# argriffing/phyly

Hardware: AMD Instinct MI355X
Metric: sites/sec (arbplf-ll) (higher is better)
Workload: dtype f64

## Files before the change

### phyly_amd/csrc/plk_engine.hip

```cpp
#include <hip/hip_runtime.h>
#include <algorithm>
#include <utility>
#include <climits>
#include <cmath>
#include <cstdio>
#include <cstdlib>
#include <cstring>
#include <dlfcn.h>
#include <mutex>
#include <set>
#include <string>
#include <type_traits>
#include <vector>

#include "plk.h"
#include "plk_dd.h"
#define PLK_K1_FN __host__ __device__ static inline
#include "plk_k1_check.h"
#include "plk_program.h"

#define PLK_MAX_K 64
#define PLK_MAX_C 64

enum LlFamily { LL_FUSED4 = 1, LL_GENERIC = 2, LL_MFMA = 3, LL_VEC = 4 };
struct LlPlan {
    LlFamily family = LL_GENERIC;
    PlkK4Choice k4;
    PlkK4Stream k4s;
    bool pair_tables = false;
    int npairs = 0;
    int block = 0, wg_sites = 0;
    size_t lds = 0;
    int mfma_T = 0;
    bool mfma_ns2 = false;
    bool vec_rs = false;
    int vec_reg_lo = 0;
    long info_variant = 0, info_form = 0, info_exec_flops = 0;
};

struct plk_engine {
    int device = 0;
    hipStream_t stream = nullptr, own_stream = nullptr;
    bool info_pending = false;
    hipEvent_t ev0 = nullptr, ev1 = nullptr, ev2 = nullptr, ev3 = nullptr;
    hipEvent_t evk[64][2] = {};
    bool evk_pending[64] = {};
    int evk_next = 0;
    long evk_sum_ns = 0, evk_count = 0;
    std::string err;

    int N = 0, E = 0;
    std::vector<int> indptr, indices, preorder, b_to_idx, idx_to_a;
    int *d_indptr = nullptr, *d_indices = nullptr, *d_preorder = nullptr;

    int k = 0, C = 0, K = 0, root_mode = 0;
    std::vector<double> Qn, edge_rates, cat_rates, cat_prior, root_w;
    double *d_Qn = nullptr, *d_edge_rates = nullptr, *d_cat_rates = nullptr, *d_cat_prior = nullptr;
    double *d_root_w = nullptr;
    dd *d_Pdd = nullptr;
    double *d_P = nullptr, *d_dP = nullptr;
    bool dp_valid = false;
    dd *d_scratch = nullptr;
    size_t pdd_cap = 0, p_cap = 0, dp_cap = 0, scratch_cap = 0;
    bool model_dirty = true;

    long S = 0, Spad = 0;
    int pat_mode = 0;
    uint8_t *d_codes = nullptr;
    int nchar = 0;
    std::vector<double> defs;
    std::vector<char> node_observed;
    double *d_defs = nullptr;
    double *d_B = nullptr;
    std::vector<char> node_has_data;
    std::vector<int> node_codes;
    double *d_w = nullptr;

    bool prog_dirty = true, fmt_dirty = true, tables_dirty = true;
    LlPlan plan;
    PlkK4StreamCaps k4_caps;
    size_t k4_static_lds[3] = {};
    hipError_t k4_static_lds_err[3] = {};
    bool k4_static_lds_known = false;
    PlkProgram pg;
    std::vector<plk_op2> &ops = pg.ops;
    std::vector<int> &op_edge = pg.op_edge;
    std::vector<int> &tip_edge = pg.tip_edge;
    std::vector<char> &scale_node = pg.scale_node;
    std::vector<int> &obs_nodes = pg.obs_nodes;
    int &slots_needed = pg.slots_needed;
    PlkFused fu;
    PlkFusedPT fpt;
    unsigned *d_words_pt = nullptr;
    PlkFusedV4 fv4;
    PlkVecPT vpt;
    unsigned *d_cstream = nullptr; size_t cstream_cap = 0;
    int *d_obs_row = nullptr;
    int *d_row_nodes = nullptr, *d_tabs = nullptr;
    uint8_t *d_quad_lut = nullptr;
    int *d_quad_codes = nullptr;
    double *d_llstate = nullptr; size_t llstate_cap = 0;
    int num_cus = 256;
    int2 *d_ops = nullptr;
    int4 *d_fops = nullptr;
    unsigned *d_words = nullptr;
    std::vector<int> &mat_edge = fu.mat_edge;
    int *d_op_edge = nullptr, *d_tip_edge = nullptr, *d_obs_nodes = nullptr, *d_mat_edge = nullptr, *d_edge_slot = nullptr;
    double *d_PS = nullptr;
    double *d_tip = nullptr;
    double *d_frag = nullptr; size_t frag_cap = 0;
    double *d_root_wd = nullptr;
    int4 *d_mops = nullptr;
    double *d_exL = nullptr, *d_exF = nullptr;
    int *d_exmask = nullptr;
    dd *d_exscr = nullptr;
    size_t exL_cap = 0, exF_cap = 0, exmask_cap = 0, exscr_cap = 0;
    int *d_u4pack = nullptr;
    double *d_u4tip = nullptr;
    size_t u4pack_cap = 0, u4tip_cap = 0;
    double *d_stage = nullptr; size_t stage_cap = 0;
    double *d_uvmat = nullptr; size_t uvmat_cap = 0;
    int mfma_first_mv = -1, mfma_first_slot = -1, mfma_first_row = 0, vec_second_row = 0;
    size_t ps_cap = 0, tip_cap = 0;

    int cp_kind = 0;
    bool cp_tables_valid = false;
    PlkFused cpf;
    hipEvent_t cp_ev0 = nullptr, cp_ev1 = nullptr;
    long info_cat_posterior_ns = 0;
    int4 *d_cp_fops = nullptr;
    int2 *d_cp_ops = nullptr;
    int *d_cp_mat_edge = nullptr, *d_cp_tip_edge = nullptr, *d_cp_obs_nodes = nullptr, *d_cp_op_edge = nullptr, *d_cp_expo = nullptr, *d_cp_flag = nullptr;
    double *d_cp_PS = nullptr, *d_cp_tip = nullptr, *d_cp_out = nullptr;
    dd *d_cp_partial = nullptr;
    size_t cp_ps_cap = 0, cp_tip_cap = 0, cp_out_cap = 0, cp_expo_cap = 0, cp_partial_cap = 0;

    double *d_slots = nullptr; size_t slots_cap = 0;
    double *d_site_ll = nullptr; size_t site_ll_cap = 0;
    dd *d_partial = nullptr; size_t partial_cap = 0;
    double *d_work = nullptr; size_t work_cap = 0;

    long opt_force_generic = 0, opt_site_chunk = 0, opt_fused_ns = 0, opt_fused_asm = 1, opt_mfma = 1, opt_up_nodes = 2, opt_pair_tables = 1, opt_vec_reg_stack = 1, opt_mfma_ns2 = 0, opt_stream_grid = 0;
    void *comm = nullptr;
    int comm_ranks = 0;
    long info_pair_sums_kernel = 0, info_query_ns = 0;
    double *d_mixD = nullptr; size_t mixd_cap = 0;
    long info_mixture_sens_kernel = 0;
    long info_nni_kernel = 0;
    dd *d_plPdd = nullptr; double *d_plP = nullptr, *d_plrates = nullptr, *d_plstream = nullptr, *d_plT = nullptr, *d_pldense = nullptr;
    uint8_t *d_plcodes = nullptr;
    size_t plpdd_cap = 0, plp_cap = 0, plrates_cap = 0, plstream_cap = 0, plt_cap = 0, pldense_cap = 0, plcodes_cap = 0;
    long info_place_kernel = 0;
    long info_up4_path = 0;
    long info_down4_kernel = 0;
    hipEvent_t q_ev0 = nullptr, q_ev1 = nullptr;
    long info_ll_kernel = 0, info_updown_kernel = 0, info_ll_kernel_ns = 0, info_ll_total_ns = 0, info_ll_variant = 0, info_ll_form = 0, info_ll_fold = 0, info_ll_pairmul = 0, info_ll_triple = 0, info_ll_quad = 0, info_ll_barrier = 0, info_ll_exec_flops = 0, info_cat_posterior_kernel = 0;
};

static std::string g_create_error;

struct PlkNcclId { char internal[128]; };
struct PlkRccl {
    void *lib = nullptr;
    int (*GetUniqueId)(void *) = nullptr;
    int (*CommInitRank)(void **, int,  PlkNcclId, int) = nullptr;
    int (*AllReduce)(const void *, void *, size_t, int, int, void *, hipStream_t) = nullptr;
    int (*CommDestroy)(void *) = nullptr;
    const char *(*GetErrorString)(int) = nullptr;
    std::string err;
};
static PlkRccl g_rccl;
static std::mutex g_rccl_mu;

static bool rccl_load()
{
    std::lock_guard<std::mutex> lk(g_rccl_mu);
    if (g_rccl.lib) return true;
    const char *names[] = {"librccl.so.1", "librccl.so"};
    void *lib = nullptr;
    for (const char *n : names) if (!lib) lib = dlopen(n, RTLD_NOW | RTLD_NOLOAD);
    for (const char *n : names) if (!lib) lib = dlopen(n, RTLD_NOW | RTLD_GLOBAL);
    if (!lib) { g_rccl.err = std::string("RCCL is not available: ") + (dlerror() ? dlerror() : "librccl.so.1 not found"); return false; }
    g_rccl.GetUniqueId = reinterpret_cast<int (*)(void *)>(dlsym(lib, "ncclGetUniqueId"));
    g_rccl.CommInitRank = reinterpret_cast<int (*)(void **, int, PlkNcclId, int)>(dlsym(lib, "ncclCommInitRank"));
    g_rccl.AllReduce = reinterpret_cast<int (*)(const void *, void *, size_t, int, int, void *, hipStream_t)>(dlsym(lib, "ncclAllReduce"));
    g_rccl.CommDestroy = reinterpret_cast<int (*)(void *)>(dlsym(lib, "ncclCommDestroy"));
    g_rccl.GetErrorString = reinterpret_cast<const char *(*)(int)>(dlsym(lib, "ncclGetErrorString"));
    if (!g_rccl.GetUniqueId || !g_rccl.CommInitRank || !g_rccl.AllReduce || !g_rccl.CommDestroy) { g_rccl.err = "RCCL: entry points missing"; return false; }
    g_rccl.lib = lib;
    return true;
}

static std::string rccl_text(int rc) { return g_rccl.GetErrorString ? g_rccl.GetErrorString(rc) : ("code " + std::to_string(rc)); }



static std::mutex g_live_mu;
static std::set<const plk_engine *> g_live;
static bool g_exiting = false, g_atexit_set = false;

static bool plk_live(const plk_engine *h)
{
    if (!h) return false;
    std::lock_guard<std::mutex> lk(g_live_mu);
    return !g_exiting && g_live.count(h) != 0;
}

#define HIPCHK(h, call)                                                            \
    do {                                                                           \
        hipError_t e_ = (call);                                                    \
        if (e_ != hipSuccess) {                                                    \
            (h)->err = std::string(#call) + ": " + hipGetErrorString(e_);         \
            return PLK_E_DEVICE;                                                   \
        }                                                                          \
    } while (0)

template <typename T>
static int dev_alloc(plk_engine *h, T **p, size_t n)
{
    if (*p) { (void)hipFree(*p); *p = nullptr; }
    if (n == 0) n = 1;
    hipError_t e = hipMalloc((void **)p, n * sizeof(T));
    if (e != hipSuccess) {
        h->err = std::string("hipMalloc: ") + hipGetErrorString(e);
        *p = nullptr;
        return PLK_E_NOMEM;
    }
    return PLK_OK;
}

template <typename T>
static int dev_upload(plk_engine *h, T **p, const T *src, size_t n)
{
    int rc = dev_alloc(h, p, n);
    if (rc) return rc;
    if (n) HIPCHK(h, hipMemcpy(*p, src, n * sizeof(T), hipMemcpyHostToDevice));
    return PLK_OK;
}

template <typename T>
static int dev_reserve(plk_engine *h, T **p, size_t *cap, size_t n)
{
    if (*p && *cap >= n) return PLK_OK;
    int rc = dev_alloc(h, p, n);
    *cap = rc ? 0 : n;
    return rc;
}


__device__ static inline dd dd_div_d(dd x, double y)
{
    double q1 = x.hi / y;
    dd p = dd_two_prod(q1, y);
    dd r = dd_add(x, dd_make(-p.hi, -p.lo));
// ... 1029 lines not shown
#pragma unroll
                        for (int i = 0; i < K; i++) fe[i] *= m2[i];
                    } else {
                        const double *ev = a.EV + ((size_t)idx2 * a.C + c) * a.k * n + slc;
#pragma unroll
                        for (int i = 0; i < K; i++)
                            if (i < a.k) fe[i] *= ev[(size_t)i * n];
                    }
                }
                const double prior = as_uniform(a.cat_prior)[c] * (a.CW ? a.CW[(size_t)c * n + slc] : 1.0);
                if (want_d) {
                    if (b_leaf) up_stage_obs<K>(a, b, sg, tid, xs);
                    else {
                        const double *lb = a.LN + ((size_t)b * a.C + c) * a.k * n + slc;
                        for (int j = 0; j < a.k; j++) xs[j][tid] = lb[(size_t)j * n];
                    }
                    double y[K];
                    if (idx == a.mod_edge) up_matvec<K, 2>(a.D2T + ((size_t)c * a.E + idx) * K * K, a.k, xs, tid, y);
                    else if (a.dzero) up_matvec<K, 2>(a.DT + ((size_t)c * a.E + idx) * K * K, a.k, xs, tid, y);
                    else up_matvec<K, 0>(a.DT + ((size_t)c * a.E + idx) * K * K, a.k, xs, tid, y);
                    double d = 0.0;
#pragma unroll
                    for (int i = 0; i < K; i++) d = fma(fe[i], y[i], d);
                    dsum = fma(prior, d, dsum);
                }
                if (want_f) {
#pragma unroll
                    for (int i = 0; i < K; i++) xs[i][tid] = fe[i];
                    double fb[K];
                    up_matvec<K, 0>((idx == a.mod_edge ? a.DN : a.PN) + ((size_t)c * a.E + idx) * K * K, a.k, xs, tid, fb);
                    if (!b_leaf) {
                        double *fo = a.FN + ((size_t)b * a.C + c) * a.k * n + slc;
#pragma unroll
                        for (int i = 0; i < K; i++)
                            if (i < a.k && valid) fo[(size_t)i * n] = fb[i];
                    }
                    if (want_m) {
                        if (b_leaf) {
                            double lb[K];
                            up_load_obs_reg<K>(a, b, sg, lb);
#pragma unroll
                            for (int i = 0; i < K; i++) macc[i] = fma(prior * fb[i], lb[i], macc[i]);
                        } else {
                            const double *lb = a.LN + ((size_t)b * a.C + c) * a.k * n + slc;
#pragma unroll
                            for (int i = 0; i < K; i++)
                                if (i < a.k) macc[i] = fma(prior * fb[i], lb[(size_t)i * n], macc[i]);
                        }
                    }
                }
            }
            if (want_d && valid) a.DV[(size_t)idx * n + sl] = dsum * inv;
            if (want_m) {
                double *mv = a.MV + (size_t)b * a.k * n + slc;
#pragma unroll
                for (int i = 0; i < K; i++)
                    if (i < a.k && valid) mv[(size_t)i * n] = macc[i] * inv;
            }
        }
    }
}

#include "plk_pairsums.h"
#include "plk_mixsens.h"
#include "plk_nni.h"
#include "plk_place.h"

__global__ void k_build_edge_stream(int k, int K, int mode, const double *__restrict__ M, double *__restrict__ out)
{
    const size_t ce = blockIdx.x;
    const double *src = M + ce * k * k;
    double *dst = out + ce * K * K;
    for (int idx = threadIdx.x; idx < K * K; idx += blockDim.x) {
        int r = idx / K, q = idx - r * K;
        double v = 0.0;
        if (r < k && q < k) v = mode == 0 ? src[q * k + r] : src[r * k + q];
        dst[idx] = v;
    }
}


static int pad_K(int k)
{
    const int ks[] = {2, 4, 8, 16, 20, 32, 61, 64};
    for (int v : ks) if (k <= v) return v;
    return -1;
}

extern "C" const char *plk_create_error(void) { return g_create_error.c_str(); }

extern "C" int plk_create(plk_engine **out, int device)
{
    if (!out) return PLK_E_ARG;
    *out = nullptr;
    int ndev = 0;
    hipError_t e = hipGetDeviceCount(&ndev);
    if (e != hipSuccess || ndev <= 0) {
        g_create_error = std::string("plk_create: no HIP device available (") +
                         (e != hipSuccess ? hipGetErrorString(e) : "device count 0") +
                         "); this engine has no CPU fallback";
        return PLK_E_DEVICE;
    }
    if (device < 0 || device >= ndev) {
        g_create_error = "plk_create: device index out of range";
        return PLK_E_ARG;
    }
    e = hipSetDevice(device);
    if (e != hipSuccess) {
        g_create_error = std::string("hipSetDevice: ") + hipGetErrorString(e);
        return PLK_E_DEVICE;
    }
    plk_engine *h = new plk_engine();
    h->device = device;
    { int cus = 0; if (hipDeviceGetAttribute(&cus, hipDeviceAttributeMultiprocessorCount, device) == hipSuccess && cus > 0) h->num_cus = cus; }
    if (const char *v = getenv("ARBPLF_UP_NODES")) h->opt_up_nodes = atol(v);
    if (hipStreamCreate(&h->own_stream) != hipSuccess ||
        hipEventCreate(&h->ev0) != hipSuccess || hipEventCreate(&h->ev1) != hipSuccess ||
        hipEventCreate(&h->ev2) != hipSuccess || hipEventCreate(&h->ev3) != hipSuccess) {
        g_create_error = "plk_create: stream/event creation failed";
        delete h;
        return PLK_E_DEVICE;
    }
    {
        std::lock_guard<std::mutex> lk(g_live_mu);
        if (!g_atexit_set) {
            g_atexit_set = true;
            atexit([]() { std::lock_guard<std::mutex> lk2(g_live_mu); g_exiting = true; g_live.clear(); });
        }
        g_live.insert(h);
    }
    h->stream = h->own_stream;
    for (int i = 0; i < 64; i++)
        if (hipEventCreate(&h->evk[i][0]) != hipSuccess || hipEventCreate(&h->evk[i][1]) != hipSuccess) {
            g_create_error = "plk_create: event creation failed";
            plk_destroy(h);
            return PLK_E_DEVICE;
        }
    *out = h;
    return PLK_OK;
}

extern "C" void plk_destroy(plk_engine *h)
{
    if (!h) return;
    {
        std::lock_guard<std::mutex> lk(g_live_mu);
        if (g_exiting || !g_live.erase(h)) return;
    }
    (void)hipSetDevice(h->device);
    if (h->comm && g_rccl.CommDestroy) { (void)hipStreamSynchronize(h->stream); (void)g_rccl.CommDestroy(h->comm); h->comm = nullptr; }
    void *ptrs[] = {h->d_indptr, h->d_indices, h->d_preorder, h->d_Qn, h->d_edge_rates, h->d_cat_rates,
                    h->d_cat_prior, h->d_root_w, h->d_Pdd, h->d_P, h->d_dP, h->d_scratch, h->d_codes,
                    h->d_defs, h->d_B, h->d_w, h->d_ops, h->d_fops, h->d_words, h->d_mat_edge, h->d_edge_slot, h->d_op_edge, h->d_tip_edge, h->d_obs_nodes,
                    h->d_words_pt, h->d_row_nodes, h->d_tabs, h->d_quad_lut, h->d_quad_codes, h->d_llstate, h->d_cstream, h->d_obs_row, h->d_PS, h->d_tip, h->d_frag, h->d_root_wd, h->d_mops, h->d_u4pack, h->d_u4tip, h->d_uvmat, h->d_stage, h->d_exL, h->d_exF, h->d_exmask, h->d_exscr, h->d_slots, h->d_site_ll, h->d_partial, h->d_work,
                    h->d_cp_fops, h->d_cp_ops, h->d_cp_mat_edge, h->d_cp_tip_edge, h->d_cp_obs_nodes, h->d_cp_op_edge, h->d_cp_expo, h->d_cp_flag,
                    h->d_cp_PS, h->d_cp_tip, h->d_cp_out, h->d_cp_partial, h->d_mixD,
                    h->d_plPdd, h->d_plP, h->d_plrates, h->d_plstream, h->d_plT, h->d_pldense, h->d_plcodes};
    for (void *p : ptrs) if (p) (void)hipFree(p);
    if (h->ev0) (void)hipEventDestroy(h->ev0);
    if (h->ev1) (void)hipEventDestroy(h->ev1);
    if (h->ev2) (void)hipEventDestroy(h->ev2);
    if (h->ev3) (void)hipEventDestroy(h->ev3);
    if (h->cp_ev0) (void)hipEventDestroy(h->cp_ev0);
    if (h->q_ev0) (void)hipEventDestroy(h->q_ev0);
    if (h->q_ev1) (void)hipEventDestroy(h->q_ev1);
    if (h->cp_ev1) (void)hipEventDestroy(h->cp_ev1);
    for (int i = 0; i < 64; i++) for (int j = 0; j < 2; j++) if (h->evk[i][j]) (void)hipEventDestroy(h->evk[i][j]);
    if (h->own_stream) (void)hipStreamDestroy(h->own_stream);
    delete h;
}

extern "C" const char *plk_last_error(const plk_engine *h) { return plk_live(h) ? h->err.c_str() : "invalid engine handle"; }

extern "C" int plk_set_option(plk_engine *h, int option, long value)
{
    if (!plk_live(h)) return PLK_E_ARG;
    if (option == PLK_OPT_FORCE_GENERIC) { h->opt_force_generic = value; h->prog_dirty = true; return PLK_OK; }
    if (option == PLK_OPT_SITE_CHUNK) { h->opt_site_chunk = value; return PLK_OK; }
    if (option == PLK_OPT_FUSED_SITES_PER_LANE) { h->opt_fused_ns = value; h->fmt_dirty = true; return PLK_OK; }
    if (option == PLK_OPT_FUSED_ASM) { h->opt_fused_asm = value; h->fmt_dirty = true; return PLK_OK; }
    if (option == PLK_OPT_UP_NODES) { h->opt_up_nodes = value; return PLK_OK; }
    if (option == PLK_OPT_MFMA) { h->opt_mfma = value; h->fmt_dirty = true; return PLK_OK; }
    if (option == PLK_OPT_MFMA_NS2) { h->opt_mfma_ns2 = value; h->fmt_dirty = true; return PLK_OK; }
    if (option == PLK_OPT_VEC_REG_STACK) { h->opt_vec_reg_stack = value; h->fmt_dirty = true; return PLK_OK; }
    if (option == PLK_OPT_PAIR_TABLES) { h->opt_pair_tables = value; h->fmt_dirty = true; return PLK_OK; }
    if (option == PLK_OPT_STREAM_GRID) {
        if (value < 0) { h->err = "PLK_OPT_STREAM_GRID: a workgroup count, or 0 for the default"; return PLK_E_ARG; }
        h->opt_stream_grid = value; h->fmt_dirty = true; return PLK_OK;
    }
    h->err = "plk_set_option: unknown option";
    return PLK_E_ARG;
}

static int evk_resolve(plk_engine *h, int i)
{
    if (!h->evk_pending[i]) return PLK_OK;
    float ms = 0;
    HIPCHK(h, hipEventSynchronize(h->evk[i][1]));
    HIPCHK(h, hipEventElapsedTime(&ms, h->evk[i][0], h->evk[i][1]));
    h->evk_pending[i] = false;
    h->info_ll_kernel_ns = (long)(ms * 1e6);
    h->evk_sum_ns += h->info_ll_kernel_ns;
    h->evk_count++;
    return PLK_OK;
}

extern "C" int plk_get_info(plk_engine *h, int what, long *out)
{
    if (!plk_live(h) || !out) return PLK_E_ARG;
    if (what >= PLK_INFO_LAST_LL_KERNEL_NS && what <= PLK_INFO_LL_KERNEL_COUNT) {
        HIPCHK(h, hipSetDevice(h->device));
        int rc;
        for (int j = 0; j < 64; j++) if ((rc = evk_resolve(h, (h->evk_next + j) & 63))) return rc;
        if (h->info_pending) {
            float ms_t = 0;
            HIPCHK(h, hipEventSynchronize(h->ev3));
            HIPCHK(h, hipEventElapsedTime(&ms_t, h->ev0, h->ev3));
            h->info_ll_total_ns = (long)(ms_t * 1e6);
            h->info_pending = false;
        }
    }
    switch (what) {
    case PLK_INFO_LL_KERNEL_NS_SUM: *out = h->evk_sum_ns; h->evk_sum_ns = 0; return PLK_OK;
    case PLK_INFO_LL_KERNEL_COUNT: *out = h->evk_count; h->evk_count = 0; return PLK_OK;
    case PLK_INFO_LL_KERNEL: *out = h->info_ll_kernel; return PLK_OK;
    case PLK_INFO_UPDOWN_KERNEL: *out = h->info_updown_kernel; return PLK_OK;
    case PLK_INFO_CAT_POSTERIOR_KERNEL: *out = h->info_cat_posterior_kernel; return PLK_OK;
    case PLK_INFO_CATEGORIES: *out = h->C; return PLK_OK;
    case PLK_INFO_LAST_CAT_POSTERIOR_NS: *out = h->info_cat_posterior_ns; return PLK_OK;
    case PLK_INFO_PAIR_SUMS_KERNEL: *out = h->info_pair_sums_kernel; return PLK_OK;
    case PLK_INFO_LAST_QUERY_NS: *out = h->info_query_ns; return PLK_OK;
    case PLK_INFO_MIXTURE_SENS_KERNEL: *out = h->info_mixture_sens_kernel; return PLK_OK;
    case PLK_INFO_NNI_KERNEL: *out = h->info_nni_kernel; return PLK_OK;
    case PLK_INFO_PLACE_KERNEL: *out = h->info_place_kernel; return PLK_OK;
    case PLK_INFO_UP4_PATH: *out = h->info_up4_path; return PLK_OK;
    case PLK_INFO_DOWN4_KERNEL: *out = h->info_down4_kernel; return PLK_OK;
    case PLK_INFO_LL_VARIANT: *out = h->info_ll_variant; return PLK_OK;
    case PLK_INFO_LL_FORM: *out = h->info_ll_form; return PLK_OK;
    case PLK_INFO_LL_FOLD: *out = h->info_ll_fold; return PLK_OK;
    case PLK_INFO_LL_PAIRMUL: *out = h->info_ll_pairmul; return PLK_OK;
    case PLK_INFO_LL_TRIPLE: *out = h->info_ll_triple; return PLK_OK;
    case PLK_INFO_LL_QUAD: *out = h->info_ll_quad; return PLK_OK;
    case PLK_INFO_LL_BARRIER: *out = h->info_ll_barrier; return PLK_OK;
    case PLK_INFO_LL_EXEC_FLOPS: *out = h->info_ll_exec_flops; return PLK_OK;
    case PLK_INFO_PAIR_TABLES: *out = !h->fmt_dirty && h->plan.pair_tables ? h->plan.npairs : 0; return PLK_OK;
    case PLK_INFO_STACK_SLOTS: *out = h->slots_needed; return PLK_OK;
    case PLK_INFO_PROGRAM_OPS: *out = (long)h->ops.size(); return PLK_OK;
    case PLK_INFO_LAST_LL_KERNEL_NS: *out = h->info_ll_kernel_ns; return PLK_OK;
    case PLK_INFO_LAST_LL_TOTAL_NS: *out = h->info_ll_total_ns; return PLK_OK;
    }
    h->err = "plk_get_info: unknown item";
    return PLK_E_ARG;
}

extern "C" int plk_set_tree(plk_engine *h, int N, const int *indptr, const int *indices, const int *preorder)
{
    if (!plk_live(h)) return PLK_E_ARG;
    if (N < 2 || !indptr || !indices || !preorder) { h->err = "plk_set_tree: bad arguments"; return PLK_E_ARG; }
    HIPCHK(h, hipSetDevice(h->device));
    const int E = N - 1;
    if (indptr[0] != 0 || indptr[N] != E) { h->err = "plk_set_tree: indptr does not describe N-1 edges"; return PLK_E_ARG; }
    std::vector<int> b2i(N, -1), i2a(E, -1);
    for (int a = 0; a < N; a++) {
        if (indptr[a + 1] < indptr[a]) { h->err = "plk_set_tree: indptr not monotone"; return PLK_E_ARG; }
        for (int idx = indptr[a]; idx < indptr[a + 1]; idx++) {
            int b = indices[idx];
            if (b < 0 || b >= N || b == a || b2i[b] != -1) { h->err = "plk_set_tree: not a tree"; return PLK_E_ARG; }
            b2i[b] = idx;
            i2a[idx] = a;
        }
    }
    std::vector<char> seen(N, 0);
    for (int u = 0; u < N; u++) {
        int a = preorder[u];
        if (a < 0 || a >= N || seen[a]) { h->err = "plk_set_tree: preorder is not a permutation"; return PLK_E_ARG; }
        if (u == 0 ? b2i[a] != -1 : (b2i[a] == -1 || !seen[i2a[b2i[a]]])) {
            h->err = "plk_set_tree: preorder does not start at the root / parents first";
            return PLK_E_ARG;
        }
        seen[a] = 1;
    }
    h->N = N; h->E = E;
    h->indptr.assign(indptr, indptr + N + 1);
    h->indices.assign(indices, indices + E);
    h->preorder.assign(preorder, preorder + N);
    h->b_to_idx = b2i; h->idx_to_a = i2a;
    int rc;
    if ((rc = dev_upload(h, &h->d_indptr, indptr, (size_t)N + 1))) return rc;
    if ((rc = dev_upload(h, &h->d_indices, indices, (size_t)E))) return rc;
    if ((rc = dev_upload(h, &h->d_preorder, preorder, (size_t)N))) return rc;
    h->prog_dirty = true;
    h->model_dirty = true;
    h->pat_mode = 0;
    h->k = 0;
    return PLK_OK;
}

#define K1_CSR_NOTE " (edges numbered in CSR order)"

static int k1_check(plk_engine *h, const char *who, const double *edge_rates)
{
    char msg[320];
    const size_t kk = (size_t)h->k * h->k;
    if (plk_k1_check_values(h->k, h->C, h->E, h->Qn.data(), h->Qn.data() + kk, edge_rates, h->cat_rates.data(), h->cat_prior.data(),
                            h->root_mode, h->root_w.data(), msg, sizeof msg)) {
        h->err = std::string(who) + ": " + msg + K1_CSR_NOTE;
        return PLK_E_ARG;
// ... 270 lines not shown

static bool use_vec(const plk_engine *h)
{
    return !h->opt_force_generic && h->opt_mfma == 1 && h->pat_mode == 1 && h->k >= 9 && h->k <= 32;
}

static bool use_mfma(const plk_engine *h)
{
    return !h->opt_force_generic && h->opt_mfma && h->pat_mode == 1 && h->k >= 9 && h->k <= 64;
}

static size_t mfma_ll_lds_bytes(const plk_engine *h, int sites)
{
    const int T = (h->k + 15) / 16, kk4 = (h->k + 3) / 4;
    return (size_t)T * kk4 * 64 * sizeof(double) + h->obs_nodes.size() * (size_t)sites;
}

static int vec_reg_window(const plk_engine *h)
{
    std::vector<long> per_slot(std::max(h->slots_needed, 1), 0);
    for (const plk_op2 &o : h->ops) if ((o.x & 0xff) == OP_PUSH && o.y < (int)per_slot.size()) per_slot[o.y]++;
    long best = -1;
    int lo_best = 0;
    for (int lo = 0; lo + 3 <= std::max(h->slots_needed, 3); lo++) {
        long cnt = 0;
        for (int q = lo; q < lo + 3 && q < (int)per_slot.size(); q++) cnt += per_slot[q];
        if (cnt > best) { best = cnt; lo_best = lo; }
    }
    return lo_best;
}

static int upload_pair_table_lists(plk_engine *h)
{
    const PlkFusedPT &f = h->fpt;
    int rc;
    const size_t nrows = f.row_node.size(), ntab = f.tab_unit.size();
    std::vector<int> rn(5 * nrows, -1);
    for (size_t r = 0; r < nrows; r++) {
        rn[r] = f.row_node[r]; rn[nrows + r] = f.row_node2[r];
        if (r < f.row_node3.size()) rn[2 * nrows + r] = f.row_node3[r];
        if (r < f.row_node4.size()) { rn[3 * nrows + r] = f.row_node4[r]; rn[4 * nrows + r] = f.row_lut[r]; }
    }
    if ((rc = dev_upload(h, &h->d_row_nodes, rn.data(), rn.size()))) return rc;
    auto kind = [&](size_t t) { return t < f.tab_shape.size() && f.tab_shape[t] ? 2 : t < f.tab_el.size() && f.tab_el[t] >= 0 ? 1 : 0; };
    std::vector<size_t> order;
    for (int pass = 0; pass < 3; pass++)
        for (size_t t = 0; t < ntab; t++) if (kind(t) == pass) order.push_back(t);
    std::vector<int> tabs(10 * ntab, -1);
    std::vector<int> qcodes;
    for (size_t q = 0; q < ntab; q++) {
        const size_t t = order[q];
        tabs[q] = f.tab_unit[t]; tabs[ntab + q] = f.tab_edge[t]; tabs[2 * ntab + q] = f.tab_eb[t]; tabs[3 * ntab + q] = f.tab_ec[t];
        if (t < f.tab_el.size()) { tabs[4 * ntab + q] = f.tab_ea[t]; tabs[5 * ntab + q] = f.tab_el[t]; }
        if (t < f.tab_shape.size()) { tabs[6 * ntab + q] = f.tab_shape[t]; tabs[7 * ntab + q] = f.tab_et[t]; tabs[8 * ntab + q] = f.tab_ef[t]; tabs[9 * ntab + q] = f.tab_eg[t]; }
        if (kind(t) != 2) continue;
        const int row = t < f.tab_row.size() ? f.tab_row[t] : -1;
        if (row < 0 || (size_t)row >= nrows || f.row_lut[row] < 0 || h->node_codes.size() != (size_t)h->N) { h->err = "internal: a four-leaf table without its rank tables"; return PLK_E_ARG; }
        const int nd[4] = {f.row_node[row], f.row_node2[row], f.row_node3[row], f.row_node4[row]};
        for (int j = 0; j < 4; j++) {
            int code_of[4];
            plk_v4q_rank_codes(h->node_codes[nd[j]], code_of);
            qcodes.insert(qcodes.end(), code_of, code_of + 4);
        }
    }
    if (f.nquads > 0) {
        if ((rc = dev_upload(h, &h->d_quad_lut, f.lut.data(), f.lut.size()))) return rc;
        if ((rc = dev_upload(h, &h->d_quad_codes, qcodes.data(), qcodes.size()))) return rc;
    }
    return dev_upload(h, &h->d_tabs, tabs.data(), tabs.size());
}

static int stream_cus(const plk_engine *h) { return h->opt_stream_grid > 0 ? (int)std::min<long>(h->opt_stream_grid, h->num_cus) : h->num_cus; }

static int upload_formats_fused4(plk_engine *h, LlPlan &p)
{
    int rc;
    if (!h->k4_static_lds_known) {
        const void *fns[3] = {(const void *)k_ll_fused4_v4s<768>, (const void *)k_ll_fused4_v4<768>, (const void *)k_ll_fused4_v4<512>};
        for (int i = 0; i < 3; i++) {
            hipFuncAttributes fa;
            h->k4_static_lds_err[i] = hipFuncGetAttributes(&fa, fns[i]);
            if (h->k4_static_lds_err[i] == hipSuccess) h->k4_static_lds[i] = fa.sharedSizeBytes;
            else (void)hipGetLastError();
        }
        auto same_static_lds = [&](const void *fn) {
            hipFuncAttributes fh;
            if (hipFuncGetAttributes(&fh, fn) != hipSuccess) { (void)hipGetLastError(); return false; }
            return h->k4_static_lds_err[PLK_K4_LDS_V4S_768] == hipSuccess && fh.sharedSizeBytes == h->k4_static_lds[PLK_K4_LDS_V4S_768];
        };
        h->k4_caps.held = same_static_lds((const void *)k_ll_fused4_v4s<768, true>);
        h->k4_caps.pair = same_static_lds((const void *)k_ll_fused4_v4s<768, true, true>);
        h->k4_caps.groups = same_static_lds((const void *)k_ll_fused4_v4s<768, true, true, true>);
        h->k4_static_lds_known = true;
    }
    PlkK4Shape sh = {h->nchar, h->C, h->S, stream_cus(h), h->opt_pair_tables, h->opt_fused_asm, h->opt_fused_ns, {}};
    std::copy(h->k4_static_lds, h->k4_static_lds + 3, sh.static_lds);
    sh.node_codes = h->nchar <= 16 && h->node_codes.size() == (size_t)h->N ? h->node_codes.data() : nullptr;
    const long nunits = (h->S + PLK_V4S_UNIT - 1) / PLK_V4S_UNIT;
    PlkFusedV4S fv4s;
    p.k4 = plk_k4_choose(h->N, h->indptr.data(), h->indices.data(), h->pg, sh, h->k4_static_lds_err[PLK_K4_LDS_V4S_768] == hipSuccess, h->fu, h->fpt, h->fv4, fv4s);
    if (p.k4.variant == PLK_K4_V4S && dev_reserve(h, &h->d_cstream, &h->cstream_cap, (size_t)nunits * fv4s.chunks * PLK_V4S_UNIT) != PLK_OK) {
        h->err.clear();
        (void)hipGetLastError();
        p.k4 = plk_k4_choose(h->N, h->indptr.data(), h->indices.data(), h->pg, sh, false, h->fu, h->fpt, h->fv4, fv4s);
    }
    const PlkK4Choice &c = p.k4;
    if (c.variant == PLK_K4_NONE) return PLK_OK;
    if (c.variant == PLK_K4_V4) HIPCHK(h, h->k4_static_lds_err[c.tile == 1536 ? PLK_K4_LDS_V4_768 : PLK_K4_LDS_V4_512]);
    if (!c.bad.empty()) { h->err = "internal: " + c.bad; return PLK_E_ARG; }
    p.family = LL_FUSED4;
    p.block = c.block; p.wg_sites = c.tile; p.lds = c.lds;
    p.info_variant = c.variant == PLK_K4_CPP ? 3 : c.variant == PLK_K4_ASM ? 1 : c.variant == PLK_K4_ASM_PT ? 5 : 6;
    p.info_form = c.variant == PLK_K4_V4S ? 1 : 0;
    if (c.variant == PLK_K4_V4S) {
        PlkK4StreamCaps caps = h->k4_caps;
        if (c.triple.nodes + c.triple.quads > 0 && c.triple.groups > 1 && plk_k4_stream_can_group(c, caps) &&
            dev_reserve(h, &h->d_llstate, &h->llstate_cap, (size_t)nunits * PLK_V4S_UNIT * 3 / 2) != PLK_OK) {
            h->err.clear();
            (void)hipGetLastError();
            caps.partial_sums = false;
        }
        p.k4s = plk_k4_stream(h->N, h->indptr.data(), h->indices.data(), h->pg, sh, c, caps, h->fpt, std::move(fv4s));
        p.lds = p.k4s.lds;
        if (!p.k4s.note.empty()) h->err = p.k4s.note;
    }
    const int ntips = (int)h->tip_edge.size();
    if (c.variant == PLK_K4_CPP || c.variant == PLK_K4_ASM) {
        if ((rc = dev_upload(h, &h->d_fops, reinterpret_cast<const int4 *>(h->fu.fops.data()), h->fu.fops.size()))) return rc;
        if ((rc = dev_upload(h, &h->d_words, h->fu.words.data(), h->fu.words.size()))) return rc;
        std::vector<int> me = h->mat_edge;
        me.push_back(-1);
        if ((rc = dev_upload(h, &h->d_mat_edge, me.data(), me.size()))) return rc;
        std::vector<int> em(2 * (size_t)h->E, -1);
        for (size_t mi = 0; mi < h->mat_edge.size(); mi++) em[h->mat_edge[mi]] = (int)mi;
        for (int t = 0; t < ntips; t++) em[(size_t)h->E + h->tip_edge[t]] = t;
        if ((rc = dev_upload(h, &h->d_edge_slot, em.data(), em.size()))) return rc;
        if ((rc = dev_reserve(h, &h->d_PS, &h->ps_cap, (size_t)h->C * (h->mat_edge.size() + 1) * 16))) return rc;
        if ((rc = dev_reserve(h, &h->d_tip, &h->tip_cap, (size_t)h->C * (ntips + 1) * h->nchar * 4))) return rc;
        HIPCHK(h, hipMemsetAsync(h->d_PS, 0, (size_t)h->C * (h->mat_edge.size() + 1) * 16 * sizeof(double), h->stream));
        hipLaunchKernelGGL(k_build_tip, dim3(ntips + 1, h->C), dim3(64), 0, h->stream,
                           h->E, ntips + 1, h->nchar, h->d_tip_edge, h->d_Pdd, h->d_defs, h->d_tip);
        HIPCHK(h, hipGetLastError());
        return PLK_OK;
    }
    const PlkFusedPT &f = h->fpt;
    p.pair_tables = true; p.npairs = f.npairs;
    const PlkFusedV4S &vs = p.k4s.fv4s;
    const std::vector<unsigned> &words = c.variant == PLK_K4_V4S ? p.k4s.words() : c.variant == PLK_K4_V4 ? h->fv4.words : f.words;
    if ((rc = dev_upload(h, &h->d_words_pt, words.data(), words.size()))) return rc;
    if (c.variant == PLK_K4_V4S && (rc = dev_upload(h, &h->d_obs_row, vs.obs_row.data(), vs.obs_row.size()))) return rc;
    if ((rc = upload_pair_table_lists(h))) return rc;
    if (c.variant == PLK_K4_V4S) {
        const size_t total = (size_t)nunits * vs.chunks * PLK_V4S_UNIT;
        if (total > h->cstream_cap || (total + 255) / 256 > 0x7fffffffu) { h->err = "internal: code stream size"; return PLK_E_ARG; }
        hipLaunchKernelGGL(k_build_code_stream, dim3((unsigned)((total + 255) / 256)), dim3(256), 0, h->stream, h->d_codes, h->Spad, nunits,
                           h->d_obs_row, vs.nobs, h->d_row_nodes, (int)f.row_node.size(), h->nchar, vs.chunks,
                           f.nquads > 0 ? h->d_quad_lut : (const uint8_t *)nullptr, h->d_cstream);
        HIPCHK(h, hipGetLastError());
    }
    std::vector<int> em(2 * (size_t)h->E, -1);
    for (size_t mi = 0; mi < f.mat_edge.size(); mi++) em[f.mat_edge[mi]] = (int)mi;
    if ((rc = dev_upload(h, &h->d_edge_slot, em.data(), em.size()))) return rc;
    if ((rc = dev_reserve(h, &h->d_PS, &h->ps_cap, (size_t)h->C * (f.mat_edge.size() + 1) * 16))) return rc;
    if ((rc = dev_reserve(h, &h->d_tip, &h->tip_cap, (size_t)h->C * f.units * h->nchar * 4))) return rc;
    HIPCHK(h, hipMemsetAsync(h->d_PS, 0, (size_t)h->C * (f.mat_edge.size() + 1) * 16 * sizeof(double), h->stream));
    return PLK_OK;
}

static int upload_formats_generic(plk_engine *h, LlPlan &p)
{
    int rc;
    const int nops = (int)h->ops.size();
    std::vector<plk_op2> gops(h->ops);
    int first = -1, prev = -1;
    for (int pc = 0; pc < nops; pc++)
        if ((gops[pc].x & 0xff) == OP_MATVEC) {
            if (first < 0) first = pc;
            if (prev >= 0) gops[prev].y = pc;
            prev = pc;
        }
    if (prev >= 0) gops[prev].y = first;
    if ((rc = dev_upload(h, &h->d_ops, reinterpret_cast<const int2 *>(gops.data()), gops.size()))) return rc;
    if ((rc = dev_upload(h, &h->d_op_edge, h->op_edge.data(), h->op_edge.size()))) return rc;
    if ((rc = dev_reserve(h, &h->d_PS, &h->ps_cap, (size_t)h->C * std::max(nops, 1) * h->K * h->K))) return rc;
    p.family = LL_GENERIC;
    p.block = GEN_BLOCK; p.wg_sites = GEN_BLOCK;
    return PLK_OK;
}

static int upload_formats_vec(plk_engine *h, LlPlan &p)
{
    int rc;
    if ((rc = upload_formats_generic(h, p))) return rc;
    p.family = LL_VEC;
    p.block = VEC_BLOCK; p.wg_sites = VEC_BLOCK;
    p.vec_rs = h->opt_vec_reg_stack && h->K <= 20 && h->slots_needed >= 1;
    p.vec_reg_lo = p.vec_rs ? vec_reg_window(h) : 0;
    if (h->opt_pair_tables && h->K <= 32 && !h->obs_nodes.empty()) {
        const long per_pair = (long)h->nchar * h->nchar * h->K * (long)sizeof(double);
        const int max_pairs = (int)std::min<long>(INT_MAX, (64L << 20) / std::max<long>(per_pair, 1));
        plk_fused_pt_build(h->N, h->indptr.data(), h->indices.data(), h->pg, h->nchar, max_pairs, h->fpt, false);
        if (h->fpt.npairs > 0) {
            plk_vec_pt_build(h->fpt, h->nchar, h->vpt);
            const std::string bad = plk_vec_pt_check(h->N, h->indptr.data(), h->indices.data(), h->pg, h->fpt, h->vpt, h->nchar, h->E);
            if (!bad.empty()) { h->err = "internal: " + bad; return PLK_E_ARG; }
            if ((rc = upload_pair_table_lists(h)) ||
                (rc = dev_upload(h, &h->d_mops, reinterpret_cast<const int4 *>(h->vpt.ops.data()), h->vpt.ops.size())) ||
                (rc = dev_upload(h, &h->d_op_edge, h->vpt.op_edge.data(), h->vpt.op_edge.size())) ||
                (rc = dev_reserve(h, &h->d_PS, &h->ps_cap, (size_t)h->C * h->vpt.ops.size() * h->K * h->K)) ||
                (rc = dev_reserve(h, &h->d_tip, &h->tip_cap, (size_t)h->C * h->fpt.units * h->nchar * h->K))) return rc;
            p.pair_tables = true; p.npairs = h->fpt.npairs;
            return PLK_OK;
        }
    }
    if ((rc = dev_reserve(h, &h->d_tip, &h->tip_cap, (size_t)h->C * (h->tip_edge.size() + 1) * h->nchar * h->K))) return rc;
    PlkChain ch;
    plk_chain_build(h->N, h->pg, 3, h->indices.data(), nullptr, nullptr, nullptr, ch);
    const std::string bad = plk_chain_check(h->N, h->pg, ch, 3, INT_MAX, 0, 0, 0, 0, 0);
    if (!bad.empty()) { h->err = "internal: " + bad; return PLK_E_ARG; }
    h->mfma_first_slot = ch.first_slot; h->mfma_first_row = ch.first_row; h->vec_second_row = ch.second_row;
    return dev_upload(h, &h->d_mops, reinterpret_cast<const int4 *>(ch.ops.data()), ch.ops.size());
}

static int upload_formats_mfma(plk_engine *h, LlPlan &p)
{
    int rc;
    if ((rc = upload_formats_generic(h, p))) return rc;
    const int nops = (int)h->ops.size(), ntips = (int)h->tip_edge.size();
    const int T = (h->k + 15) / 16, R = 4 * T, kk4 = (h->k + 3) / 4;
    p.family = LL_MFMA;
    p.mfma_T = T;
    p.mfma_ns2 = h->opt_mfma_ns2 == 1 && T >= 3 && mfma_ll_lds_bytes(h, 2 * MF_SITES) <= PLK_LDS_LIMIT;
    p.block = MF_BLOCK; p.wg_sites = p.mfma_ns2 ? 2 * MF_SITES : MF_SITES;
    p.lds = mfma_ll_lds_bytes(h, p.wg_sites);
    std::vector<double> rwd((size_t)4 * R, 0.0);
    for (int i = 0; i < h->k; i++) rwd[(size_t)(i & 3) * R + (i >> 2)] = h->root_w[i];
    if ((rc = dev_upload(h, &h->d_root_wd, rwd.data(), rwd.size()))) return rc;
    if ((rc = dev_reserve(h, &h->d_frag, &h->frag_cap, (size_t)h->C * nops * T * kk4 * 64))) return rc;
    if ((rc = dev_reserve(h, &h->d_tip, &h->tip_cap, (size_t)h->C * (ntips + 1) * h->nchar * 4 * R))) return rc;
    PlkChain ch;
    plk_chain_build(h->N, h->pg, 0, nullptr, nullptr, nullptr, nullptr, ch);
    const std::string bad = plk_chain_check(h->N, h->pg, ch, 0, INT_MAX, 0, 0, 0, MF_SITES, (size_t)h->obs_nodes.size() * MF_SITES);
    if (!bad.empty()) { h->err = "internal: " + bad; return PLK_E_ARG; }
    h->mfma_first_slot = ch.first_slot; h->mfma_first_row = ch.first_row;
    h->mfma_first_mv = -1;
    for (size_t pc = 0; pc < h->pg.ops.size() && h->mfma_first_mv < 0; pc++) if ((h->pg.ops[pc].x & 0xff) == OP_MATVEC) h->mfma_first_mv = (int)pc;
    return dev_upload(h, &h->d_mops, reinterpret_cast<const int4 *>(ch.ops.data()), ch.ops.size());
}

static long ll_exec_flops(const plk_engine *h, const LlPlan &p)
{
    long nprod = 0, nmul = 0;
    if (p.family == LL_VEC && p.pair_tables) {
        for (const PlkFusedPT::VOp &o : h->fpt.vops) { if (o.code == OP_MATVEC) nprod++; if (o.code == OP_TIP_MUL || o.code == OP_POPMUL) nmul++; }
    } else if (p.family == LL_FUSED4 && p.pair_tables) {
        nprod = (long)h->fpt.mat_edge.size();
        for (unsigned w : h->fpt.words) {
            const unsigned hx = w & 31;
            if (hx == OP_TIP_MUL || hx == PLK_WORD_TIPMUL_NOWAIT || hx == PLK_WORD_MATVEC_TIPMUL) nmul++;
            if ((hx >= 16 && hx < 20) || hx >= 28 || (hx >= PLK_WORD_SET_POPMUL && hx < PLK_WORD_SET_POPMUL + 4)) nmul++;
        }
    } else {
        for (const plk_op2 &o : h->ops) {
            const int code = o.x & 0xff;
            if (code == OP_MATVEC) nprod++;
            if (code == OP_TIP_MUL || code == OP_NODE_MUL || code == OP_POPMUL) nmul++;
            if ((code == OP_TIP_SET || code == OP_TIP_MUL) && p.family == LL_GENERIC) { nprod++; if (code == OP_TIP_MUL) nmul++; }
        }
    }
    const long kp = p.family == LL_MFMA ? (h->k + 15) / 16 * 16 : h->k;
    return (long)h->C * (nprod * (2 * kp * kp - kp) + nmul * h->k);
}

static int upload_formats(plk_engine *h)
{
    int rc;
    h->fmt_dirty = true;
    std::vector<int> te = h->tip_edge;
    te.push_back(-1);
    if ((rc = dev_upload(h, &h->d_tip_edge, te.data(), te.size()))) return rc;
    if ((rc = dev_upload(h, &h->d_obs_nodes, h->obs_nodes.data(), h->obs_nodes.size()))) return rc;
    LlPlan p;
    if (!h->opt_force_generic && h->k == 4 && h->pat_mode == 1 && (rc = upload_formats_fused4(h, p))) return rc;
    if (p.family != LL_FUSED4) {
        if (use_vec(h)) rc = upload_formats_vec(h, p);
        else if (use_mfma(h) && mfma_ll_lds_bytes(h, MF_SITES) <= PLK_LDS_LIMIT) rc = upload_formats_mfma(h, p);
        else rc = upload_formats_generic(h, p);
        if (rc) return rc;
    }
    p.info_exec_flops = ll_exec_flops(h, p);
    h->plan = std::move(p);
    h->fmt_dirty = false;
    h->tables_dirty = true;
    return PLK_OK;
}

static int build_tables(plk_engine *h)
{
    const LlPlan &p = h->plan;
    const int nops = (int)h->ops.size(), ntips = (int)h->tip_edge.size(), K = h->K, C = h->C;
    if (p.family == LL_FUSED4) return run_expm(h, true);
    if (p.family == LL_VEC && p.pair_tables) {
        const int nv = (int)h->vpt.ops.size(), ntab = (int)h->fpt.tab_unit.size();
        hipLaunchKernelGGL(k_build_stream, dim3(nv, C), dim3(K * K >= 256 ? 256 : 64), 0, h->stream,
                           h->k, K, h->E, nv, h->d_op_edge, h->d_P, h->d_PS);
        hipLaunchKernelGGL(k_build_tables_pt_vec, dim3(ntab, C, 8), dim3(256), (size_t)4 * h->nchar * h->k * sizeof(double), h->stream,
                           h->k, K, h->E, ntab, h->fpt.units, h->nchar, h->d_tabs, h->d_Pdd, h->d_defs, h->d_tip);
        HIPCHK(h, hipGetLastError());
        h->tables_dirty = false;
        return PLK_OK;
    }
    if (nops > 0)
        hipLaunchKernelGGL(k_build_stream, dim3(nops, C), dim3(K * K >= 256 ? 256 : 64), 0, h->stream,
                           h->k, K, h->E, nops, h->d_op_edge, h->d_P, h->d_PS);
    if (p.family == LL_VEC) {
        hipLaunchKernelGGL(k_build_tip_vec, dim3(ntips + 1, C), dim3(256), 0, h->stream,
                           h->k, K, h->E, ntips, h->nchar, h->d_tip_edge, h->d_Pdd, h->d_defs, h->d_tip);
    } else if (p.family == LL_MFMA) {
        const int T = p.mfma_T, R = 4 * T, kk4 = (h->k + 3) / 4;
        hipLaunchKernelGGL(k_build_frag, dim3(nops, C), dim3(256), 0, h->stream,
                           h->k, T, kk4, h->E, nops, h->d_op_edge, h->d_P, h->d_frag);
        hipLaunchKernelGGL(k_build_tip_dist, dim3(ntips + 1, C), dim3(256), 0, h->stream,
                           h->k, R, h->E, ntips, h->nchar, h->d_tip_edge, h->d_Pdd, h->d_defs, h->K, h->d_tip);
    }
    HIPCHK(h, hipGetLastError());
    h->tables_dirty = false;
    return PLK_OK;
}

template <int D, int NS>
static void launch_fused(plk_engine *h, const FusedArgs &a, unsigned grid, size_t lds)
{
    hipLaunchKernelGGL((k_ll_fused4<D, NS>), dim3(grid), dim3(PLK_TILE), lds, h->stream, a);
}

template <typename F>
static void dispatch_K(int K, F &&f)
{
    switch (K) {
    case 2: f(std::integral_constant<int, 2>{}); break;
    case 4: f(std::integral_constant<int, 4>{}); break;
    case 8: f(std::integral_constant<int, 8>{}); break;
    case 16: f(std::integral_constant<int, 16>{}); break;
    case 20: f(std::integral_constant<int, 20>{}); break;
    case 32: f(std::integral_constant<int, 32>{}); break;
    case 61: f(std::integral_constant<int, 61>{}); break;
    default: f(std::integral_constant<int, 64>{}); break;
    }
}

template <int K>
static void launch_generic(plk_engine *h, const GenArgs &a, unsigned grid)
{
    hipLaunchKernelGGL(k_ll_generic<K>, dim3(grid), dim3(GEN_BLOCK), 0, h->stream, a);
}

#define PLK_PARTIAL_OFF 72

static int reserve_partials(plk_engine *h, bool want_sum, unsigned n, dd **partial)
{
    *partial = nullptr;
    if (!want_sum) return PLK_OK;
    const int rc = dev_reserve(h, &h->d_partial, &h->partial_cap, (size_t)n + PLK_PARTIAL_OFF);
    if (rc == PLK_OK) *partial = h->d_partial + PLK_PARTIAL_OFF;
    return rc;
}

static int launch_ll_fused4(plk_engine *h, const LlPlan &p, double *d_out, bool want_sum, unsigned *npartials)
{
    const PlkK4Choice &c = p.k4;
    const long S = h->S;
    const int ntiles = (int)((S + p.wg_sites - 1) / p.wg_sites);
    unsigned grid = (unsigned)ntiles;
    if (c.variant == PLK_K4_V4S) grid = (unsigned)std::min<long>(((S + PLK_V4S_UNIT - 1) / PLK_V4S_UNIT + 11) / 12, stream_cus(h));
    else if (c.variant == PLK_K4_V4 || c.variant == PLK_K4_ASM_PT) grid = (unsigned)std::min(ntiles, c.tile == 512 ? 2 * h->num_cus : h->num_cus);
    *npartials = c.variant == PLK_K4_V4S ? grid * 12 : (unsigned)ntiles;
    int rc;
    FusedArgs a;
    if ((rc = reserve_partials(h, want_sum, *npartials, &a.partial))) return rc;
    a.S = S; a.Spad = h->Spad; a.C = h->C; a.nops = (int)h->ops.size(); a.nmat = (int)h->mat_edge.size();
    a.ntips = (int)h->tip_edge.size() + 1; a.nchar = h->nchar; a.nobs = (int)h->obs_nodes.size();
    a.ops = h->d_fops; a.PS = h->d_PS; a.tip = h->d_tip;
    a.codes = h->d_codes; a.obs_nodes = h->d_obs_nodes; a.defs = h->d_defs;
    a.cat_prior = h->d_cat_prior; a.root_w = h->d_root_w; a.w = h->d_w;
    a.site_ll = d_out;
    a.root_mode = h->root_mode; a.first_row = h->fu.first_row;
    if (p.pair_tables) {
        const PlkFusedPT &f = h->fpt;
        FusedPTArgs pa;
        pa.f = a;
        pa.f.nmat = (int)f.mat_edge.size(); pa.f.ntips = f.units; pa.f.nobs = (int)f.row_node.size();
        pa.words = h->d_words_pt; pa.row_nodes = h->d_row_nodes; pa.nwords = (int)(c.variant == PLK_K4_ASM_PT ? f.words.size() : h->fv4.words.size());
        pa.first_unit = f.first_unit; pa.first_row = f.first_row; pa.second_row = f.second_row; pa.ntiles = ntiles;
        pa.warm = c.warm;
        if (c.variant == PLK_K4_V4S) {
            FusedV4SArgs sa;
            sa.pt = pa;
            const PlkK4Stream &r = p.k4s;
            const bool pairmul = r.runs == PlkK4Stream::PAIR;
            sa.pt.nwords = (int)r.stride();
            sa.stream = h->d_cstream; sa.chunks = r.fv4s.chunks; sa.first_y = r.fv4s.first_y[0];
            sa.sync = r.sync;
            h->info_ll_barrier = (sa.sync == 0 ? 1 : sa.sync == 1 ? 2 : 3) | (r.sync_auto ? 16 : 0);
            sa.first_y1 = pairmul ? r.pair.first_y1[0] : 0u; sa.first_b1 = pairmul ? r.pair.first_b1 : 0u;
            sa.groups = r.triple.groups; sa.cg = r.triple.Cg > 0 ? r.triple.Cg : h->C;
            sa.part_sum = h->d_llstate;
            sa.part_exp = h->d_llstate ? reinterpret_cast<int *>(h->d_llstate + (size_t)((S + PLK_V4S_UNIT - 1) / PLK_V4S_UNIT) * PLK_V4S_UNIT) : nullptr;
            if (sa.groups > 1) {
                if (!pairmul || !h->d_llstate || h->llstate_cap < (size_t)((S + PLK_V4S_UNIT - 1) / PLK_V4S_UNIT) * PLK_V4S_UNIT * 3 / 2) { h->err = "internal: category groups without their plan"; return PLK_E_ARG; }
                hipLaunchKernelGGL((k_ll_fused4_v4s<768, true, true, true>), dim3(grid), dim3(p.block), p.lds, h->stream, sa);
            } else if (pairmul) hipLaunchKernelGGL((k_ll_fused4_v4s<768, true, true>), dim3(grid), dim3(p.block), p.lds, h->stream, sa);
            else if (r.held) hipLaunchKernelGGL((k_ll_fused4_v4s<768, true>), dim3(grid), dim3(p.block), p.lds, h->stream, sa);
            else hipLaunchKernelGGL((k_ll_fused4_v4s<768, false>), dim3(grid), dim3(p.block), p.lds, h->stream, sa);
        } else if (c.variant == PLK_K4_V4) {
            FusedV4Args va;
            va.pt = pa; va.first_y = h->fv4.first_y; va.first_z = h->fv4.first_z; va.second_z = h->fv4.second_z;
            if (c.tile == 1536) hipLaunchKernelGGL(k_ll_fused4_v4<768>, dim3(grid), dim3(p.block), p.lds, h->stream, va);
            else hipLaunchKernelGGL(k_ll_fused4_v4<512>, dim3(grid), dim3(p.block), p.lds, h->stream, va);
        } else if (c.tile == 1024) hipLaunchKernelGGL(k_ll_fused4_asm_pt<1024>, dim3(grid), dim3(p.block), p.lds, h->stream, pa);
        else hipLaunchKernelGGL(k_ll_fused4_asm_pt<512>, dim3(grid), dim3(p.block), p.lds, h->stream, pa);
        return PLK_OK;
    }
    if (c.variant == PLK_K4_ASM) {
        FusedAsmArgs aa;
        aa.f = a; aa.words = h->d_words;
        aa.first_tip = h->fu.asm_first_tip; aa.first_row = h->fu.asm_first_row; aa.second_row = h->fu.asm_second_row;
        aa.pack4 = c.pack4;
        if (c.D == 4) hipLaunchKernelGGL(k_ll_fused4_asm<4>, dim3(grid), dim3(p.block), p.lds, h->stream, aa);
        else hipLaunchKernelGGL(k_ll_fused4_asm<8>, dim3(grid), dim3(p.block), p.lds, h->stream, aa);
        return PLK_OK;
    }
    if (c.NS == 2) {
        if (c.D == 4) launch_fused<4, 2>(h, a, grid, p.lds);
        else launch_fused<8, 2>(h, a, grid, p.lds);
    } else {
        if (c.D == 4) launch_fused<4, 1>(h, a, grid, p.lds);
        else if (c.D == 8) launch_fused<8, 1>(h, a, grid, p.lds);
        else launch_fused<16, 1>(h, a, grid, p.lds);
    }
    return PLK_OK;
}

static int launch_ll_vec(plk_engine *h, const LlPlan &p, double *d_out, bool want_sum, unsigned *npartials)
{
    const long S = h->S;
    const int K = h->K;
    const unsigned grid = (unsigned)((S + p.wg_sites - 1) / p.wg_sites);
    *npartials = grid;
    int rc;
    VecArgs a;
    if ((rc = reserve_partials(h, want_sum, grid, &a.partial))) return rc;
    if ((rc = dev_reserve(h, &h->d_slots, &h->slots_cap, (size_t)std::max(h->slots_needed, 1) * K * S))) return rc;
    a.S = S; a.Spad = h->Spad; a.k = h->k; a.C = h->C; a.nops = (int)h->ops.size(); a.ntips = (int)h->tip_edge.size(); a.nchar = h->nchar;
    a.root_mode = h->root_mode; a.ops = h->d_mops; a.PS = h->d_PS; a.tip = h->d_tip; a.codes = h->d_codes;
    a.obs_nodes = h->d_obs_nodes; a.first_slot = h->mfma_first_slot; a.first_row = h->mfma_first_row; a.second_row = h->vec_second_row;
    a.obs_nodes2 = nullptr; a.units = 0;
    if (p.pair_tables) {
        const int nrows = (int)h->fpt.row_node.size();
        a.nops = (int)h->vpt.ops.size(); a.obs_nodes = h->d_row_nodes; a.obs_nodes2 = h->d_row_nodes + nrows; a.units = h->fpt.units;
        a.first_slot = 0; a.first_row = h->vpt.first_row;
    }
    a.cat_prior = h->d_cat_prior; a.root_w = h->d_root_w; a.w = h->d_w; a.slots = h->d_slots; a.site_ll = d_out;
    a.reg_lo = p.vec_reg_lo;
    if (p.vec_rs && K == 16) hipLaunchKernelGGL((k_ll_vec_rs<16, 3>), dim3(grid), dim3(p.block), 0, h->stream, a);
    else if (p.vec_rs) hipLaunchKernelGGL((k_ll_vec_rs<20, 3>), dim3(grid), dim3(p.block), 0, h->stream, a);
    else if (K == 16) hipLaunchKernelGGL(k_ll_vec<16>, dim3(grid), dim3(p.block), 0, h->stream, a);
    else if (K == 20) hipLaunchKernelGGL(k_ll_vec<20>, dim3(grid), dim3(p.block), 0, h->stream, a);
    else hipLaunchKernelGGL(k_ll_vec<32>, dim3(grid), dim3(p.block), 0, h->stream, a);
    return PLK_OK;
}

static int launch_ll_mfma(plk_engine *h, const LlPlan &p, double *d_out, bool want_sum, unsigned *npartials)
{
    const long S = h->S;
    const int T = p.mfma_T, R = 4 * T, kk4 = (h->k + 3) / 4;
    const unsigned grid = (unsigned)((S + p.wg_sites - 1) / p.wg_sites);
    *npartials = grid;
    int rc;
    MfmaArgs a;
    if ((rc = reserve_partials(h, want_sum, grid, &a.partial))) return rc;
    const long slot_stride = (long)grid * p.wg_sites * 4;
    if ((rc = dev_reserve(h, &h->d_slots, &h->slots_cap, (size_t)std::max(h->slots_needed, 1) * R * slot_stride))) return rc;
    a.S = S; a.Spad = h->Spad; a.k = h->k; a.kk4 = kk4; a.C = h->C; a.nops = (int)h->ops.size(); a.ntips = (int)h->tip_edge.size();
    a.nchar = h->nchar; a.root_mode = h->root_mode; a.ops = h->d_mops; a.frag = h->d_frag; a.tip = h->d_tip;
    a.obs_nodes = h->d_obs_nodes; a.nobs = (int)h->obs_nodes.size();
    a.first_slot = h->mfma_first_slot; a.first_row = h->mfma_first_row; a.first_mv = h->mfma_first_mv;
    a.codes = h->d_codes; a.cat_prior = h->d_cat_prior; a.root_wd = h->d_root_wd; a.w = h->d_w;
    a.slots = h->d_slots; a.slot_stride = slot_stride; a.site_ll = d_out;
    if (p.mfma_ns2 && T == 3) hipLaunchKernelGGL(k_ll_mfma_ns2<3>, dim3(grid), dim3(p.block), p.lds, h->stream, a);
    else if (p.mfma_ns2) hipLaunchKernelGGL(k_ll_mfma_ns2<4>, dim3(grid), dim3(p.block), p.lds, h->stream, a);
    else if (T == 1) hipLaunchKernelGGL(k_ll_mfma<1>, dim3(grid), dim3(p.block), p.lds, h->stream, a);
    else if (T == 2) hipLaunchKernelGGL(k_ll_mfma<2>, dim3(grid), dim3(p.block), p.lds, h->stream, a);
    else if (T == 3) hipLaunchKernelGGL(k_ll_mfma_occ4<3>, dim3(grid), dim3(p.block), p.lds, h->stream, a);
    else hipLaunchKernelGGL(k_ll_mfma_occ4<4>, dim3(grid), dim3(p.block), p.lds, h->stream, a);
    return PLK_OK;
}

static int launch_ll_generic(plk_engine *h, const LlPlan &p, double *d_out, bool want_sum, unsigned *npartials)
{
    const long S = h->S;
    const unsigned grid = (unsigned)((S + p.wg_sites - 1) / p.wg_sites);
    *npartials = grid;
    int rc;
    GenArgs a;
    if ((rc = reserve_partials(h, want_sum, grid, &a.partial))) return rc;
    if ((rc = dev_reserve(h, &h->d_slots, &h->slots_cap, (size_t)std::max(h->slots_needed, 1) * h->k * S))) return rc;
    a.S = S; a.Spad = h->Spad; a.k = h->k; a.C = h->C; a.nops = (int)h->ops.size(); a.nchar = h->nchar;
    a.pat_mode = h->pat_mode; a.root_mode = h->root_mode; a.ops = h->d_ops; a.PS = h->d_PS;
    a.codes = h->d_codes; a.defs = h->d_defs; a.B = h->d_B; a.cat_prior = h->d_cat_prior;
    a.root_w = h->d_root_w; a.w = h->d_w; a.slots = h->d_slots; a.site_ll = d_out;
    dispatch_K(h->K, [&](auto Kc) { launch_generic<decltype(Kc)::value>(h, a, grid); });
    return PLK_OK;
}

static int ll_impl(plk_engine *h, double *site_ll_out, int where, double *sum_out, double *sum_dev, bool async)
{
    if (h->k == 0 || h->pat_mode == 0) { h->err = "plk_ll: tree, model and patterns must be set"; return PLK_E_ARG; }
    HIPCHK(h, hipSetDevice(h->device));
    int rc;
    HIPCHK(h, hipEventRecord(h->ev0, h->stream));
    if (h->prog_dirty) { if ((rc = build_program(h))) return rc; }
    if (h->fmt_dirty) { if ((rc = upload_formats(h))) return rc; }
    if (h->model_dirty) { if ((rc = run_expm(h, true, false))) return rc; }
    if (h->tables_dirty) { if ((rc = build_tables(h))) return rc; }
    const LlPlan &p = h->plan;
    const bool want_sum = sum_out || sum_dev;
    const long S = h->S;
    double *d_out = nullptr;
    if (site_ll_out) {
        if (where == PLK_DEVICE) d_out = site_ll_out;
        else { if ((rc = dev_reserve(h, &h->d_site_ll, &h->site_ll_cap, (size_t)S))) return rc; d_out = h->d_site_ll; }
    }
    const int evi = h->evk_next;
    h->evk_next = (evi + 1) & 63;
    if ((rc = evk_resolve(h, evi))) return rc;
    HIPCHK(h, hipEventRecord(h->evk[evi][0], h->stream));
    unsigned npartials = 0;
    h->info_ll_barrier = 0;
    switch (p.family) {
    case LL_FUSED4: rc = launch_ll_fused4(h, p, d_out, want_sum, &npartials); break;
    case LL_VEC: rc = launch_ll_vec(h, p, d_out, want_sum, &npartials); break;
    case LL_MFMA: rc = launch_ll_mfma(h, p, d_out, want_sum, &npartials); break;
    default: rc = launch_ll_generic(h, p, d_out, want_sum, &npartials); break;
    }
    if (rc) return rc;
    h->info_ll_kernel = p.family; h->info_ll_variant = p.info_variant; h->info_ll_form = p.info_form; h->info_ll_fold = p.k4s.info_fold; h->info_ll_pairmul = p.k4s.info_pairmul; h->info_ll_triple = p.k4s.info_triple; h->info_ll_quad = p.k4s.info_quad; h->info_ll_exec_flops = p.info_exec_flops;
    HIPCHK(h, hipGetLastError());
    HIPCHK(h, hipEventRecord(h->evk[evi][1], h->stream));
    h->evk_pending[evi] = true;
    if (want_sum) {
        dd *out = sum_dev ? reinterpret_cast<dd *>(sum_dev) : h->d_partial;
        const int g2 = npartials > 1024 ? (int)std::min<unsigned>(64u, (npartials + 511) / 512) : 1;
        if (g2 > 1) {
            hipLaunchKernelGGL(k_dd_slices, dim3(g2), dim3(256), 0, h->stream, (int)npartials, h->d_partial + PLK_PARTIAL_OFF, h->d_partial + 4);
            hipLaunchKernelGGL(k_dd_final, dim3(1), dim3(64), 0, h->stream, g2, h->d_partial + 4, out);
        } else {
            hipLaunchKernelGGL(k_dd_final, dim3(1), dim3(256), 0, h->stream, (int)npartials, h->d_partial + PLK_PARTIAL_OFF, out);
        }
// ... 2127 lines not shown
```

### phyly_amd/csrc/plk_fused4_v4p_asm.h

```cpp
#ifndef PLK_FUSED4_V4P_ASM_H
#define PLK_FUSED4_V4P_ASM_H

#define PLK_V4P_STACK_SLOTS 3
#define PLK_V4P_FOLD_ADV 36
#define PLK_V4P_PAIR_EVEN 52
#define PLK_V4P_PAIR_ODD 55
#define PLK_V4P_GEN_OBS_EVEN {0, 1, 3, 4, 12, 13, 14, 20, 21, 22}
#define PLK_V4P_GEN_OBS_ODD {5, 11, 15, 19, 23, 27, 31, -1, 59, 63}
#define PLK_V4P_GEN_OBS_FOLDED {1, 4, 12, 13, 14, 21, 22}

#define PLK_V4P_PROGRAM_HELD \
        "v_mov_b32 v24, 0\n\t" \
        "v_mov_b32 v25, 0x3ff00000\n\t" \
        "v_mov_b32 v32, 0\n\t" \
        "v_mov_b32 v33, 0x3ff00000\n\t" \
        "v_mov_b32 v26, 0\n\t" \
        "v_mov_b32 v27, 0x3ff00000\n\t" \
        "v_mov_b32 v34, 0\n\t" \
        "v_mov_b32 v35, 0x3ff00000\n\t" \
        "v_mov_b32 v28, 0\n\t" \
        "v_mov_b32 v29, 0x3ff00000\n\t" \
        "v_mov_b32 v36, 0\n\t" \
        "v_mov_b32 v37, 0x3ff00000\n\t" \
        "v_mov_b32 v30, 0\n\t" \
        "v_mov_b32 v31, 0x3ff00000\n\t" \
        "v_mov_b32 v38, 0\n\t" \
        "v_mov_b32 v39, 0x3ff00000\n\t" \
        "v_mov_b32 v76, %[voff]\n\t" \
        "s_mov_b64 s[34:35], %[strm]\n\t" \
        "v_mov_b64 v[74:75], %[c0]\n\t" \
        "v_mov_b64 v[146:147], %[c1]\n\t" \
        "v_mov_b64 v[148:149], %[c2]\n\t" \
        "s_add_u32 s34, s34, 0x600\n\t" \
        "s_addc_u32 s35, s35, 0\n\t" \
        "v_mov_b32 v78, 0\n\t" \
        "v_mov_b32 v79, 0\n\t" \
        "s_mov_b64 s[20:21], %[ops]\n\t" \
        "s_mov_b64 s[30:31], %[mstream]\n\t" \
        "s_movk_i32 s27, 0xfc02\n\t" \
        "s_mov_b32 m0, 0\n\t" \
        "s_load_dwordx16 s[68:83], s[20:21], 0x0\n\t" \
        "s_load_dwordx16 s[84:99], s[20:21], 0x40\n\t" \
        "s_add_u32 s20, s20, 0x80\n\t" \
        "s_addc_u32 s21, s21, 0\n\t" \
        "s_load_dwordx16 s[36:51], s[30:31], 0x0\n\t" \
        "s_load_dwordx16 s[52:67], s[30:31], 0x40\n\t" \
        "s_getpc_b64 s[24:25]\n\t" \
        ".Lpcref_%=:\n" \
        "s_add_u32 s26, s24, .Lh0_%=-.Lpcref_%=\n\t" \
        "s_addc_u32 s25, s25, 0\n\t" \
        "v_bfe_u32 v72, v74, 0, 8\n\t" \
        "v_bfe_u32 v73, v75, 0, 8\n\t" \
        "v_add_lshl_u32 v72, v72, %[y0], 5\n\t" \
        "v_add_lshl_u32 v73, v73, %[y0], 5\n\t" \
        "ds_read_b128 v[56:59], v72\n\t" \
        "ds_read_b128 v[60:63], v72 offset:16\n\t" \
        "ds_read_b128 v[64:67], v73\n\t" \
        "ds_read_b128 v[68:71], v73 offset:16\n\t" \
        "v_bfe_u32 v72, v74, %[b1], 8\n\t" \
        "v_bfe_u32 v73, v75, %[b1], 8\n\t" \
        "v_add_lshl_u32 v72, v72, %[y1], 5\n\t" \
        "v_add_lshl_u32 v73, v73, %[y1], 5\n\t" \
        "ds_read_b128 v[130:133], v72\n\t" \
        "ds_read_b128 v[134:137], v72 offset:16\n\t" \
        "ds_read_b128 v[138:141], v73\n\t" \
        "ds_read_b128 v[142:145], v73 offset:16\n\t" \
        "s_waitcnt lgkmcnt(0)\n\t" \
        "s_movrels_b64 s[22:23], s[68:69]\n\t" \
        "s_addk_i32 m0, 0x2\n\t" \
        "s_or_b32 s24, s26, s22\n\t" \
        "s_setpc_b64 s[24:25]\n\t" \
        ".p2align 15\n" \
        ".Lh0_%=:\n" \
        "s_waitcnt lgkmcnt(0)\n\t" \
        "v_mov_b64 v[24:25], v[56:57]\n\t" \
        "v_mov_b64 v[32:33], v[64:65]\n\t" \
        "v_mov_b64 v[26:27], v[58:59]\n\t" \
        "v_mov_b64 v[34:35], v[66:67]\n\t" \
        "v_mov_b64 v[28:29], v[60:61]\n\t" \
        "v_mov_b64 v[36:37], v[68:69]\n\t" \
        "v_mov_b64 v[30:31], v[62:63]\n\t" \
        "v_mov_b64 v[38:39], v[70:71]\n\t" \
        "s_lshr_b32 s28, s23, 16\n\t" \
        "v_bfe_u32 v72, v74, s23, 8\n\t" \
        "v_bfe_u32 v73, v75, s23, 8\n\t" \
        "v_add_lshl_u32 v72, v72, s28, 5\n\t" \
        "v_add_lshl_u32 v73, v73, s28, 5\n\t" \
        "ds_read_b128 v[56:59], v72\n\t" \
        "ds_read_b128 v[60:63], v72 offset:16\n\t" \
        "ds_read_b128 v[64:67], v73\n\t" \
        "ds_read_b128 v[68:71], v73 offset:16\n\t" \
        "s_movrels_b64 s[22:23], s[68:69]\n\t" \
        "s_addk_i32 m0, 0x2\n\t" \
        "s_or_b32 s24, s26, s22\n\t" \
        "s_setpc_b64 s[24:25]\n\t" \
        ".p2align 9\n" \
        "s_waitcnt lgkmcnt(0)\n\t" \
        "v_mul_f64 v[24:25], v[24:25], v[56:57]\n\t" \
        "v_mul_f64 v[32:33], v[32:33], v[64:65]\n\t" \
        "v_mul_f64 v[26:27], v[26:27], v[58:59]\n\t" \
        "v_mul_f64 v[34:35], v[34:35], v[66:67]\n\t" \
        "v_mul_f64 v[28:29], v[28:29], v[60:61]\n\t" \
        "v_mul_f64 v[36:37], v[36:37], v[68:69]\n\t" \
        "v_mul_f64 v[30:31], v[30:31], v[62:63]\n\t" \
        "v_mul_f64 v[38:39], v[38:39], v[70:71]\n\t" \
        "s_lshr_b32 s28, s23, 16\n\t" \
        "v_bfe_u32 v72, v74, s23, 8\n\t" \
        "v_bfe_u32 v73, v75, s23, 8\n\t" \
        "v_add_lshl_u32 v72, v72, s28, 5\n\t" \
        "v_add_lshl_u32 v73, v73, s28, 5\n\t" \
        "ds_read_b128 v[56:59], v72\n\t" \
        "ds_read_b128 v[60:63], v72 offset:16\n\t" \
        "ds_read_b128 v[64:67], v73\n\t" \
        "ds_read_b128 v[68:71], v73 offset:16\n\t" \
        "s_movrels_b64 s[22:23], s[68:69]\n\t" \
        "s_addk_i32 m0, 0x2\n\t" \
        "s_or_b32 s24, s26, s22\n\t" \
        "s_setpc_b64 s[24:25]\n\t" \
        ".p2align 9\n" \
        "s_waitcnt lgkmcnt(0)\n\t" \
        "v_mul_f64 v[40:41], s[36:37], v[24:25]\n\t" \
        "v_mul_f64 v[48:49], s[36:37], v[32:33]\n\t" \
        "v_mul_f64 v[42:43], s[38:39], v[24:25]\n\t" \
        "v_mul_f64 v[50:51], s[38:39], v[32:33]\n\t" \
        "v_mul_f64 v[44:45], s[40:41], v[24:25]\n\t" \
        "v_mul_f64 v[52:53], s[40:41], v[32:33]\n\t" \
        "v_mul_f64 v[46:47], s[42:43], v[24:25]\n\t" \
        "v_mul_f64 v[54:55], s[42:43], v[32:33]\n\t" \
        "v_fma_f64 v[40:41], s[44:45], v[26:27], v[40:41]\n\t" \
        "v_fma_f64 v[48:49], s[44:45], v[34:35], v[48:49]\n\t" \
        "v_fma_f64 v[42:43], s[46:47], v[26:27], v[42:43]\n\t" \
        "v_fma_f64 v[50:51], s[46:47], v[34:35], v[50:51]\n\t" \
        "v_fma_f64 v[44:45], s[48:49], v[26:27], v[44:45]\n\t" \
        "v_fma_f64 v[52:53], s[48:49], v[34:35], v[52:53]\n\t" \
        "v_fma_f64 v[46:47], s[50:51], v[26:27], v[46:47]\n\t" \
        "v_fma_f64 v[54:55], s[50:51], v[34:35], v[54:55]\n\t" \
        "v_fma_f64 v[40:41], s[52:53], v[28:29], v[40:41]\n\t" \
        "v_fma_f64 v[48:49], s[52:53], v[36:37], v[48:49]\n\t" \
        "v_fma_f64 v[42:43], s[54:55], v[28:29], v[42:43]\n\t" \
        "v_fma_f64 v[50:51], s[54:55], v[36:37], v[50:51]\n\t" \
        "v_fma_f64 v[44:45], s[56:57], v[28:29], v[44:45]\n\t" \
        "v_fma_f64 v[52:53], s[56:57], v[36:37], v[52:53]\n\t" \
        "v_fma_f64 v[46:47], s[58:59], v[28:29], v[46:47]\n\t" \
        "v_fma_f64 v[54:55], s[58:59], v[36:37], v[54:55]\n\t" \
        "v_fma_f64 v[24:25], s[60:61], v[30:31], v[40:41]\n\t" \
        "v_fma_f64 v[32:33], s[60:61], v[38:39], v[48:49]\n\t" \
        "v_fma_f64 v[26:27], s[62:63], v[30:31], v[42:43]\n\t" \
        "v_fma_f64 v[34:35], s[62:63], v[38:39], v[50:51]\n\t" \
        "v_fma_f64 v[28:29], s[64:65], v[30:31], v[44:45]\n\t" \
        "v_fma_f64 v[36:37], s[64:65], v[38:39], v[52:53]\n\t" \
        "v_fma_f64 v[30:31], s[66:67], v[30:31], v[46:47]\n\t" \
        "v_fma_f64 v[38:39], s[66:67], v[38:39], v[54:55]\n\t" \
        "s_add_u32 s30, s30, 0x80\n\t" \
        "s_addc_u32 s31, s31, 0\n\t" \
        "s_load_dwordx16 s[36:51], s[30:31], 0x0\n\t" \
        "s_load_dwordx16 s[52:67], s[30:31], 0x40\n\t" \
        "s_movrels_b64 s[22:23], s[68:69]\n\t" \
        "s_addk_i32 m0, 0x2\n\t" \
        "s_or_b32 s24, s26, s22\n\t" \
        "s_setpc_b64 s[24:25]\n\t" \
        ".p2align 9\n" \
        "v_mul_f64 v[24:25], v[24:25], v[56:57]\n\t" \
        "v_mul_f64 v[32:33], v[32:33], v[64:65]\n\t" \
        "v_mul_f64 v[26:27], v[26:27], v[58:59]\n\t" \
        "v_mul_f64 v[34:35], v[34:35], v[66:67]\n\t" \
        "v_mul_f64 v[28:29], v[28:29], v[60:61]\n\t" \
        "v_mul_f64 v[36:37], v[36:37], v[68:69]\n\t" \
        "v_mul_f64 v[30:31], v[30:31], v[62:63]\n\t" \
        "v_mul_f64 v[38:39], v[38:39], v[70:71]\n\t" \
        "s_lshr_b32 s28, s23, 16\n\t" \
        "v_bfe_u32 v72, v74, s23, 8\n\t" \
        "v_bfe_u32 v73, v75, s23, 8\n\t" \
        "v_add_lshl_u32 v72, v72, s28, 5\n\t" \
        "v_add_lshl_u32 v73, v73, s28, 5\n\t" \
        "ds_read_b128 v[56:59], v72\n\t" \
        "ds_read_b128 v[60:63], v72 offset:16\n\t" \
        "ds_read_b128 v[64:67], v73\n\t" \
        "ds_read_b128 v[68:71], v73 offset:16\n\t" \
        "s_movrels_b64 s[22:23], s[68:69]\n\t" \
        "s_addk_i32 m0, 0x2\n\t" \
        "s_or_b32 s24, s26, s22\n\t" \
        "s_setpc_b64 s[24:25]\n\t" \
        ".p2align 9\n" \
        "s_waitcnt lgkmcnt(0)\n\t" \
        "v_mul_f64 v[40:41], s[36:37], v[24:25]\n\t" \
        "v_mul_f64 v[48:49], s[36:37], v[32:33]\n\t" \
        "v_mul_f64 v[42:43], s[38:39], v[24:25]\n\t" \
        "v_mul_f64 v[50:51], s[38:39], v[32:33]\n\t" \
        "v_mul_f64 v[44:45], s[40:41], v[24:25]\n\t" \
        "v_mul_f64 v[52:53], s[40:41], v[32:33]\n\t" \
        "v_mul_f64 v[46:47], s[42:43], v[24:25]\n\t" \
        "v_mul_f64 v[54:55], s[42:43], v[32:33]\n\t" \
        "v_fma_f64 v[40:41], s[44:45], v[26:27], v[40:41]\n\t" \
        "v_fma_f64 v[48:49], s[44:45], v[34:35], v[48:49]\n\t" \
        "v_fma_f64 v[42:43], s[46:47], v[26:27], v[42:43]\n\t" \
        "v_fma_f64 v[50:51], s[46:47], v[34:35], v[50:51]\n\t" \
        "v_fma_f64 v[44:45], s[48:49], v[26:27], v[44:45]\n\t" \
        "v_fma_f64 v[52:53], s[48:49], v[34:35], v[52:53]\n\t" \
        "v_fma_f64 v[46:47], s[50:51], v[26:27], v[46:47]\n\t" \
        "v_fma_f64 v[54:55], s[50:51], v[34:35], v[54:55]\n\t" \
        "v_fma_f64 v[40:41], s[52:53], v[28:29], v[40:41]\n\t" \
        "v_fma_f64 v[48:49], s[52:53], v[36:37], v[48:49]\n\t" \
        "v_fma_f64 v[42:43], s[54:55], v[28:29], v[42:43]\n\t" \
        "v_fma_f64 v[50:51], s[54:55], v[36:37], v[50:51]\n\t" \
        "v_fma_f64 v[44:45], s[56:57], v[28:29], v[44:45]\n\t" \
        "v_fma_f64 v[52:53], s[56:57], v[36:37], v[52:53]\n\t" \
        "v_fma_f64 v[46:47], s[58:59], v[28:29], v[46:47]\n\t" \
        "v_fma_f64 v[54:55], s[58:59], v[36:37], v[54:55]\n\t" \
        "v_fma_f64 v[24:25], s[60:61], v[30:31], v[40:41]\n\t" \
        "v_fma_f64 v[32:33], s[60:61], v[38:39], v[48:49]\n\t" \
        "v_fma_f64 v[26:27], s[62:63], v[30:31], v[42:43]\n\t" \
        "v_fma_f64 v[34:35], s[62:63], v[38:39], v[50:51]\n\t" \
        "v_fma_f64 v[28:29], s[64:65], v[30:31], v[44:45]\n\t" \
        "v_fma_f64 v[36:37], s[64:65], v[38:39], v[52:53]\n\t" \
        "v_fma_f64 v[30:31], s[66:67], v[30:31], v[46:47]\n\t" \
// ... 1571 lines not shown
        "v_mul_f64 v[46:47], s[42:43], v[24:25]\n\t" \
        "v_mul_f64 v[54:55], s[42:43], v[32:33]\n\t" \
        "v_fma_f64 v[40:41], s[44:45], v[26:27], v[40:41]\n\t" \
        "v_fma_f64 v[48:49], s[44:45], v[34:35], v[48:49]\n\t" \
        "v_fma_f64 v[42:43], s[46:47], v[26:27], v[42:43]\n\t" \
        "v_fma_f64 v[50:51], s[46:47], v[34:35], v[50:51]\n\t" \
        "v_fma_f64 v[44:45], s[48:49], v[26:27], v[44:45]\n\t" \
        "v_fma_f64 v[52:53], s[48:49], v[34:35], v[52:53]\n\t" \
        "v_fma_f64 v[46:47], s[50:51], v[26:27], v[46:47]\n\t" \
        "v_fma_f64 v[54:55], s[50:51], v[34:35], v[54:55]\n\t" \
        "v_fma_f64 v[40:41], s[52:53], v[28:29], v[40:41]\n\t" \
        "v_fma_f64 v[48:49], s[52:53], v[36:37], v[48:49]\n\t" \
        "v_fma_f64 v[42:43], s[54:55], v[28:29], v[42:43]\n\t" \
        "v_fma_f64 v[50:51], s[54:55], v[36:37], v[50:51]\n\t" \
        "v_fma_f64 v[44:45], s[56:57], v[28:29], v[44:45]\n\t" \
        "v_fma_f64 v[52:53], s[56:57], v[36:37], v[52:53]\n\t" \
        "v_fma_f64 v[46:47], s[58:59], v[28:29], v[46:47]\n\t" \
        "v_fma_f64 v[54:55], s[58:59], v[36:37], v[54:55]\n\t" \
        "v_fma_f64 v[24:25], s[60:61], v[30:31], v[40:41]\n\t" \
        "v_fma_f64 v[32:33], s[60:61], v[38:39], v[48:49]\n\t" \
        "v_fma_f64 v[26:27], s[62:63], v[30:31], v[42:43]\n\t" \
        "v_fma_f64 v[34:35], s[62:63], v[38:39], v[50:51]\n\t" \
        "v_fma_f64 v[28:29], s[64:65], v[30:31], v[44:45]\n\t" \
        "v_fma_f64 v[36:37], s[64:65], v[38:39], v[52:53]\n\t" \
        "v_fma_f64 v[30:31], s[66:67], v[30:31], v[46:47]\n\t" \
        "v_fma_f64 v[38:39], s[66:67], v[38:39], v[54:55]\n\t" \
        "s_add_u32 s30, s30, 0x80\n\t" \
        "s_addc_u32 s31, s31, 0\n\t" \
        "s_load_dwordx16 s[36:51], s[30:31], 0x0\n\t" \
        "s_load_dwordx16 s[52:67], s[30:31], 0x40\n\t" \
        "v_mul_f64 v[24:25], v[24:25], v[98:99]\n\t" \
        "v_mul_f64 v[32:33], v[32:33], v[106:107]\n\t" \
        "v_mul_f64 v[26:27], v[26:27], v[100:101]\n\t" \
        "v_mul_f64 v[34:35], v[34:35], v[108:109]\n\t" \
        "v_mul_f64 v[28:29], v[28:29], v[102:103]\n\t" \
        "v_mul_f64 v[36:37], v[36:37], v[110:111]\n\t" \
        "v_mul_f64 v[30:31], v[30:31], v[104:105]\n\t" \
        "v_mul_f64 v[38:39], v[38:39], v[112:113]\n\t" \
        "v_max_u32 v80, v25, v27\n\t" \
        "v_max3_u32 v80, v29, v31, v80\n\t" \
        "v_lshrrev_b32 v80, 20, v80\n\t" \
        "v_sub_u32 v72, 0x3fe, v80\n\t" \
        "v_ldexp_f64 v[24:25], v[24:25], v72\n\t" \
        "v_ldexp_f64 v[26:27], v[26:27], v72\n\t" \
        "v_ldexp_f64 v[28:29], v[28:29], v72\n\t" \
        "v_ldexp_f64 v[30:31], v[30:31], v72\n\t" \
        "v_add3_u32 v78, v78, v80, s27\n\t" \
        "v_max_u32 v81, v33, v35\n\t" \
        "v_max3_u32 v81, v37, v39, v81\n\t" \
        "v_lshrrev_b32 v81, 20, v81\n\t" \
        "v_sub_u32 v72, 0x3fe, v81\n\t" \
        "v_ldexp_f64 v[32:33], v[32:33], v72\n\t" \
        "v_ldexp_f64 v[34:35], v[34:35], v72\n\t" \
        "v_ldexp_f64 v[36:37], v[36:37], v72\n\t" \
        "v_ldexp_f64 v[38:39], v[38:39], v72\n\t" \
        "v_add3_u32 v79, v79, v81, s27\n\t" \
        "s_movrels_b64 s[22:23], s[68:69]\n\t" \
        "s_addk_i32 m0, 0x2\n\t" \
        "s_or_b32 s24, s26, s22\n\t" \
        "s_setpc_b64 s[24:25]\n\t" \
        ".p2align 9\n" \
        "s_waitcnt lgkmcnt(0)\n\t" \
        "v_mul_f64 v[40:41], s[36:37], v[24:25]\n\t" \
        "v_mul_f64 v[48:49], s[36:37], v[32:33]\n\t" \
        "v_mul_f64 v[42:43], s[38:39], v[24:25]\n\t" \
        "v_mul_f64 v[50:51], s[38:39], v[32:33]\n\t" \
        "v_mul_f64 v[44:45], s[40:41], v[24:25]\n\t" \
        "v_mul_f64 v[52:53], s[40:41], v[32:33]\n\t" \
        "v_mul_f64 v[46:47], s[42:43], v[24:25]\n\t" \
        "v_mul_f64 v[54:55], s[42:43], v[32:33]\n\t" \
        "v_fma_f64 v[40:41], s[44:45], v[26:27], v[40:41]\n\t" \
        "v_fma_f64 v[48:49], s[44:45], v[34:35], v[48:49]\n\t" \
        "v_fma_f64 v[42:43], s[46:47], v[26:27], v[42:43]\n\t" \
        "v_fma_f64 v[50:51], s[46:47], v[34:35], v[50:51]\n\t" \
        "v_fma_f64 v[44:45], s[48:49], v[26:27], v[44:45]\n\t" \
        "v_fma_f64 v[52:53], s[48:49], v[34:35], v[52:53]\n\t" \
        "v_fma_f64 v[46:47], s[50:51], v[26:27], v[46:47]\n\t" \
        "v_fma_f64 v[54:55], s[50:51], v[34:35], v[54:55]\n\t" \
        "v_fma_f64 v[40:41], s[52:53], v[28:29], v[40:41]\n\t" \
        "v_fma_f64 v[48:49], s[52:53], v[36:37], v[48:49]\n\t" \
        "v_fma_f64 v[42:43], s[54:55], v[28:29], v[42:43]\n\t" \
        "v_fma_f64 v[50:51], s[54:55], v[36:37], v[50:51]\n\t" \
        "v_fma_f64 v[44:45], s[56:57], v[28:29], v[44:45]\n\t" \
        "v_fma_f64 v[52:53], s[56:57], v[36:37], v[52:53]\n\t" \
        "v_fma_f64 v[46:47], s[58:59], v[28:29], v[46:47]\n\t" \
        "v_fma_f64 v[54:55], s[58:59], v[36:37], v[54:55]\n\t" \
        "v_fma_f64 v[24:25], s[60:61], v[30:31], v[40:41]\n\t" \
        "v_fma_f64 v[32:33], s[60:61], v[38:39], v[48:49]\n\t" \
        "v_fma_f64 v[26:27], s[62:63], v[30:31], v[42:43]\n\t" \
        "v_fma_f64 v[34:35], s[62:63], v[38:39], v[50:51]\n\t" \
        "v_fma_f64 v[28:29], s[64:65], v[30:31], v[44:45]\n\t" \
        "v_fma_f64 v[36:37], s[64:65], v[38:39], v[52:53]\n\t" \
        "v_fma_f64 v[30:31], s[66:67], v[30:31], v[46:47]\n\t" \
        "v_fma_f64 v[38:39], s[66:67], v[38:39], v[54:55]\n\t" \
        "s_add_u32 s30, s30, 0x80\n\t" \
        "s_addc_u32 s31, s31, 0\n\t" \
        "s_load_dwordx16 s[36:51], s[30:31], 0x0\n\t" \
        "s_load_dwordx16 s[52:67], s[30:31], 0x40\n\t" \
        "v_mul_f64 v[24:25], v[24:25], v[114:115]\n\t" \
        "v_mul_f64 v[32:33], v[32:33], v[122:123]\n\t" \
        "v_mul_f64 v[26:27], v[26:27], v[116:117]\n\t" \
        "v_mul_f64 v[34:35], v[34:35], v[124:125]\n\t" \
        "v_mul_f64 v[28:29], v[28:29], v[118:119]\n\t" \
        "v_mul_f64 v[36:37], v[36:37], v[126:127]\n\t" \
        "v_mul_f64 v[30:31], v[30:31], v[120:121]\n\t" \
        "v_mul_f64 v[38:39], v[38:39], v[128:129]\n\t" \
        "v_max_u32 v80, v25, v27\n\t" \
        "v_max3_u32 v80, v29, v31, v80\n\t" \
        "v_lshrrev_b32 v80, 20, v80\n\t" \
        "v_sub_u32 v72, 0x3fe, v80\n\t" \
        "v_ldexp_f64 v[24:25], v[24:25], v72\n\t" \
        "v_ldexp_f64 v[26:27], v[26:27], v72\n\t" \
        "v_ldexp_f64 v[28:29], v[28:29], v72\n\t" \
        "v_ldexp_f64 v[30:31], v[30:31], v72\n\t" \
        "v_add3_u32 v78, v78, v80, s27\n\t" \
        "v_max_u32 v81, v33, v35\n\t" \
        "v_max3_u32 v81, v37, v39, v81\n\t" \
        "v_lshrrev_b32 v81, 20, v81\n\t" \
        "v_sub_u32 v72, 0x3fe, v81\n\t" \
        "v_ldexp_f64 v[32:33], v[32:33], v72\n\t" \
        "v_ldexp_f64 v[34:35], v[34:35], v72\n\t" \
        "v_ldexp_f64 v[36:37], v[36:37], v72\n\t" \
        "v_ldexp_f64 v[38:39], v[38:39], v72\n\t" \
        "v_add3_u32 v79, v79, v81, s27\n\t" \
        "s_movrels_b64 s[22:23], s[68:69]\n\t" \
        "s_addk_i32 m0, 0x2\n\t" \
        "s_or_b32 s24, s26, s22\n\t" \
        "s_setpc_b64 s[24:25]\n\t" \
        ".p2align 9\n" \
        "s_waitcnt lgkmcnt(0)\n\t" \
        "v_mov_b64 v[114:115], v[130:131]\n\t" \
        "v_mov_b64 v[122:123], v[138:139]\n\t" \
        "v_mov_b64 v[116:117], v[132:133]\n\t" \
        "v_mov_b64 v[124:125], v[140:141]\n\t" \
        "v_mov_b64 v[118:119], v[134:135]\n\t" \
        "v_mov_b64 v[126:127], v[142:143]\n\t" \
        "v_mov_b64 v[120:121], v[136:137]\n\t" \
        "v_mov_b64 v[128:129], v[144:145]\n\t" \
        "s_lshr_b32 s28, s23, 16\n\t" \
        "v_bfe_u32 v72, v74, s23, 8\n\t" \
        "v_bfe_u32 v73, v75, s23, 8\n\t" \
        "v_add_lshl_u32 v72, v72, s28, 5\n\t" \
        "v_add_lshl_u32 v73, v73, s28, 5\n\t" \
        "ds_read_b128 v[130:133], v72\n\t" \
        "ds_read_b128 v[134:137], v72 offset:16\n\t" \
        "ds_read_b128 v[138:141], v73\n\t" \
        "ds_read_b128 v[142:145], v73 offset:16\n\t" \
        "s_movrels_b64 s[22:23], s[68:69]\n\t" \
        "s_addk_i32 m0, 0x2\n\t" \
        "s_or_b32 s24, s26, s22\n\t" \
        "s_setpc_b64 s[24:25]\n\t" \
        ".p2align 9\n" \
        ".Ldone_%=:\n" \
        "s_waitcnt vmcnt(0) lgkmcnt(0)\n\t" \
        "v_mul_f64 v[40:41], %[w0], v[24:25]\n\t" \
        "v_fma_f64 v[40:41], %[w1], v[26:27], v[40:41]\n\t" \
        "v_fma_f64 v[40:41], %[w2], v[28:29], v[40:41]\n\t" \
        "v_fma_f64 v[40:41], %[w3], v[30:31], v[40:41]\n\t" \
        "v_mul_f64 v[48:49], %[w0], v[32:33]\n\t" \
        "v_fma_f64 v[48:49], %[w1], v[34:35], v[48:49]\n\t" \
        "v_fma_f64 v[48:49], %[w2], v[36:37], v[48:49]\n\t" \
        "v_fma_f64 v[48:49], %[w3], v[38:39], v[48:49]\n\t" \
        "v_mov_b32 %[al], v40\n\t" \
        "v_mov_b32 %[ah], v41\n\t" \
        "v_mov_b32 %[bl], v48\n\t" \
        "v_mov_b32 %[bh], v49\n\t" \
        "v_mov_b32 %[ea], v78\n\t" \
        "v_mov_b32 %[eb], v79\n\t" \
        "s_nop 1\n\t" \
        ""

#endif
```

### phyly_amd/csrc/plk_fused4_v4s.h

```cpp
#ifndef PLK_FUSED4_V4S_H
#define PLK_FUSED4_V4S_H

#include "plk_fused4_v4s_asm.h"
#include "plk_fused4_v4p_asm.h"

struct FusedV4SArgs {
    FusedPTArgs pt;
    const unsigned *stream;
    int chunks;
    unsigned first_y;
    int sync;
    unsigned first_y1, first_b1;
    int groups, cg;
    double *part_sum;
    int *part_exp;
};
#define PLK_V4S_NO_TERM INT_MIN

__global__ __launch_bounds__(256) void k_build_code_stream(const uint8_t *__restrict__ codes, long Spad, long nunits,
                                                           const int *__restrict__ obs_row, int nobs, const int *__restrict__ row_nodes ,
                                                           int nrows, int nchar, int chunks, const uint8_t *__restrict__ luts, unsigned *__restrict__ out)
{
    const size_t idx = (size_t)blockIdx.x * 256 + threadIdx.x, total = (size_t)nunits * chunks * PLK_V4S_UNIT;
    if (idx >= total) return;
    const int half = (int)(idx & 1), lane = (int)((idx >> 1) & 63);
    const size_t uc = idx >> 7, unit = uc / (size_t)chunks;
    const int chunk = (int)(uc - unit * (size_t)chunks);
    const size_t site = unit * PLK_V4S_UNIT + (size_t)half * 64 + lane;
    out[plk_stream_dword(unit, chunk, lane, half, chunks)] =
        site < (size_t)Spad ? plk_stream_site_dword(codes, (size_t)Spad, site, obs_row, nobs, row_nodes, nrows, nchar, chunk, 5, luts) : 0u;
}

template <bool HELD, bool PAIR>
__device__ __forceinline__ void fused_run_program_v4s(double &lha, double &lhb, int &ea, int &eb, const void *ops, const void *mstream,
                                                       const void *strm, unsigned voff, unsigned y0,
                                                       double w0, double w1, double w2, double w3,
                                                       unsigned long long c0, unsigned long long c1, unsigned long long c2,
                                                       unsigned y1, unsigned b1)
{
    int al, ah, bl, bh;
#ifdef PLK_EXP_EMPTY
    al = bl = 0; ah = bh = 0x3ff00000; ea = eb = 0;
#else
    static_assert(HELD || !PAIR, "the pair-product text has the held prologue only");
    if constexpr (PAIR)
        asm volatile(PLK_V4P_PROGRAM_HELD
                     : [al] "=v"(al), [ah] "=v"(ah), [bl] "=v"(bl), [bh] "=v"(bh), [ea] "=v"(ea), [eb] "=v"(eb)
                     : [voff] "v"(voff), [ops] "s"(ops), [mstream] "s"(mstream), [strm] "s"(strm), [y0] "s"(y0), [y1] "s"(y1), [b1] "s"(b1),
                       [w0] "s"(w0), [w1] "s"(w1), [w2] "s"(w2), [w3] "s"(w3), [c0] "v"(c0), [c1] "v"(c1), [c2] "v"(c2)
                     : PLK_V4S_CLOBBERS);
    else if constexpr (HELD)
        asm volatile(PLK_V4S_PROGRAM_HELD
                     : [al] "=v"(al), [ah] "=v"(ah), [bl] "=v"(bl), [bh] "=v"(bh), [ea] "=v"(ea), [eb] "=v"(eb)
                     : [voff] "v"(voff), [ops] "s"(ops), [mstream] "s"(mstream), [strm] "s"(strm), [y0] "s"(y0),
                       [w0] "s"(w0), [w1] "s"(w1), [w2] "s"(w2), [w3] "s"(w3), [c0] "v"(c0), [c1] "v"(c1), [c2] "v"(c2)
                     : PLK_V4S_CLOBBERS);
    else
        asm volatile(PLK_V4S_PROGRAM
                     : [al] "=v"(al), [ah] "=v"(ah), [bl] "=v"(bl), [bh] "=v"(bh), [ea] "=v"(ea), [eb] "=v"(eb)
                     : [voff] "v"(voff), [ops] "s"(ops), [mstream] "s"(mstream), [strm] "s"(strm), [y0] "s"(y0),
                       [w0] "s"(w0), [w1] "s"(w1), [w2] "s"(w2), [w3] "s"(w3)
                     : PLK_V4S_CLOBBERS);
#endif
    lha = __hiloint2double(ah, al);
    lhb = __hiloint2double(bh, bl);
}

template <int THREADS, bool HELD = false, bool PAIR = false, bool GROUPS = false>
__global__ __launch_bounds__(THREADS) void k_ll_fused4_v4s(FusedV4SArgs va)
{
    constexpr int NW = THREADS / 64;
    const FusedPTArgs &aa = va.pt;
    const FusedArgs &a = aa.f;
    extern __shared__ double lds_dyn[];
    const int tip_doubles = a.ntips * a.nchar * 4;
    const int tid = threadIdx.x;
    const int lane = tid & 63, wave = __builtin_amdgcn_readfirstlane(tid >> 6);
    const PLK_AS4 double *prior = as_uniform(a.cat_prior);
    const PLK_AS4 double *rootw = as_uniform(a.root_w);
    const bool plain = a.root_mode == PLK_ROOT_NONE || a.root_mode == PLK_ROOT_UNIFORM;
    const double wu = a.root_mode == PLK_ROOT_NONE ? 1.0 : 0.25;
    const double rw0 = plain ? wu : rootw[0], rw1 = plain ? wu : rootw[1], rw2 = plain ? wu : rootw[2], rw3 = plain ? wu : rootw[3];
    const long nunits = (a.S + PLK_V4S_UNIT - 1) / PLK_V4S_UNIT;
    const unsigned cat32 = (unsigned)(a.ntips * a.nchar);
    dd acc = dd_make(0.0, 0.0);
    const long stride = (long)gridDim.x * NW, passes = (nunits + stride - 1) / stride;
    const int ngroups = GROUPS ? va.groups : 1;
    for (int g = 0; g < ngroups; g++) {
        const int c_lo = GROUPS ? g * va.cg : 0, c_hi = GROUPS ? min(a.C, c_lo + va.cg) : a.C;
        if (GROUPS && g > 0) __syncthreads();
        {
            const double2 *src = reinterpret_cast<const double2 *>(a.tip) + (size_t)c_lo * (tip_doubles / 2);
            double2 *dst = reinterpret_cast<double2 *>(lds_dyn);
            const int n2 = (c_hi - c_lo) * (tip_doubles / 2);
            int first = tid;
            if (GROUPS) {
                int l;
                asm volatile("v_mbcnt_lo_u32_b32 %0, -1, 0\n\tv_mbcnt_hi_u32_b32 %0, -1, %0" : "=v"(l));
                first = wave * 64 + l;
            }
            for (int i0 = first; i0 < n2; i0 += 4 * THREADS) {
                double2 v[4];
#pragma unroll
                for (int u = 0; u < 4; u++) v[u] = i0 + u * THREADS < n2 ? src[i0 + u * THREADS] : double2{0.0, 0.0};
#pragma unroll
                for (int u = 0; u < 4; u++) if (i0 + u * THREADS < n2) dst[i0 + u * THREADS] = v[u];
            }
        }
        __syncthreads();
        unsigned long long c0 = 0, c1 = 0, c2 = 0;
        auto request = [&](long unit) {
            unsigned off = (unsigned)lane * 8u;
            asm volatile("" : "+v"(off));
            const char *p = reinterpret_cast<const char *>(va.stream + (size_t)unit * (size_t)va.chunks * PLK_V4S_UNIT) + off;
            c0 = *reinterpret_cast<const unsigned long long *>(p);
            c1 = *reinterpret_cast<const unsigned long long *>(p + PLK_V4S_CHUNK_BYTES);
            c2 = *reinterpret_cast<const unsigned long long *>(p + 2 * PLK_V4S_CHUNK_BYTES);
        };
        if (HELD && (long)blockIdx.x * NW + wave < nunits) request((long)blockIdx.x * NW + wave);
        for (long pass = 0; pass < passes; pass++) {
            const long u = pass * stride + (long)blockIdx.x * NW + wave;
            const bool active = u < nunits;
            const unsigned *strm = va.stream + (size_t)(active ? u : 0) * (size_t)va.chunks * PLK_V4S_UNIT;
            double sum[2] = {0.0, 0.0};
            int Eexp[2] = {0, 0};
            bool have[2] = {false, false};
            if (GROUPS && g > 0 && active) {
#pragma unroll
                for (int j = 0; j < 2; j++) {
                    const size_t s = (size_t)u * PLK_V4S_UNIT + j * 64 + lane;
                    sum[j] = va.part_sum[s]; Eexp[j] = va.part_exp[s];
                    have[j] = Eexp[j] != PLK_V4S_NO_TERM;
                }
            }
            if (va.sync & 1) __syncthreads();
            for (int c = c_lo; c < c_hi; c++) {
                const double *ps = a.PS + (size_t)c * (a.nmat + 1) * 16;
                const unsigned *ops = aa.words + (size_t)c * aa.nwords;
                if (va.sync & 2) __syncthreads();
                if (!active) continue;
                if (aa.warm) {
                    fused_touch_lines(ps, (unsigned)(a.nmat + 1) * 128u, (unsigned)wave * 64u, NW * 64u);
                    fused_touch_lines(ops, (unsigned)aa.nwords * 4u, (unsigned)wave * 64u, NW * 64u);
                }
                double lhs[2];
                int esc[2];
                fused_run_program_v4s<HELD, PAIR>(lhs[0], lhs[1], esc[0], esc[1], ops, ps, strm, (unsigned)lane * 8u, va.first_y + (unsigned)(c - c_lo) * cat32,
                                                  rw0, rw1, rw2, rw3, c0, c1, c2, va.first_y1 + (unsigned)(c - c_lo) * cat32, va.first_b1);
#pragma unroll
                for (int j = 0; j < 2; j++) {
                    const double lh = lhs[j];
                    const double term = prior[c] * lh;
                    if (term != 0.0) {
                        if (!have[j]) { sum[j] = term; Eexp[j] = esc[j]; have[j] = true; }
                        else if (esc[j] > Eexp[j]) { sum[j] = ldexp(sum[j], Eexp[j] - esc[j]) + term; Eexp[j] = esc[j]; }
                        else sum[j] += ldexp(term, esc[j] - Eexp[j]);
                    }
                }
            }
            if (HELD && u + stride < nunits) request(u + stride);
            if (GROUPS && g + 1 < ngroups) {
                if (active) {
#pragma unroll
                    for (int j = 0; j < 2; j++) {
                        const size_t s = (size_t)u * PLK_V4S_UNIT + j * 64 + lane;
                        va.part_sum[s] = sum[j]; va.part_exp[s] = have[j] ? Eexp[j] : PLK_V4S_NO_TERM;
                    }
                }
                continue;
            }
#pragma unroll
            for (int j = 0; j < 2; j++) {
                const long s = u * PLK_V4S_UNIT + j * 64 + lane;
                const double ll = have[j] ? log(sum[j]) + (double)Eexp[j] * 0.6931471805599453094 : -INFINITY;
                if (active && s < a.S) {
                    if (a.site_ll) a.site_ll[s] = ll;
                    acc = dd_add(acc, dd_weighted(a.w, s, ll));
                }
            }
        }
    }
    if (a.partial) {
        const dd r = dd_wave_sum(acc);
        if (lane == 0) a.partial[(size_t)blockIdx.x * NW + wave] = r;
    }
}

#endif
```

### phyly_amd/csrc/plk_fused4_v4s_asm.h

```cpp
#ifndef PLK_FUSED4_V4S_ASM_H
#define PLK_FUSED4_V4S_ASM_H

#define PLK_V4S_ADVANCE 34
#define PLK_V4S_CHUNK_BYTES 512
#define PLK_V4S_FOLD_ADV 36
#define PLK_V4S_FOLD_SCALE 60

#define PLK_V4S_PROLOGUE \
        "v_mov_b32 v24, 0\n\t" \
        "v_mov_b32 v25, 0x3ff00000\n\t" \
        "v_mov_b32 v32, 0\n\t" \
        "v_mov_b32 v33, 0x3ff00000\n\t" \
        "v_mov_b32 v26, 0\n\t" \
        "v_mov_b32 v27, 0x3ff00000\n\t" \
        "v_mov_b32 v34, 0\n\t" \
        "v_mov_b32 v35, 0x3ff00000\n\t" \
        "v_mov_b32 v28, 0\n\t" \
        "v_mov_b32 v29, 0x3ff00000\n\t" \
        "v_mov_b32 v36, 0\n\t" \
        "v_mov_b32 v37, 0x3ff00000\n\t" \
        "v_mov_b32 v30, 0\n\t" \
        "v_mov_b32 v31, 0x3ff00000\n\t" \
        "v_mov_b32 v38, 0\n\t" \
        "v_mov_b32 v39, 0x3ff00000\n\t" \
        "s_waitcnt vmcnt(0)\n\t" \
        "v_mov_b32 v76, %[voff]\n\t" \
        "s_mov_b64 s[34:35], %[strm]\n\t" \
        "global_load_dwordx2 v[74:75], v76, s[34:35]\n\t" \
        "global_load_dwordx2 v[146:147], v76, s[34:35] offset:512\n\t" \
        "global_load_dwordx2 v[148:149], v76, s[34:35] offset:1024\n\t" \
        "s_add_u32 s34, s34, 0x600\n\t" \
        "s_addc_u32 s35, s35, 0\n\t" \
        "v_mov_b32 v78, 0\n\t" \
        "v_mov_b32 v79, 0\n\t" \
        "s_mov_b64 s[20:21], %[ops]\n\t" \
        "s_mov_b64 s[30:31], %[mstream]\n\t" \
        "s_movk_i32 s27, 0xfc02\n\t" \
        "s_mov_b32 m0, 0\n\t" \
        "s_load_dwordx16 s[68:83], s[20:21], 0x0\n\t" \
        "s_load_dwordx16 s[84:99], s[20:21], 0x40\n\t" \
        "s_add_u32 s20, s20, 0x80\n\t" \
        "s_addc_u32 s21, s21, 0\n\t" \
        "s_load_dwordx16 s[36:51], s[30:31], 0x0\n\t" \
        "s_load_dwordx16 s[52:67], s[30:31], 0x40\n\t" \
        "s_getpc_b64 s[24:25]\n\t" \
        ".Lpcref_%=:\n" \
        "s_add_u32 s26, s24, .Lh0_%=-.Lpcref_%=\n\t" \
        "s_addc_u32 s25, s25, 0\n\t" \
        "s_waitcnt vmcnt(2)\n\t" \
        "v_bfe_u32 v72, v74, 0, 8\n\t" \
        "v_bfe_u32 v73, v75, 0, 8\n\t" \
        "v_add_lshl_u32 v72, v72, %[y0], 5\n\t" \
        "v_add_lshl_u32 v73, v73, %[y0], 5\n\t" \
        "ds_read_b128 v[56:59], v72\n\t" \
        "ds_read_b128 v[60:63], v72 offset:16\n\t" \
        "ds_read_b128 v[64:67], v73\n\t" \
        "ds_read_b128 v[68:71], v73 offset:16\n\t" \
        "s_waitcnt lgkmcnt(0)\n\t" \
        "s_movrels_b64 s[22:23], s[68:69]\n\t" \
        "s_addk_i32 m0, 0x2\n\t" \
        "s_or_b32 s24, s26, s22\n\t" \
        "s_setpc_b64 s[24:25]\n\t" \
        ""

#define PLK_V4S_PROLOGUE_HELD \
        "v_mov_b32 v24, 0\n\t" \
        "v_mov_b32 v25, 0x3ff00000\n\t" \
        "v_mov_b32 v32, 0\n\t" \
        "v_mov_b32 v33, 0x3ff00000\n\t" \
        "v_mov_b32 v26, 0\n\t" \
        "v_mov_b32 v27, 0x3ff00000\n\t" \
        "v_mov_b32 v34, 0\n\t" \
        "v_mov_b32 v35, 0x3ff00000\n\t" \
        "v_mov_b32 v28, 0\n\t" \
        "v_mov_b32 v29, 0x3ff00000\n\t" \
        "v_mov_b32 v36, 0\n\t" \
        "v_mov_b32 v37, 0x3ff00000\n\t" \
        "v_mov_b32 v30, 0\n\t" \
        "v_mov_b32 v31, 0x3ff00000\n\t" \
        "v_mov_b32 v38, 0\n\t" \
        "v_mov_b32 v39, 0x3ff00000\n\t" \
        "v_mov_b32 v76, %[voff]\n\t" \
        "s_mov_b64 s[34:35], %[strm]\n\t" \
        "v_mov_b64 v[74:75], %[c0]\n\t" \
        "v_mov_b64 v[146:147], %[c1]\n\t" \
        "v_mov_b64 v[148:149], %[c2]\n\t" \
        "s_add_u32 s34, s34, 0x600\n\t" \
        "s_addc_u32 s35, s35, 0\n\t" \
        "v_mov_b32 v78, 0\n\t" \
        "v_mov_b32 v79, 0\n\t" \
        "s_mov_b64 s[20:21], %[ops]\n\t" \
        "s_mov_b64 s[30:31], %[mstream]\n\t" \
        "s_movk_i32 s27, 0xfc02\n\t" \
        "s_mov_b32 m0, 0\n\t" \
        "s_load_dwordx16 s[68:83], s[20:21], 0x0\n\t" \
        "s_load_dwordx16 s[84:99], s[20:21], 0x40\n\t" \
        "s_add_u32 s20, s20, 0x80\n\t" \
        "s_addc_u32 s21, s21, 0\n\t" \
        "s_load_dwordx16 s[36:51], s[30:31], 0x0\n\t" \
        "s_load_dwordx16 s[52:67], s[30:31], 0x40\n\t" \
        "s_getpc_b64 s[24:25]\n\t" \
        ".Lpcref_%=:\n" \
        "s_add_u32 s26, s24, .Lh0_%=-.Lpcref_%=\n\t" \
        "s_addc_u32 s25, s25, 0\n\t" \
        "v_bfe_u32 v72, v74, 0, 8\n\t" \
        "v_bfe_u32 v73, v75, 0, 8\n\t" \
        "v_add_lshl_u32 v72, v72, %[y0], 5\n\t" \
        "v_add_lshl_u32 v73, v73, %[y0], 5\n\t" \
        "ds_read_b128 v[56:59], v72\n\t" \
        "ds_read_b128 v[60:63], v72 offset:16\n\t" \
        "ds_read_b128 v[64:67], v73\n\t" \
        "ds_read_b128 v[68:71], v73 offset:16\n\t" \
        "s_waitcnt lgkmcnt(0)\n\t" \
        "s_movrels_b64 s[22:23], s[68:69]\n\t" \
        "s_addk_i32 m0, 0x2\n\t" \
        "s_or_b32 s24, s26, s22\n\t" \
        "s_setpc_b64 s[24:25]\n\t" \
        ""

#define PLK_V4S_TABLE \
        ".p2align 15\n" \
        ".Lh0_%=:\n" \
        "s_waitcnt lgkmcnt(0)\n\t" \
        "v_mov_b64 v[24:25], v[56:57]\n\t" \
        "v_mov_b64 v[32:33], v[64:65]\n\t" \
        "v_mov_b64 v[26:27], v[58:59]\n\t" \
        "v_mov_b64 v[34:35], v[66:67]\n\t" \
        "v_mov_b64 v[28:29], v[60:61]\n\t" \
        "v_mov_b64 v[36:37], v[68:69]\n\t" \
        "v_mov_b64 v[30:31], v[62:63]\n\t" \
        "v_mov_b64 v[38:39], v[70:71]\n\t" \
        "s_lshr_b32 s28, s23, 16\n\t" \
        "v_bfe_u32 v72, v74, s23, 8\n\t" \
        "v_bfe_u32 v73, v75, s23, 8\n\t" \
        "v_add_lshl_u32 v72, v72, s28, 5\n\t" \
        "v_add_lshl_u32 v73, v73, s28, 5\n\t" \
        "ds_read_b128 v[56:59], v72\n\t" \
        "ds_read_b128 v[60:63], v72 offset:16\n\t" \
        "ds_read_b128 v[64:67], v73\n\t" \
        "ds_read_b128 v[68:71], v73 offset:16\n\t" \
        "s_movrels_b64 s[22:23], s[68:69]\n\t" \
        "s_addk_i32 m0, 0x2\n\t" \
        "s_or_b32 s24, s26, s22\n\t" \
        "s_setpc_b64 s[24:25]\n\t" \
        ".p2align 9\n" \
        "s_waitcnt lgkmcnt(0)\n\t" \
        "v_mul_f64 v[24:25], v[24:25], v[56:57]\n\t" \
        "v_mul_f64 v[32:33], v[32:33], v[64:65]\n\t" \
        "v_mul_f64 v[26:27], v[26:27], v[58:59]\n\t" \
        "v_mul_f64 v[34:35], v[34:35], v[66:67]\n\t" \
        "v_mul_f64 v[28:29], v[28:29], v[60:61]\n\t" \
        "v_mul_f64 v[36:37], v[36:37], v[68:69]\n\t" \
        "v_mul_f64 v[30:31], v[30:31], v[62:63]\n\t" \
        "v_mul_f64 v[38:39], v[38:39], v[70:71]\n\t" \
        "s_lshr_b32 s28, s23, 16\n\t" \
        "v_bfe_u32 v72, v74, s23, 8\n\t" \
        "v_bfe_u32 v73, v75, s23, 8\n\t" \
        "v_add_lshl_u32 v72, v72, s28, 5\n\t" \
        "v_add_lshl_u32 v73, v73, s28, 5\n\t" \
        "ds_read_b128 v[56:59], v72\n\t" \
        "ds_read_b128 v[60:63], v72 offset:16\n\t" \
        "ds_read_b128 v[64:67], v73\n\t" \
        "ds_read_b128 v[68:71], v73 offset:16\n\t" \
        "s_movrels_b64 s[22:23], s[68:69]\n\t" \
        "s_addk_i32 m0, 0x2\n\t" \
        "s_or_b32 s24, s26, s22\n\t" \
        "s_setpc_b64 s[24:25]\n\t" \
        ".p2align 9\n" \
        "s_waitcnt lgkmcnt(0)\n\t" \
        "v_mul_f64 v[40:41], s[36:37], v[24:25]\n\t" \
        "v_mul_f64 v[48:49], s[36:37], v[32:33]\n\t" \
        "v_mul_f64 v[42:43], s[38:39], v[24:25]\n\t" \
        "v_mul_f64 v[50:51], s[38:39], v[32:33]\n\t" \
        "v_mul_f64 v[44:45], s[40:41], v[24:25]\n\t" \
        "v_mul_f64 v[52:53], s[40:41], v[32:33]\n\t" \
        "v_mul_f64 v[46:47], s[42:43], v[24:25]\n\t" \
        "v_mul_f64 v[54:55], s[42:43], v[32:33]\n\t" \
        "v_fma_f64 v[40:41], s[44:45], v[26:27], v[40:41]\n\t" \
        "v_fma_f64 v[48:49], s[44:45], v[34:35], v[48:49]\n\t" \
        "v_fma_f64 v[42:43], s[46:47], v[26:27], v[42:43]\n\t" \
        "v_fma_f64 v[50:51], s[46:47], v[34:35], v[50:51]\n\t" \
        "v_fma_f64 v[44:45], s[48:49], v[26:27], v[44:45]\n\t" \
        "v_fma_f64 v[52:53], s[48:49], v[34:35], v[52:53]\n\t" \
        "v_fma_f64 v[46:47], s[50:51], v[26:27], v[46:47]\n\t" \
        "v_fma_f64 v[54:55], s[50:51], v[34:35], v[54:55]\n\t" \
        "v_fma_f64 v[40:41], s[52:53], v[28:29], v[40:41]\n\t" \
        "v_fma_f64 v[48:49], s[52:53], v[36:37], v[48:49]\n\t" \
        "v_fma_f64 v[42:43], s[54:55], v[28:29], v[42:43]\n\t" \
        "v_fma_f64 v[50:51], s[54:55], v[36:37], v[50:51]\n\t" \
        "v_fma_f64 v[44:45], s[56:57], v[28:29], v[44:45]\n\t" \
        "v_fma_f64 v[52:53], s[56:57], v[36:37], v[52:53]\n\t" \
        "v_fma_f64 v[46:47], s[58:59], v[28:29], v[46:47]\n\t" \
        "v_fma_f64 v[54:55], s[58:59], v[36:37], v[54:55]\n\t" \
        "v_fma_f64 v[24:25], s[60:61], v[30:31], v[40:41]\n\t" \
        "v_fma_f64 v[32:33], s[60:61], v[38:39], v[48:49]\n\t" \
        "v_fma_f64 v[26:27], s[62:63], v[30:31], v[42:43]\n\t" \
        "v_fma_f64 v[34:35], s[62:63], v[38:39], v[50:51]\n\t" \
        "v_fma_f64 v[28:29], s[64:65], v[30:31], v[44:45]\n\t" \
        "v_fma_f64 v[36:37], s[64:65], v[38:39], v[52:53]\n\t" \
        "v_fma_f64 v[30:31], s[66:67], v[30:31], v[46:47]\n\t" \
        "v_fma_f64 v[38:39], s[66:67], v[38:39], v[54:55]\n\t" \
        "s_add_u32 s30, s30, 0x80\n\t" \
        "s_addc_u32 s31, s31, 0\n\t" \
        "s_load_dwordx16 s[36:51], s[30:31], 0x0\n\t" \
        "s_load_dwordx16 s[52:67], s[30:31], 0x40\n\t" \
        "s_movrels_b64 s[22:23], s[68:69]\n\t" \
        "s_addk_i32 m0, 0x2\n\t" \
        "s_or_b32 s24, s26, s22\n\t" \
        "s_setpc_b64 s[24:25]\n\t" \
        ".p2align 9\n" \
        "v_mul_f64 v[24:25], v[24:25], v[56:57]\n\t" \
        "v_mul_f64 v[32:33], v[32:33], v[64:65]\n\t" \
        "v_mul_f64 v[26:27], v[26:27], v[58:59]\n\t" \
        "v_mul_f64 v[34:35], v[34:35], v[66:67]\n\t" \
        "v_mul_f64 v[28:29], v[28:29], v[60:61]\n\t" \
        "v_mul_f64 v[36:37], v[36:37], v[68:69]\n\t" \
        "v_mul_f64 v[30:31], v[30:31], v[62:63]\n\t" \
        "v_mul_f64 v[38:39], v[38:39], v[70:71]\n\t" \
        "s_lshr_b32 s28, s23, 16\n\t" \
        "v_bfe_u32 v72, v74, s23, 8\n\t" \
        "v_bfe_u32 v73, v75, s23, 8\n\t" \
        "v_add_lshl_u32 v72, v72, s28, 5\n\t" \
        "v_add_lshl_u32 v73, v73, s28, 5\n\t" \
        "ds_read_b128 v[56:59], v72\n\t" \
        "ds_read_b128 v[60:63], v72 offset:16\n\t" \
        "ds_read_b128 v[64:67], v73\n\t" \
        "ds_read_b128 v[68:71], v73 offset:16\n\t" \
        "s_movrels_b64 s[22:23], s[68:69]\n\t" \
        "s_addk_i32 m0, 0x2\n\t" \
        "s_or_b32 s24, s26, s22\n\t" \
        "s_setpc_b64 s[24:25]\n\t" \
        ".p2align 9\n" \
        "s_waitcnt lgkmcnt(0)\n\t" \
        "v_mul_f64 v[40:41], s[36:37], v[24:25]\n\t" \
        "v_mul_f64 v[48:49], s[36:37], v[32:33]\n\t" \
        "v_mul_f64 v[42:43], s[38:39], v[24:25]\n\t" \
        "v_mul_f64 v[50:51], s[38:39], v[32:33]\n\t" \
        "v_mul_f64 v[44:45], s[40:41], v[24:25]\n\t" \
        "v_mul_f64 v[52:53], s[40:41], v[32:33]\n\t" \
        "v_mul_f64 v[46:47], s[42:43], v[24:25]\n\t" \
        "v_mul_f64 v[54:55], s[42:43], v[32:33]\n\t" \
        "v_fma_f64 v[40:41], s[44:45], v[26:27], v[40:41]\n\t" \
        "v_fma_f64 v[48:49], s[44:45], v[34:35], v[48:49]\n\t" \
        "v_fma_f64 v[42:43], s[46:47], v[26:27], v[42:43]\n\t" \
        "v_fma_f64 v[50:51], s[46:47], v[34:35], v[50:51]\n\t" \
        "v_fma_f64 v[44:45], s[48:49], v[26:27], v[44:45]\n\t" \
        "v_fma_f64 v[52:53], s[48:49], v[34:35], v[52:53]\n\t" \
        "v_fma_f64 v[46:47], s[50:51], v[26:27], v[46:47]\n\t" \
        "v_fma_f64 v[54:55], s[50:51], v[34:35], v[54:55]\n\t" \
        "v_fma_f64 v[40:41], s[52:53], v[28:29], v[40:41]\n\t" \
        "v_fma_f64 v[48:49], s[52:53], v[36:37], v[48:49]\n\t" \
        "v_fma_f64 v[42:43], s[54:55], v[28:29], v[42:43]\n\t" \
        "v_fma_f64 v[50:51], s[54:55], v[36:37], v[50:51]\n\t" \
        "v_fma_f64 v[44:45], s[56:57], v[28:29], v[44:45]\n\t" \
        "v_fma_f64 v[52:53], s[56:57], v[36:37], v[52:53]\n\t" \
        "v_fma_f64 v[46:47], s[58:59], v[28:29], v[46:47]\n\t" \
        "v_fma_f64 v[54:55], s[58:59], v[36:37], v[54:55]\n\t" \
        "v_fma_f64 v[24:25], s[60:61], v[30:31], v[40:41]\n\t" \
        "v_fma_f64 v[32:33], s[60:61], v[38:39], v[48:49]\n\t" \
        "v_fma_f64 v[26:27], s[62:63], v[30:31], v[42:43]\n\t" \
        "v_fma_f64 v[34:35], s[62:63], v[38:39], v[50:51]\n\t" \
// ... 1614 lines not shown
        "v_ldexp_f64 v[30:31], v[30:31], v72\n\t" \
        "v_add3_u32 v78, v78, v80, s27\n\t" \
        "v_max_u32 v81, v33, v35\n\t" \
        "v_max3_u32 v81, v37, v39, v81\n\t" \
        "v_lshrrev_b32 v81, 20, v81\n\t" \
        "v_sub_u32 v72, 0x3fe, v81\n\t" \
        "v_ldexp_f64 v[32:33], v[32:33], v72\n\t" \
        "v_ldexp_f64 v[34:35], v[34:35], v72\n\t" \
        "v_ldexp_f64 v[36:37], v[36:37], v72\n\t" \
        "v_ldexp_f64 v[38:39], v[38:39], v72\n\t" \
        "v_add3_u32 v79, v79, v81, s27\n\t" \
        "s_movrels_b64 s[22:23], s[68:69]\n\t" \
        "s_addk_i32 m0, 0x2\n\t" \
        "s_or_b32 s24, s26, s22\n\t" \
        "s_setpc_b64 s[24:25]\n\t" \
        ".p2align 9\n" \
        "s_waitcnt lgkmcnt(0)\n\t" \
        "v_mul_f64 v[40:41], s[36:37], v[24:25]\n\t" \
        "v_mul_f64 v[48:49], s[36:37], v[32:33]\n\t" \
        "v_mul_f64 v[42:43], s[38:39], v[24:25]\n\t" \
        "v_mul_f64 v[50:51], s[38:39], v[32:33]\n\t" \
        "v_mul_f64 v[44:45], s[40:41], v[24:25]\n\t" \
        "v_mul_f64 v[52:53], s[40:41], v[32:33]\n\t" \
        "v_mul_f64 v[46:47], s[42:43], v[24:25]\n\t" \
        "v_mul_f64 v[54:55], s[42:43], v[32:33]\n\t" \
        "v_fma_f64 v[40:41], s[44:45], v[26:27], v[40:41]\n\t" \
        "v_fma_f64 v[48:49], s[44:45], v[34:35], v[48:49]\n\t" \
        "v_fma_f64 v[42:43], s[46:47], v[26:27], v[42:43]\n\t" \
        "v_fma_f64 v[50:51], s[46:47], v[34:35], v[50:51]\n\t" \
        "v_fma_f64 v[44:45], s[48:49], v[26:27], v[44:45]\n\t" \
        "v_fma_f64 v[52:53], s[48:49], v[34:35], v[52:53]\n\t" \
        "v_fma_f64 v[46:47], s[50:51], v[26:27], v[46:47]\n\t" \
        "v_fma_f64 v[54:55], s[50:51], v[34:35], v[54:55]\n\t" \
        "v_fma_f64 v[40:41], s[52:53], v[28:29], v[40:41]\n\t" \
        "v_fma_f64 v[48:49], s[52:53], v[36:37], v[48:49]\n\t" \
        "v_fma_f64 v[42:43], s[54:55], v[28:29], v[42:43]\n\t" \
        "v_fma_f64 v[50:51], s[54:55], v[36:37], v[50:51]\n\t" \
        "v_fma_f64 v[44:45], s[56:57], v[28:29], v[44:45]\n\t" \
        "v_fma_f64 v[52:53], s[56:57], v[36:37], v[52:53]\n\t" \
        "v_fma_f64 v[46:47], s[58:59], v[28:29], v[46:47]\n\t" \
        "v_fma_f64 v[54:55], s[58:59], v[36:37], v[54:55]\n\t" \
        "v_fma_f64 v[24:25], s[60:61], v[30:31], v[40:41]\n\t" \
        "v_fma_f64 v[32:33], s[60:61], v[38:39], v[48:49]\n\t" \
        "v_fma_f64 v[26:27], s[62:63], v[30:31], v[42:43]\n\t" \
        "v_fma_f64 v[34:35], s[62:63], v[38:39], v[50:51]\n\t" \
        "v_fma_f64 v[28:29], s[64:65], v[30:31], v[44:45]\n\t" \
        "v_fma_f64 v[36:37], s[64:65], v[38:39], v[52:53]\n\t" \
        "v_fma_f64 v[30:31], s[66:67], v[30:31], v[46:47]\n\t" \
        "v_fma_f64 v[38:39], s[66:67], v[38:39], v[54:55]\n\t" \
        "s_add_u32 s30, s30, 0x80\n\t" \
        "s_addc_u32 s31, s31, 0\n\t" \
        "s_load_dwordx16 s[36:51], s[30:31], 0x0\n\t" \
        "s_load_dwordx16 s[52:67], s[30:31], 0x40\n\t" \
        "v_mul_f64 v[24:25], v[24:25], v[114:115]\n\t" \
        "v_mul_f64 v[32:33], v[32:33], v[122:123]\n\t" \
        "v_mul_f64 v[26:27], v[26:27], v[116:117]\n\t" \
        "v_mul_f64 v[34:35], v[34:35], v[124:125]\n\t" \
        "v_mul_f64 v[28:29], v[28:29], v[118:119]\n\t" \
        "v_mul_f64 v[36:37], v[36:37], v[126:127]\n\t" \
        "v_mul_f64 v[30:31], v[30:31], v[120:121]\n\t" \
        "v_mul_f64 v[38:39], v[38:39], v[128:129]\n\t" \
        "v_max_u32 v80, v25, v27\n\t" \
        "v_max3_u32 v80, v29, v31, v80\n\t" \
        "v_lshrrev_b32 v80, 20, v80\n\t" \
        "v_sub_u32 v72, 0x3fe, v80\n\t" \
        "v_ldexp_f64 v[24:25], v[24:25], v72\n\t" \
        "v_ldexp_f64 v[26:27], v[26:27], v72\n\t" \
        "v_ldexp_f64 v[28:29], v[28:29], v72\n\t" \
        "v_ldexp_f64 v[30:31], v[30:31], v72\n\t" \
        "v_add3_u32 v78, v78, v80, s27\n\t" \
        "v_max_u32 v81, v33, v35\n\t" \
        "v_max3_u32 v81, v37, v39, v81\n\t" \
        "v_lshrrev_b32 v81, 20, v81\n\t" \
        "v_sub_u32 v72, 0x3fe, v81\n\t" \
        "v_ldexp_f64 v[32:33], v[32:33], v72\n\t" \
        "v_ldexp_f64 v[34:35], v[34:35], v72\n\t" \
        "v_ldexp_f64 v[36:37], v[36:37], v72\n\t" \
        "v_ldexp_f64 v[38:39], v[38:39], v72\n\t" \
        "v_add3_u32 v79, v79, v81, s27\n\t" \
        "s_movrels_b64 s[22:23], s[68:69]\n\t" \
        "s_addk_i32 m0, 0x2\n\t" \
        "s_or_b32 s24, s26, s22\n\t" \
        "s_setpc_b64 s[24:25]\n\t" \
        ".p2align 9\n" \
        "s_waitcnt lgkmcnt(0)\n\t" \
        "v_mul_f64 v[40:41], s[36:37], v[24:25]\n\t" \
        "v_mul_f64 v[48:49], s[36:37], v[32:33]\n\t" \
        "v_mul_f64 v[42:43], s[38:39], v[24:25]\n\t" \
        "v_mul_f64 v[50:51], s[38:39], v[32:33]\n\t" \
        "v_mul_f64 v[44:45], s[40:41], v[24:25]\n\t" \
        "v_mul_f64 v[52:53], s[40:41], v[32:33]\n\t" \
        "v_mul_f64 v[46:47], s[42:43], v[24:25]\n\t" \
        "v_mul_f64 v[54:55], s[42:43], v[32:33]\n\t" \
        "v_fma_f64 v[40:41], s[44:45], v[26:27], v[40:41]\n\t" \
        "v_fma_f64 v[48:49], s[44:45], v[34:35], v[48:49]\n\t" \
        "v_fma_f64 v[42:43], s[46:47], v[26:27], v[42:43]\n\t" \
        "v_fma_f64 v[50:51], s[46:47], v[34:35], v[50:51]\n\t" \
        "v_fma_f64 v[44:45], s[48:49], v[26:27], v[44:45]\n\t" \
        "v_fma_f64 v[52:53], s[48:49], v[34:35], v[52:53]\n\t" \
        "v_fma_f64 v[46:47], s[50:51], v[26:27], v[46:47]\n\t" \
        "v_fma_f64 v[54:55], s[50:51], v[34:35], v[54:55]\n\t" \
        "v_fma_f64 v[40:41], s[52:53], v[28:29], v[40:41]\n\t" \
        "v_fma_f64 v[48:49], s[52:53], v[36:37], v[48:49]\n\t" \
        "v_fma_f64 v[42:43], s[54:55], v[28:29], v[42:43]\n\t" \
        "v_fma_f64 v[50:51], s[54:55], v[36:37], v[50:51]\n\t" \
        "v_fma_f64 v[44:45], s[56:57], v[28:29], v[44:45]\n\t" \
        "v_fma_f64 v[52:53], s[56:57], v[36:37], v[52:53]\n\t" \
        "v_fma_f64 v[46:47], s[58:59], v[28:29], v[46:47]\n\t" \
        "v_fma_f64 v[54:55], s[58:59], v[36:37], v[54:55]\n\t" \
        "v_fma_f64 v[24:25], s[60:61], v[30:31], v[40:41]\n\t" \
        "v_fma_f64 v[32:33], s[60:61], v[38:39], v[48:49]\n\t" \
        "v_fma_f64 v[26:27], s[62:63], v[30:31], v[42:43]\n\t" \
        "v_fma_f64 v[34:35], s[62:63], v[38:39], v[50:51]\n\t" \
        "v_fma_f64 v[28:29], s[64:65], v[30:31], v[44:45]\n\t" \
        "v_fma_f64 v[36:37], s[64:65], v[38:39], v[52:53]\n\t" \
        "v_fma_f64 v[30:31], s[66:67], v[30:31], v[46:47]\n\t" \
        "v_fma_f64 v[38:39], s[66:67], v[38:39], v[54:55]\n\t" \
        "s_add_u32 s30, s30, 0x80\n\t" \
        "s_addc_u32 s31, s31, 0\n\t" \
        "s_load_dwordx16 s[36:51], s[30:31], 0x0\n\t" \
        "s_load_dwordx16 s[52:67], s[30:31], 0x40\n\t" \
        "v_mul_f64 v[24:25], v[24:25], v[130:131]\n\t" \
        "v_mul_f64 v[32:33], v[32:33], v[138:139]\n\t" \
        "v_mul_f64 v[26:27], v[26:27], v[132:133]\n\t" \
        "v_mul_f64 v[34:35], v[34:35], v[140:141]\n\t" \
        "v_mul_f64 v[28:29], v[28:29], v[134:135]\n\t" \
        "v_mul_f64 v[36:37], v[36:37], v[142:143]\n\t" \
        "v_mul_f64 v[30:31], v[30:31], v[136:137]\n\t" \
        "v_mul_f64 v[38:39], v[38:39], v[144:145]\n\t" \
        "v_max_u32 v80, v25, v27\n\t" \
        "v_max3_u32 v80, v29, v31, v80\n\t" \
        "v_lshrrev_b32 v80, 20, v80\n\t" \
        "v_sub_u32 v72, 0x3fe, v80\n\t" \
        "v_ldexp_f64 v[24:25], v[24:25], v72\n\t" \
        "v_ldexp_f64 v[26:27], v[26:27], v72\n\t" \
        "v_ldexp_f64 v[28:29], v[28:29], v72\n\t" \
        "v_ldexp_f64 v[30:31], v[30:31], v72\n\t" \
        "v_add3_u32 v78, v78, v80, s27\n\t" \
        "v_max_u32 v81, v33, v35\n\t" \
        "v_max3_u32 v81, v37, v39, v81\n\t" \
        "v_lshrrev_b32 v81, 20, v81\n\t" \
        "v_sub_u32 v72, 0x3fe, v81\n\t" \
        "v_ldexp_f64 v[32:33], v[32:33], v72\n\t" \
        "v_ldexp_f64 v[34:35], v[34:35], v72\n\t" \
        "v_ldexp_f64 v[36:37], v[36:37], v72\n\t" \
        "v_ldexp_f64 v[38:39], v[38:39], v72\n\t" \
        "v_add3_u32 v79, v79, v81, s27\n\t" \
        "s_movrels_b64 s[22:23], s[68:69]\n\t" \
        "s_addk_i32 m0, 0x2\n\t" \
        "s_or_b32 s24, s26, s22\n\t" \
        "s_setpc_b64 s[24:25]\n\t" \
        ".p2align 9\n" \
        ".Ldone_%=:\n" \
        "s_waitcnt vmcnt(0) lgkmcnt(0)\n\t" \
        "v_mul_f64 v[40:41], %[w0], v[24:25]\n\t" \
        "v_fma_f64 v[40:41], %[w1], v[26:27], v[40:41]\n\t" \
        "v_fma_f64 v[40:41], %[w2], v[28:29], v[40:41]\n\t" \
        "v_fma_f64 v[40:41], %[w3], v[30:31], v[40:41]\n\t" \
        "v_mul_f64 v[48:49], %[w0], v[32:33]\n\t" \
        "v_fma_f64 v[48:49], %[w1], v[34:35], v[48:49]\n\t" \
        "v_fma_f64 v[48:49], %[w2], v[36:37], v[48:49]\n\t" \
        "v_fma_f64 v[48:49], %[w3], v[38:39], v[48:49]\n\t" \
        "v_mov_b32 %[al], v40\n\t" \
        "v_mov_b32 %[ah], v41\n\t" \
        "v_mov_b32 %[bl], v48\n\t" \
        "v_mov_b32 %[bh], v49\n\t" \
        "v_mov_b32 %[ea], v78\n\t" \
        "v_mov_b32 %[eb], v79\n\t" \
        "s_nop 1\n\t" \
        ""

#define PLK_V4S_PROGRAM PLK_V4S_PROLOGUE PLK_V4S_TABLE
#define PLK_V4S_PROGRAM_HELD PLK_V4S_PROLOGUE_HELD PLK_V4S_TABLE

#define PLK_V4S_CLOBBERS "memory", "scc", "vcc", \
        "v24", "v25", "v26", "v27", "v28", "v29", "v30", "v31", "v32", "v33", "v34", "v35", "v36", "v37", "v38", "v39", "v40", "v41", "v42", "v43", "v44", "v45", "v46", "v47", "v48", "v49", "v50", "v51", "v52", "v53", "v54", "v55", "v56", "v57", "v58", "v59", "v60", "v61", "v62", "v63", "v64", "v65", "v66", "v67", "v68", "v69", "v70", "v71", "v72", "v73", "v74", "v75", "v76", "v77", "v78", "v79", "v80", "v81", "v82", "v83", "v84", "v85", "v86", "v87", "v88", "v89", "v90", "v91", "v92", "v93", "v94", "v95", "v96", "v97", "v98", "v99", "v100", "v101", "v102", "v103", "v104", "v105", "v106", "v107", "v108", "v109", "v110", "v111", "v112", "v113", "v114", "v115", "v116", "v117", "v118", "v119", "v120", "v121", "v122", "v123", "v124", "v125", "v126", "v127", "v128", "v129", "v130", "v131", "v132", "v133", "v134", "v135", "v136", "v137", "v138", "v139", "v140", "v141", "v142", "v143", "v144", "v145", "v146", "v147", "v148", "v149", \
        "s20", "s21", "s22", "s23", "s24", "s25", "s26", "s27", "s28", "s29", "s30", "s31", "s32", "s33", "s34", "s35", "s36", "s37", "s38", "s39", "s40", "s41", "s42", "s43", "s44", "s45", "s46", "s47", "s48", "s49", "s50", "s51", "s52", "s53", "s54", "s55", "s56", "s57", "s58", "s59", "s60", "s61", "s62", "s63", "s64", "s65", "s66", "s67", "s68", "s69", "s70", "s71", "s72", "s73", "s74", "s75", "s76", "s77", "s78", "s79", "s80", "s81", "s82", "s83", "s84", "s85", "s86", "s87", "s88", "s89", "s90", "s91", "s92", "s93", "s94", "s95", "s96", "s97", "s98", "s99", "m0"

#endif
```

### phyly_amd/csrc/plk_program.h

```cpp
#ifndef PLK_PROGRAM_H
#define PLK_PROGRAM_H

#include <algorithm>
#include <climits>
#include <cmath>
#include <cstdint>
#include <cstdio>
#include <string>
#include <vector>

enum {
    OP_TIP_SET = 0,
    OP_TIP_MUL = 1,
    OP_MATVEC = 2,
    OP_PUSH = 3,
    OP_POPMUL = 4,
    OP_NODE_MUL = 5,
    OP_SCALE = 6,
    OP_END = 7
};
#define PLK_WORD_TIPMUL_NOWAIT 3u
#define PLK_WORD_SET_POPMUL 12u
#define PLK_WORD_SET_PUSH 20u
#define PLK_WORD_MATVEC_TIPMUL 4u

struct plk_op2 { int x, y; };
struct plk_op4 { int x, y, z, w; };

#define PLK_TILE 256
#define PLK_FUSED_SLOTS 16
#define PLK_LDS_LIMIT (150 * 1024)

struct PlkProgram {
    std::vector<plk_op2> ops;
    std::vector<int> op_edge;
    std::vector<int> tip_edge;
    std::vector<char> scale_node;
    std::vector<char> mid_scale_node;
    int mid_scales = 0;
    int wide_node = -1;
    std::vector<char> op_mid;
    std::vector<int> obs_nodes;
    int slots_needed = 0;
};

#define PLK_SCALE_RUN 32

static inline void plk_program_build(int N, const int *ip, const int *ix, const int *preorder,
                                     const char *node_has_data, PlkProgram &pg)
{
    std::vector<int> need(N, 0), since(N, 0);
    pg.scale_node.assign(N, 0);
    pg.mid_scale_node.assign(N, 0);
    pg.mid_scales = 0; pg.wide_node = -1;
    std::vector<std::vector<int>> ichild(N);
    for (int u = N - 1; u >= 0; u--) {
        const int a = preorder[u];
        if (ip[a + 1] == ip[a]) continue;
        std::vector<int> &ic = ichild[a];
        for (int idx = ip[a]; idx < ip[a + 1]; idx++)
            if (ip[ix[idx] + 1] > ip[ix[idx]]) ic.push_back(idx);
        std::stable_sort(ic.begin(), ic.end(), [&](int x, int y) { return need[ix[x]] > need[ix[y]]; });
        int nd = 0;
        for (size_t i = 0; i < ic.size(); i++) nd = std::max(nd, need[ix[ic[i]]] + (i > 0 ? 1 : 0));
        need[a] = nd;
        int acc = 0;
        auto merge = [&](int add) { if (acc + add > PLK_SCALE_RUN) { acc = 0; pg.mid_scale_node[a] = 1; } acc += add; };
        if (!ic.empty()) merge(since[ix[ic[0]]] + 1);
        for (int idx = ip[a]; idx < ip[a + 1]; idx++) if (ip[ix[idx] + 1] == ip[ix[idx]]) merge(1);
        for (size_t i = 1; i < ic.size(); i++) merge(since[ix[ic[i]]] + 1);
        if (pg.mid_scale_node[a]) pg.mid_scales++;
        if (acc >= 16 || pg.mid_scale_node[a]) { pg.scale_node[a] = 1; acc = 0; }
        since[a] = acc;
    }
    const int root = preorder[0];
    pg.slots_needed = need[root];

    pg.ops.clear(); pg.op_edge.clear(); pg.tip_edge.clear(); pg.obs_nodes.clear(); pg.op_mid.clear();
    std::vector<int> obs_row(N, -1);
    auto obs = [&](int node) {
        if (obs_row[node] < 0) { obs_row[node] = (int)pg.obs_nodes.size(); pg.obs_nodes.push_back(node); }
        return obs_row[node];
    };
    auto emit = [&](int code, int tslot, int arg, int edge) {
        plk_op2 o; o.x = code | (tslot << 8); o.y = arg;
        pg.ops.push_back(o); pg.op_edge.push_back(edge); pg.op_mid.push_back(0);
    };
    struct Frame { int a, depth, stage; bool started; int run; };
    std::vector<Frame> stk;
    stk.push_back({root, 0, 0, false, 0});
    auto mid_scale = [&](Frame &f, int add) {
        if (f.run + add > PLK_SCALE_RUN) {
            emit(OP_SCALE, 0, f.a, -1);
            pg.op_mid.back() = 1;
            f.run = 0;
            if (pg.wide_node < 0) pg.wide_node = f.a;
        }
        f.run += add;
    };
    while (!stk.empty()) {
        Frame &f = stk.back();
        const int a = f.a;
        const std::vector<int> &ic = ichild[a];
        if (f.stage == 0) {
            f.stage = 1;
            if (!ic.empty()) { const Frame nf = {ix[ic[0]], f.depth, 0, false, 0}; stk.push_back(nf); continue; }
        }
        if (f.stage == 1) {
            if (!ic.empty()) { emit(OP_MATVEC, 0, 0, ic[0]); f.started = true; f.run = since[ix[ic[0]]] + 1; }
            for (int idx = ip[a]; idx < ip[a + 1]; idx++) {
                const int b = ix[idx];
                if (ip[b + 1] > ip[b]) continue;
                const int t = (int)pg.tip_edge.size();
                pg.tip_edge.push_back(idx);
                mid_scale(f, 1);
                emit(f.started ? OP_TIP_MUL : OP_TIP_SET, t, b, idx);
                obs(b);
                f.started = true;
            }
            f.stage = 2;
        }
        if (f.stage >= 2) {
            const int i = f.stage - 1;
            if (f.stage > 2) {
                emit(OP_MATVEC, 0, 0, ic[i - 1]);
                emit(OP_POPMUL, 0, f.depth, -1);
            }
            if (i < (int)ic.size()) {
                mid_scale(f, since[ix[ic[i]]] + 1);
                emit(OP_PUSH, 0, f.depth, -1);
                f.stage++;
                const Frame nf = {ix[ic[i]], f.depth + 1, 0, false, 0};
                stk.push_back(nf);
                continue;
            }
            if (node_has_data[a]) { emit(OP_NODE_MUL, 0, a, -1); obs(a); }
            if (pg.scale_node[a]) emit(OP_SCALE, 0, a, -1);
            stk.pop_back();
        }
    }
}

static inline std::string plk_fmt(const char *fmt, long a = 0, long b = 0, long c = 0)
{
    char buf[256];
    snprintf(buf, sizeof buf, fmt, a, b, c);
    return std::string(buf);
}

static inline std::string plk_program_check(int N, const int *ip, const int *ix, const int *preorder,
                                            const char *node_has_data, const PlkProgram &pg)
{
    const int E = N - 1;
    const int nops = (int)pg.ops.size();
    if ((int)pg.op_edge.size() != nops || (int)pg.op_mid.size() != nops) return "program: op_edge size";
    if ((int)pg.scale_node.size() != N || (int)pg.mid_scale_node.size() != N) return "program: scale_node size";
    if (pg.slots_needed < 0) return "program: negative stack depth";
    std::vector<int> edge_seen(std::max(E, 1), 0), tip_seen(pg.tip_edge.size(), 0);
// ... 1927 lines not shown
            cur_row = f.z;
            oi++;
        } else if (code == OP_MATVEC) {
            if (f.w != mi || fu.mat_edge[mi] != pg.op_edge[pc]) return "fused program: matrix index mismatch";
            mi++;
        } else if (code == OP_PUSH || code == OP_POPMUL) {
            if (f.y < 0 || f.y >= D) return "fused program: stack slot out of range";
        }
    }
    for (size_t pc = nops; pc < fu.fops.size(); pc++) if ((fu.fops[pc].x & 0xff) != OP_END) return "fused program: padding is not END";
    return "";
}


enum PlkK4Variant { PLK_K4_NONE = 0, PLK_K4_CPP, PLK_K4_ASM, PLK_K4_ASM_PT, PLK_K4_V4, PLK_K4_V4S };
enum { PLK_K4_LDS_V4S_768 = 0, PLK_K4_LDS_V4_768, PLK_K4_LDS_V4_512 };

struct PlkPairTablesOpt { bool on; int mode, warm, sync , fold, held, pair, triple, groups, quad; };
static inline PlkPairTablesOpt plk_pair_tables_opt(long v)
{
    const int quad = (v & (2048 | 32768)) ? 0 : (v & 16384) ? 2 : (v & 1024) ? 0 : 1;
    return {v != 0, (int)(v & 7), (v & 8) ? 0 : 1, (v & 32) ? 0 : (v & 16) ? 1 : (v & 65536) ? 2 : -1, (v & (64 | 256)) ? 0 : 1, (v & (64 | 128)) ? 0 : 1,
            (v & (64 | 128 | 256 | 512)) ? 0 : 1, (v & 2048) ? 0 : (v & 1024) || quad == 2 ? 2 : 1,
            (v & (4096 | 8192)) == (4096 | 8192) ? 2 : (v & 4096) ? 1 : (v & 8192) ? -1 : 0, quad};
}

#define PLK_V4S_SCALAR_CACHE_BYTES (16 * 1024)
static inline int plk_v4s_auto_sync(int Cg, size_t nmat, size_t nwords)
{
    return Cg == 1 && (nmat + 1) * 128 + nwords * 4 <= (size_t)PLK_V4S_SCALAR_CACHE_BYTES ? 0 : 2;
}

struct PlkK4Shape {
    int nchar, C;
    long S;
    int num_cus;
    long pair_tables, fused_asm, sites_per_lane;
    size_t static_lds[3];
    const int *node_codes = nullptr;
};

struct PlkK4Choice {
    PlkK4Variant variant = PLK_K4_NONE;
    int tile = 0;
    int NS = 1, D = 4, pack4 = 0;
    int block = 0;
    size_t lds = 0;
    unsigned tip_base = 0;
    int warm = 1, sync = 2;
    bool sync_auto = false;
    int fold = 1, held = 1;
    int pair = 0;
    PlkV4TPlan triple;
    std::string bad;
};

static inline PlkK4Choice plk_k4_choose(int N, const int *ip, const int *ix, const PlkProgram &pg, const PlkK4Shape &sh, bool allow_stream,
                                        PlkFused &fu, PlkFusedPT &fpt, PlkFusedV4 &fv4, PlkFusedV4S &fv4s)
{
    PlkK4Choice ch;
    const int nchar = sh.nchar;
    const int NS = sh.sites_per_lane == 2 && pg.slots_needed <= 8 ? 2 : 1, pack4 = nchar <= 16 ? 1 : 0;
    const size_t lds_asm = plk_fused_lds_bytes(pg, nchar, pack4 ? PLK_TILE / 2 : PLK_TILE), lds_cpp = plk_fused_lds_bytes(pg, nchar, PLK_TILE * NS);
    const bool asm_fits = NS == 1 && plk_fused_asm_ok(pg) && sh.fused_asm && lds_asm <= PLK_LDS_LIMIT;
    if (pg.slots_needed > PLK_FUSED_SLOTS || (!asm_fits && lds_cpp > PLK_LDS_LIMIT)) return ch;
    const PlkPairTablesOpt po = plk_pair_tables_opt(sh.pair_tables);
    ch.warm = po.warm; ch.sync = po.sync < 0 ? 2 : po.sync; ch.sync_auto = po.sync < 0; ch.fold = po.fold; ch.held = po.held;
    if (po.on && sh.fused_asm && sh.sites_per_lane != 2 && pg.slots_needed <= 4 && nchar <= 16 && !pg.obs_nodes.empty()) {
        if ((po.mode == 1 || po.mode == 7) && sh.S > 0 && allow_stream) {
            plk_fused_pt_build(N, ip, ix, pg, nchar, INT_MAX, fpt, true);
            const size_t lds = plk_fused_v4s_lds_bytes(fpt, nchar, sh.C), st = sh.static_lds[PLK_K4_LDS_V4S_768];
            bool any_obs = false;
            for (const PlkFusedPT::VOp &o : fpt.vops) if (o.code == OP_TIP_SET || o.code == OP_TIP_MUL) any_obs = true;
            if (any_obs && lds + st <= plk_pt_lds_limit(1024) && (st + lds) / 32 < 65536 && fpt.units < 2048 && fpt.row_node.size() < 65536) {
                ch.variant = PLK_K4_V4S; ch.tile = 1536; ch.NS = 2; ch.block = 768; ch.lds = lds; ch.tip_base = (unsigned)st;
                ch.pair = po.pair && pg.slots_needed <= PLK_V4P_STACK_SLOTS;
                plk_fused_v4s_words(fpt, nchar, sh.C, ch.tip_base, fv4s);
                ch.bad = plk_fused_check_pt(N, ip, ix, pg, fpt, nchar, 1, 0, true, false);
                if (ch.bad.empty()) ch.bad = plk_fused_check_v4s(fpt, fv4s, nchar, sh.C, ch.tip_base, lds);
                if (ch.bad.empty())
                    ch.triple = plk_v4t_plan(fpt, nchar, sh.C, sh.S, sh.num_cus, st, po.triple, ch.pair && ch.fold && ch.held ? po.groups : 1, po.quad, sh.node_codes);
                return ch;
            }
        }
        struct Cand { PlkK4Variant variant; int tile; };
        std::vector<Cand> cands;
        switch (po.mode) {
        case 2: cands = {{PLK_K4_ASM_PT, 1024}}; break;
        case 3: cands = {{PLK_K4_ASM_PT, 512}}; break;
        case 5: cands = {{PLK_K4_V4, 1024}}; break;
        case 6: cands = {{PLK_K4_V4, 1536}}; break;
        default: {
            auto rounds = [&](long tile) { const long nt = (sh.S + tile - 1) / tile; return (double)((nt + sh.num_cus - 1) / sh.num_cus); };
            if (sh.S > 0 && rounds(1024) * 1.0 < rounds(1536) * 1.3) cands = {{PLK_K4_V4, 1024}, {PLK_K4_V4, 1536}, {PLK_K4_ASM_PT, 1024}, {PLK_K4_ASM_PT, 512}};
            else cands = {{PLK_K4_V4, 1536}, {PLK_K4_V4, 1024}, {PLK_K4_ASM_PT, 1024}, {PLK_K4_ASM_PT, 512}};
            break;
        }
        }
        for (const Cand &cd : cands) {
            const bool v4 = cd.variant == PLK_K4_V4;
            const long limit = (long)plk_pt_lds_limit(cd.tile);
            int max_pairs = INT_MAX;
            for (int attempt = 0; attempt < 3; attempt++) {
                plk_fused_pt_build(N, ip, ix, pg, nchar, max_pairs, fpt, v4);
                const long bytes = (long)plk_fused_pt_lds_bytes(fpt, nchar, cd.tile);
                if (bytes <= limit && fpt.units < 2048 && fpt.row_node.size() < 65536) {
                    ch.variant = cd.variant; ch.tile = cd.tile; ch.NS = v4 ? 2 : 1; ch.block = v4 ? cd.tile / 2 : cd.tile; ch.lds = (size_t)bytes;
                    ch.bad = plk_fused_check_pt(N, ip, ix, pg, fpt, nchar, cd.tile, ch.lds, v4);
                    if (v4) {
                        ch.tip_base = (unsigned)sh.static_lds[cd.tile == 1536 ? PLK_K4_LDS_V4_768 : PLK_K4_LDS_V4_512];
                        plk_fused_v4_words(fpt, nchar, cd.tile, ch.tip_base, fv4);
                        if (ch.bad.empty()) ch.bad = plk_fused_check_v4(fpt, fv4, nchar, cd.tile, ch.tip_base, ch.lds);
                    }
                    return ch;
                }
                if (fpt.npairs == 0) break;
                const long per_pair = (long)(nchar - 2) * nchar * 32 - cd.tile;
                if (per_pair <= 0) break;
                const long drop = (bytes - limit + per_pair - 1) / per_pair;
                max_pairs = drop >= fpt.npairs ? 0 : fpt.npairs - (int)drop;
            }
        }
    }
    plk_fused_build(N, pg, fu);
    ch.tile = PLK_TILE * NS; ch.NS = NS; ch.block = PLK_TILE;
    ch.D = pg.slots_needed <= 4 ? 4 : (pg.slots_needed <= 8 ? 8 : 16);
    if (asm_fits) {
        ch.variant = PLK_K4_ASM; ch.pack4 = pack4; ch.lds = lds_asm;
        ch.bad = plk_fused_check_asm(N, pg, fu, nchar, ch.D, pack4, lds_asm);
    } else {
        ch.variant = PLK_K4_CPP; ch.lds = lds_cpp;
        ch.bad = plk_fused_check_cpp(N, pg, fu, nchar, ch.D, NS, lds_cpp);
    }
    return ch;
}

struct PlkK4StreamCaps { bool held = true, pair = true, groups = true, partial_sums = true; };

struct PlkK4Stream {
    PlkFusedV4S fv4s;
    PlkFusedV4SFold fold; PlkFusedV4P pair;
    enum Words { CHECKED, FOLDED, PAIR } runs = CHECKED;
    bool held = false;
    PlkV4TPlan triple;
    size_t lds = 0;
    int sync = 2; bool sync_auto = false;
    long info_fold = 0, info_pairmul = 0, info_triple = 0, info_quad = 0;
    std::string note;
    const std::vector<unsigned> &words() const { return runs == PAIR ? pair.words : runs == FOLDED ? fold.words : fv4s.words; }
    size_t stride() const { return runs == PAIR ? pair.stride : runs == FOLDED ? fold.stride : fv4s.stride; }
    int Cg(int C) const { return triple.nodes + triple.quads > 0 && triple.Cg > 0 ? triple.Cg : C; }
};

static inline bool plk_k4_stream_can_group(const PlkK4Choice &ch, const PlkK4StreamCaps &caps) { return ch.pair && ch.fold && ch.held && caps.held && caps.pair && caps.groups; }

static inline void plk_k4_stream_fold_pair(PlkK4Stream &r, bool fold, bool pair, bool pair_kept = false)
{
    r.runs = PlkK4Stream::CHECKED; r.info_fold = r.held ? 2 : 0; r.info_pairmul = 0;
    if (fold) {
        plk_fused_v4s_fold(r.fv4s, r.fold);
        const std::string bad = plk_fused_check_v4s_fold(r.fv4s, r.fold);
        if (bad.empty()) {
            r.runs = PlkK4Stream::FOLDED;
            r.info_fold |= 1 | (long)(r.fold.scale_slots & 15) << 4 | (long)std::min(r.fold.standalone_scale, 255) << 8 |
                           (long)std::min(r.fold.nadv[0], 255) << 16 | (long)std::min(r.fold.nadv[1], 127) << 24;
        } else r.note = "internal: " + bad + " (the unfolded op stream runs)";
    }
    if (!pair || r.runs != PlkK4Stream::FOLDED || !r.held) return;
    if (!pair_kept) plk_fused_v4p_build(r.fv4s, r.pair);
    if (r.pair.words.empty()) return;
    const std::string bad = pair_kept ? "" : plk_fused_check_v4p(r.fv4s, r.pair);
    if (bad.empty()) { r.runs = PlkK4Stream::PAIR; r.info_pairmul = 1 | (long)std::min(r.pair.npair, 65535) << 8; }
    else r.note = "internal: " + bad + " (the folded op stream runs)";
}

static inline PlkK4Stream plk_k4_stream(int N, const int *ip, const int *ix, const PlkProgram &pg, const PlkK4Shape &sh, const PlkK4Choice &ch,
                                        const PlkK4StreamCaps &caps, PlkFusedPT &fpt, PlkFusedV4S fv4s)
{
    PlkK4Stream r;
    r.fv4s = std::move(fv4s); r.held = ch.held && caps.held; r.lds = ch.lds; r.sync = ch.sync; r.sync_auto = ch.sync_auto;
    const PlkPairTablesOpt po = plk_pair_tables_opt(sh.pair_tables);
    PlkV4TPlan tp = ch.triple;
    auto one_group = [&]() { return plk_v4t_plan(fpt, sh.nchar, sh.C, sh.S, sh.num_cus, ch.tip_base, po.triple, 1, po.quad, sh.node_codes); };
    if (tp.groups > 1 && !plk_k4_stream_can_group(ch, caps)) tp = one_group();
    if (tp.nodes + tp.quads > 0 && tp.groups > 1 && !caps.partial_sums) tp = one_group();
    bool pair_kept = false;
    for (int attempt = 0; attempt < 2 && tp.nodes + tp.quads > 0; attempt++) {
        PlkFusedPT fpt_t; PlkFusedV4S fv4s_t;
        std::string bad;
        if (tp.quads > 0) {
            plk_fused_v4q_build(fpt, pg.slots_needed, sh.nchar, sh.node_codes, tp.tri_at, tp.quad_at, tp.quad_shape, true, fpt_t);
            bad = plk_fused_check_v4q(N, ip, ix, fpt, fpt_t, sh.nchar, sh.node_codes);
            if (bad.empty() && fpt_t.nquads != tp.quads) bad = "v4q program: the builder took another number of four-leaf nodes than the plan";
        } else {
            plk_fused_v4t_build(fpt, pg.slots_needed, sh.nchar, tp.extra_bytes, true, fpt_t);
            bad = plk_fused_check_v4t(N, ip, ix, fpt, fpt_t, sh.nchar);
        }
        const size_t lds = plk_fused_v4s_lds_bytes(fpt_t, sh.nchar, tp.Cg);
        if (bad.empty() && fpt_t.ntriples != tp.nodes) bad = "v4t program: the builder took another number of nodes than the plan";
        if (bad.empty()) {
            plk_fused_v4s_words(fpt_t, sh.nchar, sh.C, ch.tip_base, fv4s_t, tp.Cg);
            bad = plk_fused_check_v4s(fpt_t, fv4s_t, sh.nchar, sh.C, ch.tip_base, lds);
        }
        if (bad.empty() && fv4s_t.chunks > r.fv4s.chunks) bad = "v4t program: more chunks than the checked stream";
        if (bad.empty() && tp.groups > 1) {
            plk_fused_v4p_build(fv4s_t, r.pair);
            if (r.pair.words.empty() || !plk_fused_check_v4p(fv4s_t, r.pair).empty()) { tp = one_group(); continue; }
            pair_kept = true;
        }
        if (bad.empty()) {
            fpt = std::move(fpt_t); r.fv4s = std::move(fv4s_t); r.lds = lds; r.triple = tp;
            r.info_triple = 1 | (long)std::min(tp.groups, 15) << 4 | (long)std::min(tp.nodes, 65535) << 8;
            r.info_quad = tp.quads > 0 ? 1 | (long)std::min(tp.quads, 65535) << 8 : 0;
        } else r.note = "internal: " + bad + (tp.quads > 0 ? " (the stream without four-leaf and three-leaf tables runs)" : " (the stream without three-leaf tables runs)");
        break;
    }
    plk_k4_stream_fold_pair(r, ch.fold != 0, ch.pair && caps.pair, pair_kept);
    if (r.sync_auto) r.sync = plk_v4s_auto_sync(r.Cg(sh.C), fpt.mat_edge.size(), r.stride());
    return r;
}


struct PlkStorageMaps {
    std::vector<int> edge_tip;
    std::vector<int> edge_int;
    std::vector<int> node_int;
    std::vector<int> node_scale;
    std::vector<int> tip_edges;
    int ntips = 0, nie = 0, nin = 0, nsc = 0;
};

static inline void plk_storage_maps_build(int N, int E, const int *indptr, const std::vector<int> &tip_edge, const char *scale_node,
                                          PlkStorageMaps &m)
{
    m.ntips = (int)tip_edge.size();
    m.edge_tip.assign(E, -1); m.edge_int.assign(E, -1); m.node_int.assign(N, -1); m.node_scale.assign(N, -1);
    m.nie = m.nin = m.nsc = 0;
    for (int t = 0; t < m.ntips; t++) m.edge_tip[tip_edge[t]] = t;
    for (int e = 0; e < E; e++) if (m.edge_tip[e] < 0) m.edge_int[e] = m.nie++;
    for (int a = 0; a < N; a++) if (indptr[a + 1] > indptr[a]) m.node_int[a] = m.nin++;
    for (int a = 0; a < N; a++) if (m.node_int[a] >= 0 && scale_node[a]) m.node_scale[a] = m.nsc++;
    m.tip_edges = tip_edge;
    m.tip_edges.push_back(-1);
}

static inline long plk_site_chunk(long S, size_t free_bytes, size_t retained_work_bytes, size_t bytes_per_site, long opt_site_chunk,
                                  int tile, bool whole_tiles)
{
    size_t budget = free_bytes > (size_t)(6ull << 30) ? free_bytes - (size_t)(4ull << 30) : free_bytes / 2;
    budget += retained_work_bytes;
    const size_t all = whole_tiles ? (size_t)((S + tile - 1) / tile * tile) : (size_t)S;
    long chunk = (long)std::min<size_t>(all, budget / bytes_per_site);
    if (opt_site_chunk > 0) chunk = std::min<long>(chunk, opt_site_chunk);
    if (whole_tiles) return chunk / tile * tile;
    if (chunk < 1) return 0;
    if (chunk < S) chunk = std::max<long>(tile, chunk / tile * tile);
    return chunk;
}


struct PlkChain {
    std::vector<plk_op4> ops;
    int first_slot = -1, first_row = 0;
    int second_row = 0;
};

static inline void plk_chain_build(int N, const PlkProgram &pg, int mode, const int *indices, const int *node_int,
                                   const int *edge_int, const int *node_scale, PlkChain &ch, const char *skip_store = nullptr)
{
    const int ntips = (int)pg.tip_edge.size();
    std::vector<int> row(N, -1);
    for (size_t r = 0; r < pg.obs_nodes.size(); r++) row[pg.obs_nodes[r]] = (int)r;
    ch.ops.assign(pg.ops.size() + 1, plk_op4{OP_END, 0, 0, 0});
    ch.first_slot = -1; ch.first_row = 0;
    int prev = -1;
    for (size_t pc = 0; pc < pg.ops.size(); pc++) {
        const int code = pg.ops[pc].x & 0xff;
        plk_op4 o = {pg.ops[pc].x, pg.ops[pc].y, 0, 0};
        if (code == OP_TIP_SET || code == OP_TIP_MUL || code == OP_NODE_MUL) {
            const int slot = code == OP_NODE_MUL ? ntips : (o.x >> 8);
            o.y = row[pg.ops[pc].y];
            if (mode != 2) {
                if (prev < 0) { ch.first_slot = slot; ch.first_row = o.y; }
                else { ch.ops[prev].z = slot; ch.ops[prev].w = o.y; }
                prev = (int)pc;
            }
        } else if (code == OP_MATVEC && mode >= 1) {
            o.y = pg.op_edge[pc];
            o.z = node_int ? node_int[indices[o.y]] : 0;
            if (mode >= 1 && skip_store && skip_store[indices[o.y]]) o.z = -1;
            if (mode == 2) o.w = edge_int[o.y];
        } else if (code == OP_SCALE && mode >= 1 && node_scale) {
            o.y = pc < pg.op_mid.size() && pg.op_mid[pc] ? -1 : node_scale[pg.ops[pc].y];
        }
        ch.ops[pc] = o;
    }
    if (prev >= 0) { ch.ops[prev].z = ch.first_slot | (1 << 30); ch.ops[prev].w = ch.first_row; }
    if (mode == 3) {
        std::vector<int> opc_, rows_;
        for (size_t pc = 0; pc < pg.ops.size(); pc++) {
            const int code = pg.ops[pc].x & 0xff;
            if (code == OP_TIP_SET || code == OP_TIP_MUL || code == OP_NODE_MUL) { opc_.push_back((int)pc); rows_.push_back(ch.ops[pc].y); }
        }
        const size_t no = opc_.size();
        ch.second_row = no ? rows_[1 % no] : 0;
        for (size_t i = 0; i < no; i++) ch.ops[opc_[i]].y = rows_[(i + 2) % no];
// ... 362 lines not shown
```

Before: 6.343 billion.

## Move per-category V4S program parameters into a device record table

Per-category parameters for the V4S/V4P assembly programs (ops and mstream pointers, first_y offsets, pair shift, root weights) are precomputed on the host into a 64-byte record per category and uploaded to the device. The inline assembly now loads them with scalar loads from a record pointer instead of taking many SGPR operands computed in the kernel. The kernel also reads kernel arguments through the kernarg segment pointer, narrows its unit indexing to 32 bits, and moves the mixing helper into a shared header. The aim is to cut scalar register pressure and per-category setup work in the hot loop. The cost is an extra dependent scalar load and wait at program start and end, plus a new device buffer to keep in sync.

```diff
diff --git a/phyly_amd/csrc/plk_engine.hip b/phyly_amd/csrc/plk_engine.hip
--- a/phyly_amd/csrc/plk_engine.hip
+++ b/phyly_amd/csrc/plk_engine.hip
@@ -100,6 +100,7 @@
     uint8_t *d_quad_lut = nullptr;
     int *d_quad_codes = nullptr;
     double *d_llstate = nullptr; size_t llstate_cap = 0;
+    PlkV4SRecord *d_v4s_rec = nullptr;
     int num_cus = 256;
     int2 *d_ops = nullptr;
     int4 *d_fops = nullptr;
@@ -1435,7 +1436,7 @@
     void *ptrs[] = {h->d_indptr, h->d_indices, h->d_preorder, h->d_Qn, h->d_edge_rates, h->d_cat_rates,
                     h->d_cat_prior, h->d_root_w, h->d_Pdd, h->d_P, h->d_dP, h->d_scratch, h->d_codes,
                     h->d_defs, h->d_B, h->d_w, h->d_ops, h->d_fops, h->d_words, h->d_mat_edge, h->d_edge_slot, h->d_op_edge, h->d_tip_edge, h->d_obs_nodes,
-                    h->d_words_pt, h->d_row_nodes, h->d_tabs, h->d_quad_lut, h->d_quad_codes, h->d_llstate, h->d_cstream, h->d_obs_row, h->d_PS, h->d_tip, h->d_frag, h->d_root_wd, h->d_mops, h->d_u4pack, h->d_u4tip, h->d_uvmat, h->d_stage, h->d_exL, h->d_exF, h->d_exmask, h->d_exscr, h->d_slots, h->d_site_ll, h->d_partial, h->d_work,
+                    h->d_words_pt, h->d_row_nodes, h->d_tabs, h->d_quad_lut, h->d_quad_codes, h->d_llstate, h->d_v4s_rec, h->d_cstream, h->d_obs_row, h->d_PS, h->d_tip, h->d_frag, h->d_root_wd, h->d_mops, h->d_u4pack, h->d_u4tip, h->d_uvmat, h->d_stage, h->d_exL, h->d_exF, h->d_exmask, h->d_exscr, h->d_slots, h->d_site_ll, h->d_partial, h->d_work,
                     h->d_cp_fops, h->d_cp_ops, h->d_cp_mat_edge, h->d_cp_tip_edge, h->d_cp_obs_nodes, h->d_cp_op_edge, h->d_cp_expo, h->d_cp_flag,
                     h->d_cp_PS, h->d_cp_tip, h->d_cp_out, h->d_cp_partial, h->d_mixD,
                     h->d_plPdd, h->d_plP, h->d_plrates, h->d_plstream, h->d_plT, h->d_pldense, h->d_plcodes};
@@ -2012,7 +2013,7 @@
     if ((rc = upload_pair_table_lists(h))) return rc;
     if (c.variant == PLK_K4_V4S) {
         const size_t total = (size_t)nunits * vs.chunks * PLK_V4S_UNIT;
-        if (total > h->cstream_cap || (total + 255) / 256 > 0x7fffffffu) { h->err = "internal: code stream size"; return PLK_E_ARG; }
+        if (total > h->cstream_cap || (total + 255) / 256 > 0x7fffffffu || nunits > 0x7fffffff) { h->err = "internal: code stream size"; return PLK_E_ARG; }
         hipLaunchKernelGGL(k_build_code_stream, dim3((unsigned)((total + 255) / 256)), dim3(256), 0, h->stream, h->d_codes, h->Spad, nunits,
                            h->d_obs_row, vs.nobs, h->d_row_nodes, (int)f.row_node.size(), h->nchar, vs.chunks,
                            f.nquads > 0 ? h->d_quad_lut : (const uint8_t *)nullptr, h->d_cstream);
@@ -2024,6 +2025,11 @@
     if ((rc = dev_reserve(h, &h->d_PS, &h->ps_cap, (size_t)h->C * (f.mat_edge.size() + 1) * 16))) return rc;
     if ((rc = dev_reserve(h, &h->d_tip, &h->tip_cap, (size_t)h->C * f.units * h->nchar * 4))) return rc;
     HIPCHK(h, hipMemsetAsync(h->d_PS, 0, (size_t)h->C * (f.mat_edge.size() + 1) * 16 * sizeof(double), h->stream));
+    if (c.variant == PLK_K4_V4S) {
+        const std::vector<PlkV4SRecord> recs = plk_v4s_records(p.k4s, h->C, (unsigned)(f.units * h->nchar), (unsigned long long)(uintptr_t)h->d_words_pt,
+                                                               (unsigned long long)(uintptr_t)h->d_PS, f.mat_edge.size(), h->root_w.data());
+        if ((rc = dev_upload(h, &h->d_v4s_rec, recs.data(), recs.size()))) return rc;
+    }
     return PLK_OK;
 }
 
@@ -2259,11 +2265,11 @@
             const PlkK4Stream &r = p.k4s;
             const bool pairmul = r.runs == PlkK4Stream::PAIR;
             sa.pt.nwords = (int)r.stride();
-            sa.stream = h->d_cstream; sa.chunks = r.fv4s.chunks; sa.first_y = r.fv4s.first_y[0];
+            sa.stream = h->d_cstream; sa.chunks = r.fv4s.chunks;
             sa.sync = r.sync;
             h->info_ll_barrier = (sa.sync == 0 ? 1 : sa.sync == 1 ? 2 : 3) | (r.sync_auto ? 16 : 0);
-            sa.first_y1 = pairmul ? r.pair.first_y1[0] : 0u; sa.first_b1 = pairmul ? r.pair.first_b1 : 0u;
             sa.groups = r.triple.groups; sa.cg = r.triple.Cg > 0 ? r.triple.Cg : h->C;
+            sa.rec = h->d_v4s_rec;
             sa.part_sum = h->d_llstate;
             sa.part_exp = h->d_llstate ? reinterpret_cast<int *>(h->d_llstate + (size_t)((S + PLK_V4S_UNIT - 1) / PLK_V4S_UNIT) * PLK_V4S_UNIT) : nullptr;
             if (sa.groups > 1) {
diff --git a/phyly_amd/csrc/plk_fused4_v4p_asm.h b/phyly_amd/csrc/plk_fused4_v4p_asm.h
--- a/phyly_amd/csrc/plk_fused4_v4p_asm.h
+++ b/phyly_amd/csrc/plk_fused4_v4p_asm.h
@@ -10,6 +10,8 @@
 #define PLK_V4P_GEN_OBS_FOLDED {1, 4, 12, 13, 14, 21, 22}
 
 #define PLK_V4P_PROGRAM_HELD \
+        "s_load_dwordx8 s[36:43], %[rec], 0x0\n\t" \
+        "s_mov_b64 s[32:33], %[rec]\n\t" \
         "v_mov_b32 v24, 0\n\t" \
         "v_mov_b32 v25, 0x3ff00000\n\t" \
         "v_mov_b32 v32, 0\n\t" \
@@ -35,32 +37,36 @@
         "s_addc_u32 s35, s35, 0\n\t" \
         "v_mov_b32 v78, 0\n\t" \
         "v_mov_b32 v79, 0\n\t" \
-        "s_mov_b64 s[20:21], %[ops]\n\t" \
-        "s_mov_b64 s[30:31], %[mstream]\n\t" \
+        "s_getpc_b64 s[24:25]\n\t" \
+        ".Lpcref_%=:\n" \
+        "s_add_u32 s26, s24, .Lh0_%=-.Lpcref_%=\n\t" \
+        "s_addc_u32 s25, s25, 0\n\t" \
         "s_movk_i32 s27, 0xfc02\n\t" \
         "s_mov_b32 m0, 0\n\t" \
+        "s_waitcnt lgkmcnt(0)\n\t" \
+        "s_mov_b64 s[20:21], s[36:37]\n\t" \
+        "s_mov_b64 s[30:31], s[38:39]\n\t" \
+        "s_mov_b32 s22, s40\n\t" \
+        "s_mov_b32 s23, s41\n\t" \
+        "s_mov_b32 s28, s42\n\t" \
         "s_load_dwordx16 s[68:83], s[20:21], 0x0\n\t" \
         "s_load_dwordx16 s[84:99], s[20:21], 0x40\n\t" \
         "s_add_u32 s20, s20, 0x80\n\t" \
         "s_addc_u32 s21, s21, 0\n\t" \
         "s_load_dwordx16 s[36:51], s[30:31], 0x0\n\t" \
         "s_load_dwordx16 s[52:67], s[30:31], 0x40\n\t" \
-        "s_getpc_b64 s[24:25]\n\t" \
-        ".Lpcref_%=:\n" \
-        "s_add_u32 s26, s24, .Lh0_%=-.Lpcref_%=\n\t" \
-        "s_addc_u32 s25, s25, 0\n\t" \
         "v_bfe_u32 v72, v74, 0, 8\n\t" \
         "v_bfe_u32 v73, v75, 0, 8\n\t" \
-        "v_add_lshl_u32 v72, v72, %[y0], 5\n\t" \
-        "v_add_lshl_u32 v73, v73, %[y0], 5\n\t" \
-        "ds_read_b128 v[56:59], v72\n\t" \
-        "ds_read_b128 v[60:63], v72 offset:16\n\t" \
-        "ds_read_b128 v[64:67], v73\n\t" \
-        "ds_read_b128 v[68:71], v73 offset:16\n\t" \
-        "v_bfe_u32 v72, v74, %[b1], 8\n\t" \
-        "v_bfe_u32 v73, v75, %[b1], 8\n\t" \
-        "v_add_lshl_u32 v72, v72, %[y1], 5\n\t" \
-        "v_add_lshl_u32 v73, v73, %[y1], 5\n\t" \
+        "v_add_lshl_u32 v72, v72, s22, 5\n\t" \
+        "v_add_lshl_u32 v73, v73, s22, 5\n\t" \
+        "ds_read_b128 v[56:59], v72\n\t" \
+        "ds_read_b128 v[60:63], v72 offset:16\n\t" \
+        "ds_read_b128 v[64:67], v73\n\t" \
+        "ds_read_b128 v[68:71], v73 offset:16\n\t" \
+        "v_bfe_u32 v72, v74, s28, 8\n\t" \
+        "v_bfe_u32 v73, v75, s28, 8\n\t" \
+        "v_add_lshl_u32 v72, v72, s23, 5\n\t" \
+        "v_add_lshl_u32 v73, v73, s23, 5\n\t" \
         "ds_read_b128 v[130:133], v72\n\t" \
         "ds_read_b128 v[134:137], v72 offset:16\n\t" \
         "ds_read_b128 v[138:141], v73\n\t" \
@@ -1938,15 +1944,16 @@
         "s_setpc_b64 s[24:25]\n\t" \
         ".p2align 9\n" \
         ".Ldone_%=:\n" \
+        "s_load_dwordx8 s[20:27], s[32:33], 0x20\n\t" \
         "s_waitcnt vmcnt(0) lgkmcnt(0)\n\t" \
-        "v_mul_f64 v[40:41], %[w0], v[24:25]\n\t" \
-        "v_fma_f64 v[40:41], %[w1], v[26:27], v[40:41]\n\t" \
-        "v_fma_f64 v[40:41], %[w2], v[28:29], v[40:41]\n\t" \
-        "v_fma_f64 v[40:41], %[w3], v[30:31], v[40:41]\n\t" \
-        "v_mul_f64 v[48:49], %[w0], v[32:33]\n\t" \
-        "v_fma_f64 v[48:49], %[w1], v[34:35], v[48:49]\n\t" \
-        "v_fma_f64 v[48:49], %[w2], v[36:37], v[48:49]\n\t" \
-        "v_fma_f64 v[48:49], %[w3], v[38:39], v[48:49]\n\t" \
+        "v_mul_f64 v[40:41], s[20:21], v[24:25]\n\t" \
+        "v_fma_f64 v[40:41], s[22:23], v[26:27], v[40:41]\n\t" \
+        "v_fma_f64 v[40:41], s[24:25], v[28:29], v[40:41]\n\t" \
+        "v_fma_f64 v[40:41], s[26:27], v[30:31], v[40:41]\n\t" \
+        "v_mul_f64 v[48:49], s[20:21], v[32:33]\n\t" \
+        "v_fma_f64 v[48:49], s[22:23], v[34:35], v[48:49]\n\t" \
+        "v_fma_f64 v[48:49], s[24:25], v[36:37], v[48:49]\n\t" \
+        "v_fma_f64 v[48:49], s[26:27], v[38:39], v[48:49]\n\t" \
         "v_mov_b32 %[al], v40\n\t" \
         "v_mov_b32 %[ah], v41\n\t" \
         "v_mov_b32 %[bl], v48\n\t" \
diff --git a/phyly_amd/csrc/plk_fused4_v4s.h b/phyly_amd/csrc/plk_fused4_v4s.h
--- a/phyly_amd/csrc/plk_fused4_v4s.h
+++ b/phyly_amd/csrc/plk_fused4_v4s.h
@@ -3,19 +3,25 @@
 
 #include "plk_fused4_v4s_asm.h"
 #include "plk_fused4_v4p_asm.h"
+#include "plk_mix.h"
 
 struct FusedV4SArgs {
     FusedPTArgs pt;
     const unsigned *stream;
     int chunks;
-    unsigned first_y;
     int sync;
-    unsigned first_y1, first_b1;
     int groups, cg;
+    const PlkV4SRecord *rec;
     double *part_sum;
     int *part_exp;
 };
-#define PLK_V4S_NO_TERM INT_MIN
+
+__device__ __forceinline__ const PLK_AS4 FusedV4SArgs *fused_v4s_args()
+{
+    auto p = __builtin_amdgcn_kernarg_segment_ptr();
+    asm volatile("" : "+s"(p));
+    return (const PLK_AS4 FusedV4SArgs *)p;
+}
 
 __global__ __launch_bounds__(256) void k_build_code_stream(const uint8_t *__restrict__ codes, long Spad, long nunits,
                                                            const int *__restrict__ obs_row, int nobs, const int *__restrict__ row_nodes ,
@@ -32,11 +38,8 @@
 }
 
 template <bool HELD, bool PAIR>
-__device__ __forceinline__ void fused_run_program_v4s(double &lha, double &lhb, int &ea, int &eb, const void *ops, const void *mstream,
-                                                       const void *strm, unsigned voff, unsigned y0,
-                                                       double w0, double w1, double w2, double w3,
-                                                       unsigned long long c0, unsigned long long c1, unsigned long long c2,
-                                                       unsigned y1, unsigned b1)
+__device__ __forceinline__ void fused_run_program_v4s(double &lha, double &lhb, int &ea, int &eb, const void *rec, const void *strm, unsigned voff,
+                                                       unsigned long long c0, unsigned long long c1, unsigned long long c2)
 {
     int al, ah, bl, bh;
 #ifdef PLK_EXP_EMPTY
@@ -46,20 +49,17 @@
     if constexpr (PAIR)
         asm volatile(PLK_V4P_PROGRAM_HELD
                      : [al] "=v"(al), [ah] "=v"(ah), [bl] "=v"(bl), [bh] "=v"(bh), [ea] "=v"(ea), [eb] "=v"(eb)
-                     : [voff] "v"(voff), [ops] "s"(ops), [mstream] "s"(mstream), [strm] "s"(strm), [y0] "s"(y0), [y1] "s"(y1), [b1] "s"(b1),
-                       [w0] "s"(w0), [w1] "s"(w1), [w2] "s"(w2), [w3] "s"(w3), [c0] "v"(c0), [c1] "v"(c1), [c2] "v"(c2)
+                     : [voff] "v"(voff), [rec] "s"(rec), [strm] "s"(strm), [c0] "v"(c0), [c1] "v"(c1), [c2] "v"(c2)
                      : PLK_V4S_CLOBBERS);
     else if constexpr (HELD)
         asm volatile(PLK_V4S_PROGRAM_HELD
                      : [al] "=v"(al), [ah] "=v"(ah), [bl] "=v"(bl), [bh] "=v"(bh), [ea] "=v"(ea), [eb] "=v"(eb)
-                     : [voff] "v"(voff), [ops] "s"(ops), [mstream] "s"(mstream), [strm] "s"(strm), [y0] "s"(y0),
-                       [w0] "s"(w0), [w1] "s"(w1), [w2] "s"(w2), [w3] "s"(w3), [c0] "v"(c0), [c1] "v"(c1), [c2] "v"(c2)
+                     : [voff] "v"(voff), [rec] "s"(rec), [strm] "s"(strm), [c0] "v"(c0), [c1] "v"(c1), [c2] "v"(c2)
                      : PLK_V4S_CLOBBERS);
     else
         asm volatile(PLK_V4S_PROGRAM
                      : [al] "=v"(al), [ah] "=v"(ah), [bl] "=v"(bl), [bh] "=v"(bh), [ea] "=v"(ea), [eb] "=v"(eb)
-                     : [voff] "v"(voff), [ops] "s"(ops), [mstream] "s"(mstream), [strm] "s"(strm), [y0] "s"(y0),
-                       [w0] "s"(w0), [w1] "s"(w1), [w2] "s"(w2), [w3] "s"(w3)
+                     : [voff] "v"(voff), [rec] "s"(rec), [strm] "s"(strm)
                      : PLK_V4S_CLOBBERS);
 #endif
     lha = __hiloint2double(ah, al);
@@ -69,37 +69,33 @@
 template <int THREADS, bool HELD = false, bool PAIR = false, bool GROUPS = false>
 __global__ __launch_bounds__(THREADS) void k_ll_fused4_v4s(FusedV4SArgs va)
 {
-    constexpr int NW = THREADS / 64;
-    const FusedPTArgs &aa = va.pt;
-    const FusedArgs &a = aa.f;
+    constexpr unsigned NW = THREADS / 64;
     extern __shared__ double lds_dyn[];
-    const int tip_doubles = a.ntips * a.nchar * 4;
     const int tid = threadIdx.x;
-    const int lane = tid & 63, wave = __builtin_amdgcn_readfirstlane(tid >> 6);
-    const PLK_AS4 double *prior = as_uniform(a.cat_prior);
-    const PLK_AS4 double *rootw = as_uniform(a.root_w);
-    const bool plain = a.root_mode == PLK_ROOT_NONE || a.root_mode == PLK_ROOT_UNIFORM;
-    const double wu = a.root_mode == PLK_ROOT_NONE ? 1.0 : 0.25;
-    const double rw0 = plain ? wu : rootw[0], rw1 = plain ? wu : rootw[1], rw2 = plain ? wu : rootw[2], rw3 = plain ? wu : rootw[3];
-    const long nunits = (a.S + PLK_V4S_UNIT - 1) / PLK_V4S_UNIT;
-    const unsigned cat32 = (unsigned)(a.ntips * a.nchar);
+    const int lane = tid & 63;
+    const unsigned wave = (unsigned)__builtin_amdgcn_readfirstlane(tid >> 6);
     dd acc = dd_make(0.0, 0.0);
-    const long stride = (long)gridDim.x * NW, passes = (nunits + stride - 1) / stride;
+    const unsigned nunits = (unsigned)((va.pt.f.S + PLK_V4S_UNIT - 1) / PLK_V4S_UNIT);
+    const unsigned stride = gridDim.x * NW, first = blockIdx.x * NW + wave, passes = (nunits + stride - 1) / stride;
     const int ngroups = GROUPS ? va.groups : 1;
     for (int g = 0; g < ngroups; g++) {
-        const int c_lo = GROUPS ? g * va.cg : 0, c_hi = GROUPS ? min(a.C, c_lo + va.cg) : a.C;
+        int c_hi;
         if (GROUPS && g > 0) __syncthreads();
         {
-            const double2 *src = reinterpret_cast<const double2 *>(a.tip) + (size_t)c_lo * (tip_doubles / 2);
+            const PLK_AS4 FusedV4SArgs *k = fused_v4s_args();
+            const int C = k->pt.f.C, c_lo = GROUPS ? g * k->cg : 0;
+            c_hi = GROUPS ? min(C, c_lo + k->cg) : C;
+            const int tip_doubles = k->pt.f.ntips * k->pt.f.nchar * 4;
+            const double2 *src = reinterpret_cast<const double2 *>(k->pt.f.tip) + (size_t)c_lo * (tip_doubles / 2);
             double2 *dst = reinterpret_cast<double2 *>(lds_dyn);
             const int n2 = (c_hi - c_lo) * (tip_doubles / 2);
-            int first = tid;
+            int i_first = tid;
             if (GROUPS) {
                 int l;
                 asm volatile("v_mbcnt_lo_u32_b32 %0, -1, 0\n\tv_mbcnt_hi_u32_b32 %0, -1, %0" : "=v"(l));
-                first = wave * 64 + l;
-            }
-            for (int i0 = first; i0 < n2; i0 += 4 * THREADS) {
+                i_first = (int)wave * 64 + l;
+            }
+            for (int i0 = i_first; i0 < n2; i0 += 4 * THREADS) {
                 double2 v[4];
 #pragma unroll
                 for (int u = 0; u < 4; u++) v[u] = i0 + u * THREADS < n2 ? src[i0 + u * THREADS] : double2{0.0, 0.0};
@@ -109,80 +105,98 @@
         }
         __syncthreads();
         unsigned long long c0 = 0, c1 = 0, c2 = 0;
-        auto request = [&](long unit) {
+        auto request = [&](unsigned unit) {
+            asm volatile("" : "+s"(unit));
+            const PLK_AS4 FusedV4SArgs *k = fused_v4s_args();
             unsigned off = (unsigned)lane * 8u;
             asm volatile("" : "+v"(off));
-            const char *p = reinterpret_cast<const char *>(va.stream + (size_t)unit * (size_t)va.chunks * PLK_V4S_UNIT) + off;
+            const char *p = reinterpret_cast<const char *>(k->stream) + (size_t)unit * ((size_t)(unsigned)k->chunks * (PLK_V4S_UNIT * sizeof(unsigned))) + off;
             c0 = *reinterpret_cast<const unsigned long long *>(p);
             c1 = *reinterpret_cast<const unsigned long long *>(p + PLK_V4S_CHUNK_BYTES);
             c2 = *reinterpret_cast<const unsigned long long *>(p + 2 * PLK_V4S_CHUNK_BYTES);
         };
-        if (HELD && (long)blockIdx.x * NW + wave < nunits) request((long)blockIdx.x * NW + wave);
-        for (long pass = 0; pass < passes; pass++) {
-            const long u = pass * stride + (long)blockIdx.x * NW + wave;
+        double nsum[2];
+        int nexp[2];
+        auto start = [&](unsigned unit, bool exists) {
+            if (GROUPS && g > 0 && exists) {
+                asm volatile("" : "+s"(unit));
+                const PLK_AS4 FusedV4SArgs *k = fused_v4s_args();
+                unsigned off = (unsigned)lane * 8u, off4 = (unsigned)lane * 4u;
+                asm volatile("" : "+v"(off), "+v"(off4));
+                const char *ps = reinterpret_cast<const char *>(k->part_sum) + (size_t)unit * (PLK_V4S_UNIT * sizeof(double)) + off;
+                const char *pe = reinterpret_cast<const char *>(k->part_exp) + (size_t)unit * (PLK_V4S_UNIT * sizeof(int)) + off4;
+#pragma unroll
+                for (int j = 0; j < 2; j++) {
+                    nsum[j] = *reinterpret_cast<const double *>(ps + j * 64 * sizeof(double));
+                    nexp[j] = *reinterpret_cast<const int *>(pe + j * 64 * sizeof(int));
+                }
+            } else {
+                nsum[0] = nsum[1] = 0.0;
+                nexp[0] = nexp[1] = PLK_V4S_NO_TERM;
+            }
+        };
+        start(first, first < nunits);
+        if (HELD && first < nunits) request(first);
+        for (unsigned pass = 0; pass < passes; pass++) {
+            unsigned u = pass * stride + first;
+            asm volatile("" : "+s"(u));
             const bool active = u < nunits;
-            const unsigned *strm = va.stream + (size_t)(active ? u : 0) * (size_t)va.chunks * PLK_V4S_UNIT;
-            double sum[2] = {0.0, 0.0};
-            int Eexp[2] = {0, 0};
-            bool have[2] = {false, false};
-            if (GROUPS && g > 0 && active) {
-#pragma unroll
-                for (int j = 0; j < 2; j++) {
-                    const size_t s = (size_t)u * PLK_V4S_UNIT + j * 64 + lane;
-                    sum[j] = va.part_sum[s]; Eexp[j] = va.part_exp[s];
-                    have[j] = Eexp[j] != PLK_V4S_NO_TERM;
-                }
-            }
-            if (va.sync & 1) __syncthreads();
-            for (int c = c_lo; c < c_hi; c++) {
-                const double *ps = a.PS + (size_t)c * (a.nmat + 1) * 16;
-                const unsigned *ops = aa.words + (size_t)c * aa.nwords;
-                if (va.sync & 2) __syncthreads();
+            double sum[2] = {nsum[0], nsum[1]};
+            int Eexp[2] = {nexp[0], nexp[1]};
+            if (fused_v4s_args()->sync & 1) __syncthreads();
+            for (unsigned c = GROUPS ? (unsigned)(g * fused_v4s_args()->cg) : 0u; c < (unsigned)c_hi; c++) {
+                const PLK_AS4 FusedV4SArgs *k = fused_v4s_args();
+                if (k->sync & 2) __syncthreads();
                 if (!active) continue;
-                if (aa.warm) {
-                    fused_touch_lines(ps, (unsigned)(a.nmat + 1) * 128u, (unsigned)wave * 64u, NW * 64u);
-                    fused_touch_lines(ops, (unsigned)aa.nwords * 4u, (unsigned)wave * 64u, NW * 64u);
-                }
+                unsigned cc = c, uu = u;
+                asm volatile("" : "+s"(cc), "+s"(uu));
+                if (k->pt.warm) {
+                    const int nmat = k->pt.f.nmat, nwords = k->pt.nwords;
+                    fused_touch_lines(k->pt.f.PS + (size_t)cc * (nmat + 1) * 16, (unsigned)(nmat + 1) * 128u, wave * 64u, NW * 64u);
+                    fused_touch_lines(k->pt.words + (size_t)cc * nwords, (unsigned)nwords * 4u, wave * 64u, NW * 64u);
+                }
+                const unsigned *strm = k->stream + (size_t)uu * ((size_t)(unsigned)k->chunks * PLK_V4S_UNIT);
                 double lhs[2];
                 int esc[2];
-                fused_run_program_v4s<HELD, PAIR>(lhs[0], lhs[1], esc[0], esc[1], ops, ps, strm, (unsigned)lane * 8u, va.first_y + (unsigned)(c - c_lo) * cat32,
-                                                  rw0, rw1, rw2, rw3, c0, c1, c2, va.first_y1 + (unsigned)(c - c_lo) * cat32, va.first_b1);
-#pragma unroll
-                for (int j = 0; j < 2; j++) {
-                    const double lh = lhs[j];
-                    const double term = prior[c] * lh;
-                    if (term != 0.0) {
-                        if (!have[j]) { sum[j] = term; Eexp[j] = esc[j]; have[j] = true; }
-                        else if (esc[j] > Eexp[j]) { sum[j] = ldexp(sum[j], Eexp[j] - esc[j]) + term; Eexp[j] = esc[j]; }
-                        else sum[j] += ldexp(term, esc[j] - Eexp[j]);
-                    }
-                }
-            }
-            if (HELD && u + stride < nunits) request(u + stride);
+                fused_run_program_v4s<HELD, PAIR>(lhs[0], lhs[1], esc[0], esc[1], k->rec + cc, strm, (unsigned)lane * 8u, c0, c1, c2);
+                const double prior = as_uniform(fused_v4s_args()->pt.f.cat_prior)[c];
+#pragma unroll
+                for (int j = 0; j < 2; j++) plk_mix_term(sum[j], Eexp[j], prior * lhs[j], esc[j]);
+            }
+            const bool next = active && u + stride < nunits;
+            start(u + stride, next);
+            if (HELD && next) request(u + stride);
+            const PLK_AS4 FusedV4SArgs *k = fused_v4s_args();
             if (GROUPS && g + 1 < ngroups) {
                 if (active) {
+                    unsigned off = (unsigned)lane * 8u, off4 = (unsigned)lane * 4u;
+                    char *ps = reinterpret_cast<char *>(k->part_sum) + (size_t)u * (PLK_V4S_UNIT * sizeof(double)) + off;
+                    char *pe = reinterpret_cast<char *>(k->part_exp) + (size_t)u * (PLK_V4S_UNIT * sizeof(int)) + off4;
 #pragma unroll
                     for (int j = 0; j < 2; j++) {
-                        const size_t s = (size_t)u * PLK_V4S_UNIT + j * 64 + lane;
-                        va.part_sum[s] = sum[j]; va.part_exp[s] = have[j] ? Eexp[j] : PLK_V4S_NO_TERM;
+                        *reinterpret_cast<double *>(ps + j * 64 * sizeof(double)) = sum[j];
+                        *reinterpret_cast<int *>(pe + j * 64 * sizeof(int)) = Eexp[j];
                     }
                 }
-                continue;
-            }
-#pragma unroll
-            for (int j = 0; j < 2; j++) {
-                const long s = u * PLK_V4S_UNIT + j * 64 + lane;
-                const double ll = have[j] ? log(sum[j]) + (double)Eexp[j] * 0.6931471805599453094 : -INFINITY;
-                if (active && s < a.S) {
-                    if (a.site_ll) a.site_ll[s] = ll;
-                    acc = dd_add(acc, dd_weighted(a.w, s, ll));
+            } else {
+                const long S = k->pt.f.S;
+                double *site_ll = k->pt.f.site_ll;
+                const double *w = k->pt.f.w;
+#pragma unroll
+                for (int j = 0; j < 2; j++) {
+                    const long s = (long)u * PLK_V4S_UNIT + j * 64 + lane;
+                    const double ll = Eexp[j] != PLK_V4S_NO_TERM ? log(sum[j]) + (double)Eexp[j] * 0.6931471805599453094 : -INFINITY;
+                    if (active && s < S) {
+                        if (site_ll) site_ll[s] = ll;
+                        acc = dd_add(acc, dd_weighted(w, s, ll));
+                    }
                 }
             }
         }
     }
-    if (a.partial) {
+    if (va.pt.f.partial) {
         const dd r = dd_wave_sum(acc);
-        if (lane == 0) a.partial[(size_t)blockIdx.x * NW + wave] = r;
+        if (lane == 0) va.pt.f.partial[(size_t)blockIdx.x * NW + wave] = r;
     }
 }
 
diff --git a/phyly_amd/csrc/plk_fused4_v4s_asm.h b/phyly_amd/csrc/plk_fused4_v4s_asm.h
--- a/phyly_amd/csrc/plk_fused4_v4s_asm.h
+++ b/phyly_amd/csrc/plk_fused4_v4s_asm.h
@@ -7,6 +7,8 @@
 #define PLK_V4S_FOLD_SCALE 60
 
 #define PLK_V4S_PROLOGUE \
+        "s_load_dwordx8 s[36:43], %[rec], 0x0\n\t" \
+        "s_mov_b64 s[32:33], %[rec]\n\t" \
         "v_mov_b32 v24, 0\n\t" \
         "v_mov_b32 v25, 0x3ff00000\n\t" \
         "v_mov_b32 v32, 0\n\t" \
@@ -33,25 +35,29 @@
         "s_addc_u32 s35, s35, 0\n\t" \
         "v_mov_b32 v78, 0\n\t" \
         "v_mov_b32 v79, 0\n\t" \
-        "s_mov_b64 s[20:21], %[ops]\n\t" \
-        "s_mov_b64 s[30:31], %[mstream]\n\t" \
+        "s_getpc_b64 s[24:25]\n\t" \
+        ".Lpcref_%=:\n" \
+        "s_add_u32 s26, s24, .Lh0_%=-.Lpcref_%=\n\t" \
+        "s_addc_u32 s25, s25, 0\n\t" \
         "s_movk_i32 s27, 0xfc02\n\t" \
         "s_mov_b32 m0, 0\n\t" \
+        "s_waitcnt lgkmcnt(0)\n\t" \
+        "s_mov_b64 s[20:21], s[36:37]\n\t" \
+        "s_mov_b64 s[30:31], s[38:39]\n\t" \
+        "s_mov_b32 s22, s40\n\t" \
+        "s_mov_b32 s23, s41\n\t" \
+        "s_mov_b32 s28, s42\n\t" \
         "s_load_dwordx16 s[68:83], s[20:21], 0x0\n\t" \
         "s_load_dwordx16 s[84:99], s[20:21], 0x40\n\t" \
         "s_add_u32 s20, s20, 0x80\n\t" \
         "s_addc_u32 s21, s21, 0\n\t" \
         "s_load_dwordx16 s[36:51], s[30:31], 0x0\n\t" \
         "s_load_dwordx16 s[52:67], s[30:31], 0x40\n\t" \
-        "s_getpc_b64 s[24:25]\n\t" \
-        ".Lpcref_%=:\n" \
-        "s_add_u32 s26, s24, .Lh0_%=-.Lpcref_%=\n\t" \
-        "s_addc_u32 s25, s25, 0\n\t" \
         "s_waitcnt vmcnt(2)\n\t" \
         "v_bfe_u32 v72, v74, 0, 8\n\t" \
         "v_bfe_u32 v73, v75, 0, 8\n\t" \
-        "v_add_lshl_u32 v72, v72, %[y0], 5\n\t" \
-        "v_add_lshl_u32 v73, v73, %[y0], 5\n\t" \
+        "v_add_lshl_u32 v72, v72, s22, 5\n\t" \
+        "v_add_lshl_u32 v73, v73, s22, 5\n\t" \
         "ds_read_b128 v[56:59], v72\n\t" \
         "ds_read_b128 v[60:63], v72 offset:16\n\t" \
         "ds_read_b128 v[64:67], v73\n\t" \
@@ -64,6 +70,8 @@
         ""
 
 #define PLK_V4S_PROLOGUE_HELD \
+        "s_load_dwordx8 s[36:43], %[rec], 0x0\n\t" \
+        "s_mov_b64 s[32:33], %[rec]\n\t" \
         "v_mov_b32 v24, 0\n\t" \
         "v_mov_b32 v25, 0x3ff00000\n\t" \
         "v_mov_b32 v32, 0\n\t" \
@@ -89,24 +97,28 @@
         "s_addc_u32 s35, s35, 0\n\t" \
         "v_mov_b32 v78, 0\n\t" \
         "v_mov_b32 v79, 0\n\t" \
-        "s_mov_b64 s[20:21], %[ops]\n\t" \
-        "s_mov_b64 s[30:31], %[mstream]\n\t" \
+        "s_getpc_b64 s[24:25]\n\t" \
+        ".Lpcref_%=:\n" \
+        "s_add_u32 s26, s24, .Lh0_%=-.Lpcref_%=\n\t" \
+        "s_addc_u32 s25, s25, 0\n\t" \
         "s_movk_i32 s27, 0xfc02\n\t" \
         "s_mov_b32 m0, 0\n\t" \
+        "s_waitcnt lgkmcnt(0)\n\t" \
+        "s_mov_b64 s[20:21], s[36:37]\n\t" \
+        "s_mov_b64 s[30:31], s[38:39]\n\t" \
+        "s_mov_b32 s22, s40\n\t" \
+        "s_mov_b32 s23, s41\n\t" \
+        "s_mov_b32 s28, s42\n\t" \
         "s_load_dwordx16 s[68:83], s[20:21], 0x0\n\t" \
         "s_load_dwordx16 s[84:99], s[20:21], 0x40\n\t" \
         "s_add_u32 s20, s20, 0x80\n\t" \
         "s_addc_u32 s21, s21, 0\n\t" \
         "s_load_dwordx16 s[36:51], s[30:31], 0x0\n\t" \
         "s_load_dwordx16 s[52:67], s[30:31], 0x40\n\t" \
-        "s_getpc_b64 s[24:25]\n\t" \
-        ".Lpcref_%=:\n" \
-        "s_add_u32 s26, s24, .Lh0_%=-.Lpcref_%=\n\t" \
-        "s_addc_u32 s25, s25, 0\n\t" \
         "v_bfe_u32 v72, v74, 0, 8\n\t" \
         "v_bfe_u32 v73, v75, 0, 8\n\t" \
-        "v_add_lshl_u32 v72, v72, %[y0], 5\n\t" \
-        "v_add_lshl_u32 v73, v73, %[y0], 5\n\t" \
+        "v_add_lshl_u32 v72, v72, s22, 5\n\t" \
+        "v_add_lshl_u32 v73, v73, s22, 5\n\t" \
         "ds_read_b128 v[56:59], v72\n\t" \
         "ds_read_b128 v[60:63], v72 offset:16\n\t" \
         "ds_read_b128 v[64:67], v73\n\t" \
@@ -2027,15 +2039,16 @@
         "s_setpc_b64 s[24:25]\n\t" \
         ".p2align 9\n" \
         ".Ldone_%=:\n" \
+        "s_load_dwordx8 s[20:27], s[32:33], 0x20\n\t" \
         "s_waitcnt vmcnt(0) lgkmcnt(0)\n\t" \
-        "v_mul_f64 v[40:41], %[w0], v[24:25]\n\t" \
-        "v_fma_f64 v[40:41], %[w1], v[26:27], v[40:41]\n\t" \
-        "v_fma_f64 v[40:41], %[w2], v[28:29], v[40:41]\n\t" \
-        "v_fma_f64 v[40:41], %[w3], v[30:31], v[40:41]\n\t" \
-        "v_mul_f64 v[48:49], %[w0], v[32:33]\n\t" \
-        "v_fma_f64 v[48:49], %[w1], v[34:35], v[48:49]\n\t" \
-        "v_fma_f64 v[48:49], %[w2], v[36:37], v[48:49]\n\t" \
-        "v_fma_f64 v[48:49], %[w3], v[38:39], v[48:49]\n\t" \
+        "v_mul_f64 v[40:41], s[20:21], v[24:25]\n\t" \
+        "v_fma_f64 v[40:41], s[22:23], v[26:27], v[40:41]\n\t" \
+        "v_fma_f64 v[40:41], s[24:25], v[28:29], v[40:41]\n\t" \
+        "v_fma_f64 v[40:41], s[26:27], v[30:31], v[40:41]\n\t" \
+        "v_mul_f64 v[48:49], s[20:21], v[32:33]\n\t" \
+        "v_fma_f64 v[48:49], s[22:23], v[34:35], v[48:49]\n\t" \
+        "v_fma_f64 v[48:49], s[24:25], v[36:37], v[48:49]\n\t" \
+        "v_fma_f64 v[48:49], s[26:27], v[38:39], v[48:49]\n\t" \
         "v_mov_b32 %[al], v40\n\t" \
         "v_mov_b32 %[ah], v41\n\t" \
         "v_mov_b32 %[bl], v48\n\t" \
diff --git a/phyly_amd/csrc/plk_mix.h b/phyly_amd/csrc/plk_mix.h
--- /dev/null
+++ b/phyly_amd/csrc/plk_mix.h
@@ -0,0 +1,29 @@
+#ifndef PLK_MIX_H
+#define PLK_MIX_H
+
+#include <limits.h>
+#include <math.h>
+
+#define PLK_V4S_NO_TERM INT_MIN
+
+#if defined(__HIPCC__) || defined(__CUDACC__)
+#define PLK_MIX_FN __host__ __device__ __forceinline__
+#else
+#define PLK_MIX_FN static inline
+#endif
+
+#define PLK_MIX_MAX_SHIFT 2200u
+
+PLK_MIX_FN void plk_mix_term(double &sum, int &E, double term, int esc)
+{
+    const bool up = esc > E;
+    const unsigned dist = up ? (unsigned)esc - (unsigned)E : (unsigned)E - (unsigned)esc;
+    const int shift = -(int)(dist < PLK_MIX_MAX_SHIFT ? dist : PLK_MIX_MAX_SHIFT);
+    const double moved = ldexp(up ? sum : term, shift);
+    const double added = up ? moved + term : sum + moved;
+    const bool use = term != 0.0;
+    sum = use ? added : sum;
+    E = use ? (up ? esc : E) : E;
+}
+
+#endif
diff --git a/phyly_amd/csrc/plk_program.h b/phyly_amd/csrc/plk_program.h
--- a/phyly_amd/csrc/plk_program.h
+++ b/phyly_amd/csrc/plk_program.h
@@ -4,6 +4,7 @@
 #include <algorithm>
 #include <climits>
 #include <cmath>
+#include <cstddef>
 #include <cstdint>
 #include <cstdio>
 #include <string>
@@ -2237,6 +2238,33 @@
     int Cg(int C) const { return triple.nodes + triple.quads > 0 && triple.Cg > 0 ? triple.Cg : C; }
 };
 
+struct PlkV4SRecord {
+    unsigned long long ops, mstream;
+    unsigned first_y, first_y1, first_b1, pad;
+    double w[4];
+};
+static_assert(sizeof(PlkV4SRecord) == 64 && offsetof(PlkV4SRecord, first_y) == 16 && offsetof(PlkV4SRecord, w) == 32, "the assembly text names these offsets");
+
+static inline std::vector<PlkV4SRecord> plk_v4s_records(const PlkK4Stream &r, int C, unsigned cat32, unsigned long long words, unsigned long long ps,
+                                                       size_t nmat, const double *root_w)
+{
+    std::vector<PlkV4SRecord> out((size_t)C);
+    const bool pairmul = r.runs == PlkK4Stream::PAIR;
+    const int cg = r.triple.groups > 1 && r.triple.Cg > 0 ? r.triple.Cg : C;
+    for (int c = 0; c < C; c++) {
+        PlkV4SRecord &q = out[c];
+        q.ops = words + (unsigned long long)c * r.stride() * sizeof(unsigned);
+        q.mstream = ps + (unsigned long long)c * (nmat + 1) * 16 * sizeof(double);
+        const unsigned image = (unsigned)(c % cg) * cat32;
+        q.first_y = r.fv4s.first_y[0] + image;
+        q.first_y1 = pairmul ? r.pair.first_y1[0] + image : 0u;
+        q.first_b1 = pairmul ? r.pair.first_b1 : 0u;
+        q.pad = 0;
+        for (int i = 0; i < 4; i++) q.w[i] = root_w[i];
+    }
+    return out;
+}
+
 static inline bool plk_k4_stream_can_group(const PlkK4Choice &ch, const PlkK4StreamCaps &caps) { return ch.pair && ch.fold && ch.held && caps.held && caps.pair && caps.groups; }
 
 static inline void plk_k4_stream_fold_pair(PlkK4Stream &r, bool fold, bool pair, bool pair_kept = false)
```

Result: faster. 6.593 billion (median of 6 runs) (+3.9%).
